# jaeyoungchoilab/Topsicle

Measured on AMD Instinct MI355X. Metric: bases_scanned_per_sec, higher is better.
Workload: dtype u8

## Files before the change

### __graft_entry__.py

```python
import os
import shutil
import subprocess
import sys

ROOT = os.path.dirname(os.path.abspath(__file__))
CSRC = os.path.join(ROOT, "topsicle_amd", "csrc")
LIB = os.path.join(ROOT, "topsicle_amd", "libtopsicle_hip.so")


def _newer(target, deps):
    return os.path.exists(target) and all(os.path.getmtime(target) >= os.path.getmtime(d) for d in deps)


HIP_FLAGS = ["--offload-arch=gfx950", "-O3", "-fno-vectorize", "-std=c++17", "-fPIC", "-Wall", "-Wno-unused-variable"]
KGROUPS = 18


def _build_hip_split(out, extra=()):
    hipcc = shutil.which("hipcc") or "/opt/rocm/bin/hipcc"
    flags = os.environ.get("TPS_HIPCC_EXTRA", "").split() + HIP_FLAGS + list(extra)
    bdir = os.path.join(CSRC, "_build", os.path.splitext(os.path.basename(out))[0])
    os.makedirs(bdir, exist_ok=True)
    jobs = []
    for g in range(KGROUPS):
        src = "topsicle_hip.hip" if g == 0 else "tps_kernels.hip"
        obj = os.path.join(bdir, f"group{g}.o")
        jobs.append((obj, subprocess.Popen([hipcc] + flags + [f"-DTPS_KGROUP={g}", "-c", "-o", obj, os.path.join(CSRC, src)], cwd=CSRC)))
    failed = [obj for obj, p in jobs if p.wait() != 0]
    if failed:
        raise RuntimeError("hipcc failed for " + ", ".join(failed))
    subprocess.check_call([hipcc, "--offload-arch=gfx950", "-shared", "-fPIC", "-o", out] + [obj for obj, _ in jobs], cwd=CSRC)
    return out


def build_hip(force=False):
    deps = [os.path.join(CSRC, f) for f in ("topsicle_hip.hip", "tps_kernels.hip", "tps_kernels.h", "tps_device.h", "tps_wave.h", "tps_plan.h", "tps_pack.h", "tps_wide.h", "tps_wide_plan.h")] + \
           [os.path.join(ROOT, "include", "topsicle_hip.h")]
    if not force and _newer(LIB, deps):
        return LIB
    return _build_hip_split(LIB)


def build_hip_diag():
    return _build_hip_split(os.path.join(ROOT, "topsicle_amd", "libtopsicle_hip_diag.so"), extra=["-DTPS_STAMPS"])


def build_io(force=False):
    src = os.path.join(CSRC, "tps_io.cpp")
    out = os.path.join(ROOT, "topsicle_amd", "libtopsicle_io.so")
    if not force and _newer(out, [src, os.path.join(CSRC, "tps_pack.h"), os.path.join(CSRC, "tps_gzpar.h"), os.path.join(ROOT, "include", "topsicle_hip.h")]):
        return out
    subprocess.check_call(["g++", "-O2", "-std=c++17", "-shared", "-fPIC", "-Wall", "-o", out, src, "-lz", "-lpthread"])
    return out


def build_oracle():
    mk = os.path.join(ROOT, "oracle", "Makefile")
    if os.path.exists(mk):
        subprocess.check_call(["make", "-s", "-C", os.path.join(ROOT, "oracle")])


def build_emulation():
    sys.path.insert(0, os.path.join(ROOT, "tests"))
    sys.path.insert(0, ROOT)
    import emu_driver
    import emu_wide_driver
    emu_driver.build()
    emu_wide_driver.build()


def build_sanitizer_variants():
    sys.path.insert(0, os.path.join(ROOT, "tests"))
    sys.path.insert(0, ROOT)
    import emu_driver
    import emu_wide_driver
    import test_sanitizers
    emu_driver.build(asan=True)
    emu_wide_driver.build(asan=True)
    test_sanitizers._build_io_asan()


def build() -> None:
    import threading
    errs = []

    def side(fn):
        try:
            fn()
        except BaseException as e:
            errs.append(e)
    th = [threading.Thread(target=side, args=(fn,)) for fn in (build_emulation, build_sanitizer_variants)]
    for t in th:
        t.start()
    build_hip()
    build_io()
    build_oracle()
    for t in th:
        t.join()
    if errs:
        raise errs[0]
    sys.path.insert(0, ROOT)
    import topsicle_amd
    from topsicle_amd import hiplib
    lib = hiplib.load_library()
    assert lib.tps_abi_version() == 4
    print("built", LIB)


def smoke() -> None:
    sys.path.insert(0, ROOT)
    sys.path.insert(0, os.path.join(ROOT, "oracle"))
    import numpy as np
    from topsicle_amd import hiplib, synth
    import topsicle_oracle as orc

    motif, k = "CCCTAA", 4
    pats = orc.kmer_table(motif, k)
    bases, offsets, _ = synth.make_reads(24, 3000, motif, seed=7, tract_min=300, tract_max=1500)
    seqs = synth.split_reads(bases, offsets)
    ratio = 1000 / len(motif)
    min_count = max(c for c in range(1001) if not (c / ratio > 0.4))
    with hiplib.HipScanner(0) as sc:
        print("smoke on:", sc.device_info())
        sc.set_patterns(pats)
        sc.upload(0, bases, offsets)
        prm = hiplib.make_params(min_len=1000, min_count=min_count, window=100, slide=6, trimfirst=100, maxlen=20000,
                                 flags=hiplib.F_STEP1 | hiplib.F_WINDOWS | hiplib.F_BINSEG | hiplib.F_STORE_SUMS)
        sc.scan(0, prm)
        sc.sync()
        res = sc.results(0)
        sums, win_off = sc.window_sums(0)
    n_pass = 0
    for i, seq in enumerate(seqs):
        cs, ce = orc.trc_counts(seq, pats)
        call = orc.trc_call(cs, ce, pats, len(motif), 0.4)
        assert bool(res["pass"][i]) == (call is not None), i
        if call is None:
            continue
        n_pass += 1
        tail = call[1]
        assert res["tail"][i] == (0 if tail == "forward" else 1)
        _, counts = orc.window_count_matrix(seq, tail, pats, 100, 6, 100, 20000)
        assert np.array_equal(sums[win_off[i]:win_off[i + 1]], counts.sum(axis=1)), i
        assert res["bkp"][i] == orc.binseg_l2_exact(counts.sum(axis=1)), i
    assert n_pass >= 12
    print(f"smoke ok: {len(seqs)} reads, {n_pass} telomeric, per-window counts bit-exact, boundaries equal")


if __name__ == "__main__":
    build()
    if len(sys.argv) > 1 and sys.argv[1] == "smoke":
        smoke()
```

### topsicle_amd/csrc/tps_device.h

```cpp
#pragma once
#include <stdint.h>
#include "../../include/topsicle_hip.h"
#include "tps_wave.h"

namespace tps {

constexpr int WPG = 4;
constexpr int WPG_MAX = 8;
constexpr uint32_t FLAG_CONFLICT = 0x80000000u;
constexpr uint32_t FLAG16 = 0x8000u;
constexpr int HIST_COPIES = 8;
constexpr int WIN_U = 4;
constexpr int COOP_MAX = 24;

typedef unsigned __int128 u128;

constexpr int cgcd(int a, int b) { return b == 0 ? a : cgcd(b, a % b); }
constexpr int clog2(int x) { return x <= 1 ? 0 : 1 + clog2(x / 2); }

struct PatInfo {
    int32_t P, k;
    uint32_t kmask;
    uint32_t all_mask;
    uint32_t so_mask;
    uint32_t dup_mask;
    int32_t n_periods;
    int32_t period[8];
    uint32_t period_pat[8];
    uint32_t hash_mul, hash_shift;
};

struct ScanArgs {
    const uint32_t* seq2;
    const uint16_t* inv;
    const tps_read_desc* desc;
    const uint8_t* tails_in;
    const uint32_t* lut;
    const uint32_t* lut_img;
    const uint32_t* pair_img;
    tps_read_result* results;
    int32_t* c_start;
    int32_t* c_end;
    const int64_t* win_off;
    int32_t* sums;
    uint16_t* sums16;
    const int64_t* win_off16;
    uint8_t* raw;
    uint64_t* stamps;
    int32_t raw_m;
    const int64_t* raw_win_off;
    const int32_t* order;
    int64_t n_reads;
    PatInfo pat;
    tps_params prm;
    int32_t variant;
    int32_t lut_n;
    int32_t seq_dw;
    int32_t head_dw;
    int32_t nblk_cap;
    int32_t spans_per_tile;
    int32_t span_dw;
    int32_t blk_log2;
    int32_t rec_rs;
    int32_t tot_dw;
    int32_t blk_dw;
    int32_t lc_cap;
    uint32_t jump_magic;
    int32_t q, r, lw;
    int32_t lc16;
    int32_t lc_global;
    int32_t lc_stride;
    uint16_t* lc_scratch;
    int32_t pair_n;
    int32_t tile_cap;
    int32_t tw;
    uint32_t tw_magic;
    int32_t tile_full;
    int32_t wpg;
    int32_t pp_d;
    int32_t so_fast;
    int32_t val_on;
    int32_t seq_alias;
    int32_t lut_fields;
    int32_t lut16;
    int32_t xt_alias;
    int32_t xt_own;
    int32_t pair16;
};

struct BinsegArgs {
    const int32_t* sums;
    const int64_t* win_off;
    int32_t* bkp;
    double* gain;
    int64_t n_reads;
    int32_t n_patterns, jump, min_size;
    uint8_t* tie;
};

constexpr int MISC_DW = 20;
constexpr int XS_DW = 64 + NT + 4 * NT + NT + 16 * 5 + 8;
constexpr int HIST_STRIDE = 33;
constexpr int HIST_DW = 2 * HIST_COPIES * HIST_STRIDE;
struct Lds {
    uint32_t* lut;
    uint32_t* lut2;
    int lshift;
    uint32_t* seq2;
    uint16_t* val;
    uint32_t* blk;
    uint32_t* G;
    uint32_t* Gp;
    uint16_t* C0;
    uint16_t* C1;
    uint32_t* XPC;
    uint32_t* XF;
    uint32_t* XT;
    uint32_t* Tot;
    uint32_t* Lc;
    uint16_t* Lc16;
    uint32_t* Tc;
    uint32_t* row;
    uint32_t* misc;
};
constexpr int XLANES = NT + 16;
TPS_HD int64_t xchg_dw(const ScanArgs& a) {
    return 9ll * NT + (a.xt_alias == 2 ? 0ll : 2ll) * XLANES;
}
TPS_HD int64_t lut_dw(const ScanArgs& a) { return a.lut16 ? ((((int64_t)a.lut_n + 1) / 2 + 3) & ~3ll) : (((int64_t)a.lut_n + 3) & ~3ll); }
TPS_HD int64_t blk_region_dw(const ScanArgs& a) {
    int64_t need = a.variant ? xchg_dw(a) : 2ll * a.nblk_cap + 2ll * ((a.nblk_cap + 1) / 2);
    if (need < XS_DW) need = XS_DW;
    if (need < HIST_DW) need = HIST_DW;
    return (need + 3) & ~3ll;
}
TPS_HD int64_t val_dw(const ScanArgs& a) { return a.val_on ? ((a.seq_dw + 4 + 3) / 4) * 2 : 0; }
TPS_HD int64_t lc_dw(const ScanArgs& a) {
    if (a.lc16) return (a.lc_global ? 0 : ((a.lc_cap + 3) / 4) * 2) + ((a.tile_cap + 1) / 2) * 2;
    return a.lc_global ? 0 : ((a.lc_cap + 1) / 2) * 2;
}
TPS_HD int64_t row_dw(const ScanArgs& a) {
    const int64_t fused = a.variant ? ((int64_t)NT << a.blk_log2) + NT : 0;
    return fused > WIN_U * NT ? fused : WIN_U * NT;
}
TPS_DEV Lds carve(uint32_t* base, uint32_t* lut, const ScanArgs& a) {
    Lds l;
    l.lut2 = lut - a.pair_n;
    uint32_t* p = base;
    l.blk = p;  p += a.blk_dw;
    l.lut = lut;
    l.lshift = a.variant ? 16 : 0;
    l.seq2 = p; p += a.seq_dw;
    l.val = (uint16_t*)p;  p += val_dw(a);
    l.Tot = p;  p += a.tot_dw;
    l.Lc = p;
    l.Lc16 = (uint16_t*)p;
    l.Tc = p + ((a.lc16 && a.lc_global) ? 0 : ((a.lc_cap + 3) / 4) * 2);
    p += lc_dw(a);
    l.row = p;  p += row_dw(a);
    l.misc = p;
    l.G = l.blk;
    l.Gp = l.G + a.nblk_cap;
    l.C0 = (uint16_t*)(l.Gp + a.nblk_cap);
    l.C1 = l.C0 + ((a.nblk_cap + 1) / 2) * 2;
    l.XPC = l.blk;
    l.XF = l.XPC + 9 * NT;
    l.XT = l.XF + XLANES;
    return l;
}
TPS_HD int64_t lds_dwords(const ScanArgs& a) {
    return (int64_t)a.blk_dw + (a.seq_alias ? 0 : a.seq_dw) + val_dw(a) + a.tot_dw + lc_dw(a) + row_dw(a) + MISC_DW +
           ((a.xt_alias && a.xt_own) ? (a.xt_alias == 2 ? 2 : 1) * XLANES : 0);
}
TPS_HD int64_t wg_lds_dwords(const ScanArgs& a) { return a.pair_n + lut_dw(a) + (int64_t)(a.wpg > 0 ? a.wpg : WPG) * ((lds_dwords(a) + 3) & ~3ll); }
constexpr int M_BEST = 0;
constexpr int M_CMASK = 2;
constexpr int M_INVALID = 4;
constexpr int M_SCAN = 10;
constexpr int M_MAXSC = 6;
constexpr int M_BESTB = 8;
constexpr int M_NTIE = 9;
constexpr int X_Q = 0;
constexpr int X_BS = 64;
constexpr int X_CD = X_BS + NT;
constexpr int X_CDEN = X_CD + 2 * NT;
constexpr int X_CB = X_CDEN + 2 * NT;
constexpr int X_R = X_CB + NT;

TPS_DEV int padded(int i, int pad_log2) { return i + (i >> pad_log2); }
TPS_DEV uint32_t wg_exclusive_scan(uint32_t* arr, int n, uint32_t* scratch, int pad_log2 = 30) {
    (void)scratch;
    const int per = (n + NT - 1) / NT;
    Lane<uint32_t> s;
    TPS_LANES {
        const int lo = tid * per, hi = (lo + per < n) ? lo + per : n;
        uint32_t t = 0;
        for (int i = lo; i < hi; ++i) t += arr[padded(i, pad_log2)];
        TPS_AT(s) = t;
    }
    const Lane<uint32_t> inc = wave_incl_sum(s);
    const uint32_t total = wave_read_lane(inc, 63);
    TPS_LANES {
        const int lo = tid * per, hi = (lo + per < n) ? lo + per : n;
        uint32_t run = TPS_AT(inc) - TPS_AT(s);
        for (int i = lo; i < hi; ++i) { uint32_t t = arr[padded(i, pad_log2)]; arr[padded(i, pad_log2)] = run; run += t; }
    }
    TPS_SYNC();
    return total;
}

struct Stage {
    uint64_t q0;
    uint64_t v0;
    int32_t delta;
    int32_t nq;
    int32_t n;
    bool reverse;
};
TPS_DEV Stage stage_plan(const uint32_t* seq2_base, const uint16_t* inv_base, int64_t word_off, int64_t L, bool reverse, int64_t t, int64_t i0, int32_t n) {
    Stage st;
    st.reverse = reverse;
    st.n = n;
    const int64_t pos = reverse ? (L - 1 - t - i0) : (t + i0);
    const int64_t w = word_off + 4 * (pos >> 6);
    st.delta = reverse ? 63 - (int32_t)(pos & 63) : (int32_t)(pos & 63);
    st.q0 = (uint64_t)(uintptr_t)seq2_base + (uint64_t)w * 4u;
    st.v0 = (uint64_t)(uintptr_t)inv_base + (uint64_t)w * 2u;
    st.nq = n > 0 ? (st.delta + n + 63) >> 6 : 0;
    return st;
}
constexpr int STAGE_KMAX = 1 << 16;
TPS_DEV const uint8_t* stage_addr(const Stage& st, int c) {
    const uint8_t* base = (const uint8_t*)(uintptr_t)(st.reverse ? st.q0 - 16ull * STAGE_KMAX : st.q0);
    const uint32_t off = st.reverse ? 16u * (uint32_t)(STAGE_KMAX - c) : 16u * (uint32_t)c;
    return base + off;
}
TPS_DEV const uint8_t* stage_inv_addr(const Stage& st, int c) {
    const uint8_t* base = (const uint8_t*)(uintptr_t)(st.reverse ? st.v0 - 8ull * STAGE_KMAX : st.v0);
    const uint32_t off = st.reverse ? 8u * (uint32_t)(STAGE_KMAX - c) : 8u * (uint32_t)c;
    return base + off;
}
TPS_DEV uint32_t rev2(uint32_t x) {
    const uint32_t y = bitrev32(x);
    return ((y >> 1) & 0x55555555u) | ((y & 0x55555555u) << 1);
}
TPS_DEV u32x4 stage_reversed(const u32x4& v) {
    u32x4 r;
    r.x = rev2(v.w); TPS_PIN_V(r.x);
    r.y = rev2(v.z); TPS_PIN_V(r.y);
    r.z = rev2(v.y); TPS_PIN_V(r.z);
    r.w = rev2(v.x); TPS_PIN_V(r.w);
    return r;
}
TPS_DEV u32x4 stage_orient(const Stage& st, const u32x4& v) {
    if (!st.reverse) return v;
    u32x4 r;
    r.x = rev2(v.w); r.y = rev2(v.z); r.z = rev2(v.y); r.w = rev2(v.x);
    return r;
}
TPS_DEV uint32_t stage_lane_off(bool reverse, int lane) { return reverse ? 16u * (uint32_t)(STAGE_KMAX - lane) : 16u * (uint32_t)lane; }
TPS_DEV const uint8_t* stage_base(const Stage& st, int c0) {
    return (const uint8_t*)(uintptr_t)(st.reverse ? st.q0 - 16ull * STAGE_KMAX - 16ull * (uint32_t)c0 : st.q0 + 16ull * (uint32_t)c0);
}
TPS_DEV const uint8_t* stage_inv_base(const Stage& st, int c0) {
    return (const uint8_t*)(uintptr_t)(st.reverse ? st.v0 - 8ull * STAGE_KMAX - 8ull * (uint32_t)c0 : st.v0 + 8ull * (uint32_t)c0);
}
TPS_DEV u32x2 stage_orient_inv(const Stage& st, const u32x2& v) {
    if (!st.reverse) return v;
    u32x2 r;
    r.x = bitrev32(v.y); r.y = bitrev32(v.x);
    return r;
}

TPS_DEV void stage_thread(const Stage& st, bool has_inv, uint32_t* seq2, uint16_t* val, int nqd, uint32_t* invalid_flag, int tid) {
    for (int base = tid; base < nqd; base += 4 * NT) {
        u32x4 v[4];
        u32x2 b[4];
        TPS_UNROLL
        for (int u = 0; u < 4; ++u) {
            const int c = base + u * NT;
            v[u].x = v[u].y = v[u].z = v[u].w = 0;
            b[u].x = b[u].y = 0;
            if (c < nqd && c < st.nq) {
                v[u] = load16(stage_addr(st, c));
                if (has_inv) b[u] = load8(stage_inv_addr(st, c));
            }
        }
        TPS_UNROLL
        for (int u = 0; u < 4; ++u) {
            const int c = base + u * NT;
            if (c < nqd) {
                lds_store16(seq2 + 4 * c, stage_orient(st, v[u]));
                if (has_inv) {
                    const u32x2 o = stage_orient_inv(st, b[u]);
                    if (o.x | o.y) *invalid_flag = 1u;
                    lds_store8((uint32_t*)val + 2 * c, o);
                }
            }
        }
    }
}

TPS_DEV uint32_t v_at(const uint32_t* seq2, int q) {
    int idx = q >> 4;
    return alignbit(seq2[idx + 1], seq2[idx], (uint32_t)(q & 15) * 2u);
}
TPS_DEV bool invalid_at(const uint16_t* val, int q, int k) {
    int idx = q >> 4;
    uint64_t v = (uint64_t)val[idx] | ((uint64_t)val[idx + 1] << 16) | ((uint64_t)val[idx + 2] << 32);
    return ((v >> (q & 15)) & ((1ull << k) - 1ull)) != 0;
}
constexpr int LUT_FIELDS = 32;
constexpr int LUT_M16 = 48;
constexpr int LUT_F16 = 64;
TPS_HD int pp_field(int p) { return 4 * (p & 3) + 2 * ((p >> 2) & 1) + (p >> 3); }
TPS_HD int pp_pattern(int f) { return (f >> 2) + 4 * (((f >> 1) & 1) + 2 * (f & 1)); }
TPS_HD uint32_t mask_to_fields(uint32_t m) {
    uint32_t f = 0;
    for (int p = 0; p < 16; ++p) f |= ((m >> p) & 1u) << (2 * pp_field(p));
    return f;
}
TPS_DEV uint32_t field_to_mask(uint32_t f) { return f ? 1u << pp_pattern(ffs0(f) >> 1) : 0u; }
TPS_DEV uint32_t field_to_entry(uint32_t f) { return f ? ((1u << (16 + pp_pattern(ffs0(f) >> 1))) | 1u) : 0u; }
template <int N> struct IntC { static constexpr int value = N; };
TPS_DEV uint32_t lut_mask(const uint32_t* lut, int lshift, const PatInfo& pat, uint32_t v) {
    const uint32_t code = v & pat.kmask;
    if (pat.hash_shift) {
        const uint32_t slot = (code * pat.hash_mul) >> pat.hash_shift;
        return lut[2 * slot] == code ? lut[2 * slot + 1] : 0u;
    }
    if (lshift == LUT_FIELDS) return field_to_mask(lut[code]);
    if (lshift == LUT_M16) return ((const uint16_t*)lut)[code];
    if (lshift == LUT_F16) { const uint32_t m = ((const uint16_t*)lut)[code]; return m ? 1u << pp_pattern(ffs0(m)) : 0u; }
    return lut[code] >> lshift;
}
TPS_DEV uint32_t h_at(const uint32_t* lut, int lshift, const uint32_t* seq2, const uint16_t* val, const PatInfo& pat, int q, bool any_invalid) {
    uint32_t h = lut_mask(lut, lshift, pat, v_at(seq2, q));
    if (any_invalid && h && invalid_at(val, q, pat.k)) h = 0;
    return h;
}
TPS_DEV uint32_t conflict_bits(const PatInfo& pat, uint32_t v, uint32_t h) {
    if (pat.hash_shift) return h & pat.so_mask;
    uint32_t c = 0;
    TPS_NOVEC
    for (int i = 0; i < pat.n_periods; ++i) {
        uint32_t hp = h & pat.period_pat[i];
        if (hp && (((v ^ (v >> (2 * pat.period[i]))) & pat.kmask) == 0)) c |= hp;
    }
    return c;
}

TPS_DEV void greedy_count(const uint32_t* lut, int lshift, const uint32_t* seq2, const uint16_t* val, const PatInfo& pat, int q0,
                          int npos, int bit, bool any_invalid, int& occ, int& greedy) {
    occ = 0; greedy = 0;
    int cursor = 0;
    for (int p = 0; p < npos; ++p) {
        uint32_t h = h_at(lut, lshift, seq2, val, pat, q0 + p, any_invalid);
        if ((h >> bit) & 1u) {
            ++occ;
            if (p >= cursor) { ++greedy; cursor = p + pat.k; }
        }
    }
}

template <bool PLAIN>
TPS_DEV void trc_count_thread(const ScanArgs& a, const Lds& l, const Stage& st_s, const Stage& st_e, int tid) {
    const PatInfo& pat = a.pat;
    const int side = tid >> 5, t = tid & 31;
    const int delta = side ? st_e.delta : st_s.delta;
    const uint32_t* seq2 = l.seq2 + side * a.head_dw;
    const uint16_t* val = l.val + side * a.head_dw;
    const bool inv = !PLAIN && l.misc[M_INVALID] != 0;
    const bool so = !PLAIN && pat.so_mask != 0;
    const int npos = st_s.n - pat.k + 1;
    uint32_t* hist = l.blk + (side * HIST_COPIES + (tid & (HIST_COPIES - 1))) * HIST_STRIDE;
    uint32_t cm = 0;
    for (int p0 = t * 8; p0 < npos; p0 += 32 * 8) {
        const int q0 = delta + p0, idx = q0 >> 4;
        const uint32_t sh = (uint32_t)(q0 & 15) * 2u;
        const uint32_t d0 = seq2[idx], d1 = seq2[idx + 1], d2 = seq2[idx + 2];
        const uint32_t w0 = alignbit(d1, d0, sh), w1 = alignbit(d2, d1, sh);
        uint32_t h[8], v[8];
        TPS_UNROLL
        for (int j = 0; j < 8; ++j) {
            v[j] = j ? alignbit(w1, w0, 2u * j) : w0;
            h[j] = lut_mask(l.lut, l.lshift, pat, v[j]);
        }
        TPS_UNROLL
        for (int j = 0; j < 8; ++j) {
            uint32_t hj = h[j];
            if (p0 + j >= npos) hj = 0;
            if (PLAIN) {
                if (hj) lds_add(&hist[ffs0(hj)], 1u);
            } else {
                if (hj && inv && invalid_at(val, q0 + j, pat.k)) hj = 0;
                if (hj) {
                    if (so && (hj & pat.so_mask)) cm |= conflict_bits(pat, v[j], hj);
                    do {
                        int b = ffs0(hj);
                        hj &= hj - 1;
                        lds_add(&hist[b], 1u);
                    } while (hj);
                }
            }
        }
    }
    if (!PLAIN && cm) lds_or(&l.misc[M_CMASK + side], cm);
}
TPS_DEV int min_period(const PatInfo& pat) {
    int m = pat.k;
    TPS_NOVEC
    for (int i = 0; i < pat.n_periods; ++i) m = pat.period[i] < m ? pat.period[i] : m;
    return m;
}
TPS_DEV bool trc_packed_ok(const ScanArgs& a, int npos) {
    const int nchunks = (npos + 15) >> 4, iters = (nchunks + 31) >> 5;
    const int mp = min_period(a.pat);
    int maxd = 0;
    TPS_NOVEC
    for (int i = 0; i < a.pat.n_periods; ++i) maxd = a.pat.period[i] > maxd ? a.pat.period[i] : maxd;
    return a.pat.P <= 15 && maxd <= 6 && mp >= 3 && npos <= 255 * mp && iters * ((16 + mp - 1) / mp) <= 15;
}
template <bool SO_, int FMT = 0>
TPS_DEV void trc_count_packed(const ScanArgs& a, const Lds& l, const Stage& st_s, const Stage& st_e, int tid, uint32_t* keep = nullptr) {
    const PatInfo& pat = a.pat;
    const int side = tid >> 5, t = tid & 31;
    const int delta = side ? st_e.delta : st_s.delta;
    const uint32_t* seq2 = l.seq2 + side * a.head_dw;
    constexpr bool FLD = FMT == 1, M16 = FMT == 2 || FMT == 3, F16 = FMT == 3;
    constexpr int LS = M16 ? 1 : 2;
    const uint32_t amask = pat.kmask << LS;
    const int npos = st_s.n - pat.k + 1;
    const int nchunks = (npos + 15) >> 4;
    const int k = pat.k;
    auto fieldsq = [&](uint32_t h) -> uint32_t { return FLD ? h : M16 ? mul24(h, h) : mulhi32(h, h); };
    uint32_t ne = 0, no = 0;
    uint32_t pe = 0, po = 0, te = 0, to = 0;
    uint32_t cf = 0;
    for (int c0 = 0; c0 < nchunks; c0 += 32) {
        const int c = c0 + t;
        const int bo = 2 * (delta + 16 * c) - LS;
        const int idx = bo >> 5;
        const uint32_t sh = (uint32_t)(bo & 31);
        const uint32_t d0 = seq2[idx], d1 = seq2[idx + 1], d2 = seq2[idx + 2];
        const uint32_t w0 = alignbit(d1, d0, sh), w1 = alignbit(d2, d1, sh);
        uint32_t h[16];
        TPS_UNROLL
        for (int j = 0; j < 16; ++j) {
            const uint32_t v_ = j == 0 ? w0 : alignbit(w1, w0, 2u * j);
            h[j] = M16 ? lut16_at(l.lut, v_, amask) : lut_at(l.lut, v_, amask);
        }
        const bool last_pass = 16 * (c0 + 32) + 32 > npos;
        if (last_pass) {
            int nv = npos - 16 * c;
            TPS_PIN_V(nv);
            TPS_UNROLL
            for (int j = 0; j < 16; ++j)
                if (j >= nv) h[j] = 0;
        }
        TPS_UNROLL
        for (int half = 0; half < 2; ++half) {
            uint32_t x2 = 0;
            TPS_UNROLL
            for (int j = 8 * half; j < 8 * half + 8; ++j) x2 += fieldsq(h[j]);
            ne += x2 & 0x33333333u;
            no += (x2 >> 2) & 0x33333333u;
        }
        if (SO_) {
            const uint32_t w2 = alignbit(seq2[idx + 3], d2, sh);
            const uint32_t a0 = alignbit(w1, w0, (uint32_t)LS), a1 = alignbit(w2, w1, (uint32_t)LS), a2 = w2 >> LS;
            TPS_NOVEC
            for (int pi = 0; pi < pat.n_periods; ++pi) {
                const int d = pat.period[pi];
                const uint32_t x0 = a0 ^ alignbit(a1, a0, 2u * (uint32_t)d), x1 = a1 ^ alignbit(a2, a1, 2u * (uint32_t)d);
// ... 46 lines not shown
    dst[3] = ((no >> 4) & 0x0F0F0F0Fu) - ((po >> 4) & 0x0F0F0F0Fu) + ((to >> 4) & 0x0F0F0F0Fu);
}
constexpr int OCC_SLOTS = 4;
constexpr int OCC_BASE_DW = 256;
TPS_DEV int occ_slot(uint32_t cmask, int p) {
    return popc(cmask & ((1u << p) - 1u));
}
TPS_DEV void trc_publish_occ(const ScanArgs& a, const Lds& l, const Stage& st_s, const Stage& st_e, int tid) {
    const PatInfo& pat = a.pat;
    const int side = tid >> 5, t = tid & 31;
    const uint32_t cmask = l.misc[M_CMASK + side];
    if (!cmask || popc(cmask) > OCC_SLOTS || st_s.n - a.pat.k + 1 > 1024) return;
    const int delta = side ? st_e.delta : st_s.delta;
    const uint32_t* seq2 = l.seq2 + side * a.head_dw;
    const uint32_t amask = pat.kmask << 2;
    const int npos = st_s.n - pat.k + 1;
    const int nchunks = (npos + 15) >> 4;
    uint16_t* occ = (uint16_t*)(l.blk + OCC_BASE_DW + side * OCC_SLOTS * 32);
    for (int c = t; c < 64; c += 32) {
        uint32_t bits[OCC_SLOTS] = {0, 0, 0, 0};
        if (c < nchunks) {
            const int qm = delta + 16 * c - 1;
            const int idx = qm >> 4;
            const uint32_t sh = (uint32_t)(qm & 15) * 2u;
            const uint32_t d0 = seq2[idx], d1 = seq2[idx + 1], d2 = seq2[idx + 2];
            const uint32_t w0 = alignbit(d1, d0, sh), w1 = alignbit(d2, d1, sh);
            TPS_UNROLL
            for (int j = 0; j < 16; ++j) {
                uint32_t h = lut_mask(l.lut, l.lshift, pat, (j ? alignbit(w1, w0, 2u * j) : w0) >> 2);
                if (16 * c + j >= npos) h = 0;
                h &= cmask;
                while (h) {
                    const int b = ffs0(h);
                    h &= h - 1;
                    const int sl = occ_slot(cmask, b);
                    TPS_UNROLL
                    for (int q = 0; q < OCC_SLOTS; ++q)
                        if (q == sl) bits[q] |= 1u << j;
                }
            }
        }
        TPS_UNROLL
        for (int q = 0; q < OCC_SLOTS; ++q) occ[q * 64 + c] = (uint16_t)bits[q];
    }
}
TPS_DEV int trc_walk_occ(const Lds& l, int side, int slot, int k) {
    const uint32_t* occ = l.blk + OCC_BASE_DW + (side * OCC_SLOTS + slot) * 32;
    int greedy = 0, cursor = 0;
    for (int wd = 0; wd < 32; ++wd) {
        uint32_t m = occ[wd];
        while (m) {
            const int p = 32 * wd + ffs0(m);
            m &= m - 1;
            if (p >= cursor) { ++greedy; cursor = p + k; }
        }
    }
    return greedy;
}
TPS_DEV void trc_sum_packed(const ScanArgs& a, const Lds& l, const Stage& st_s, const Stage& st_e, int64_t r, int tid) {
    const int side = tid >> 5, p = tid & 31;
    if (p < a.pat.P) {
        const int pbyte = (l.lshift == LUT_FIELDS || l.lshift == LUT_F16) ? p : 4 * (((p & 1) << 1) | ((p >> 1) & 1)) + (p >> 2);
        const uint8_t* src = (const uint8_t*)(l.blk + 4 * 32 * side) + pbyte;
        uint32_t sm = 0;
        TPS_UNROLL
        for (int t = 0; t < 32; ++t) sm += src[16 * t];
        const uint32_t cmask = l.misc[M_CMASK + side];
        if ((cmask >> p) & 1u) {
            if (popc(cmask) <= OCC_SLOTS && st_s.n - a.pat.k + 1 <= 1024) {
                sm = (uint32_t)trc_walk_occ(l, side, occ_slot(cmask, p), a.pat.k);
            } else {
                int occ, g;
                greedy_count(l.lut, l.lshift, l.seq2 + side * a.head_dw, l.val + side * a.head_dw, a.pat, side ? st_e.delta : st_s.delta,
                             st_s.n - a.pat.k + 1, p, false, occ, g);
                sm = (uint32_t)g;
            }
        }
        int32_t* dst = side ? a.c_end : a.c_start;
        if (dst) dst[r * a.pat.P + p] = (int32_t)sm;
        lds_max_i32((int32_t*)&l.misc[M_BEST + side], (int32_t)((sm << 5) | (uint32_t)(31 - p)));
    }
}

#ifndef TPS_EMU
template <int FMT = 0>
TPS_DEV void trc_decide_packed(const ScanArgs& a, const Lds& l, const Stage& st_s, const Stage& st_e, int64_t r, uint32_t& ks, uint32_t& ke) {
    uint32_t x[4];
    TPS_PHASE { trc_count_packed<false, FMT>(a, l, st_s, st_e, tid, x); }
    uint32_t s0[4], s1[4];
    TPS_UNROLL
    for (int w = 0; w < 4; ++w) {
        uint32_t v = x[w];
        v += (uint32_t)__builtin_amdgcn_update_dpp(0, (int)v, 0x111, 0xf, 0xf, false);
        v += (uint32_t)__builtin_amdgcn_update_dpp(0, (int)v, 0x112, 0xf, 0xf, false);
        v += (uint32_t)__builtin_amdgcn_update_dpp(0, (int)v, 0x114, 0xf, 0xf, false);
        v += (uint32_t)__builtin_amdgcn_update_dpp(0, (int)v, 0x118, 0xf, 0xf, false);
        v += (uint32_t)__builtin_amdgcn_update_dpp(0, (int)v, 0x142, 0xa, 0xf, false);
        s0[w] = (uint32_t)__builtin_amdgcn_readlane((int)v, 31);
        s1[w] = (uint32_t)__builtin_amdgcn_readlane((int)v, 63);
    }
    const int P = a.pat.P;
    uint32_t bs = 0, be = 0;
    TPS_UNROLL
    for (int p = 0; p < 15; ++p) {
        if (p < P) {
            const int wi = ((p & 1) << 1) | ((p >> 1) & 1), sh = 8 * (p >> 2);
            const uint32_t c0 = (s0[wi] >> sh) & 255u, c1 = (s1[wi] >> sh) & 255u;
            const uint32_t k0 = (c0 << 5) | (uint32_t)(31 - p), k1 = (c1 << 5) | (uint32_t)(31 - p);
            bs = k0 > bs ? k0 : bs;
            be = k1 > be ? k1 : be;
        }
    }
    ks = bs;
    ke = be;
    if (a.c_start) {
        const int lane = (int)(threadIdx.x & 63u), side = lane >> 5, p = lane & 31;
        if (p < P) {
            const int wi = ((p & 1) << 1) | ((p >> 1) & 1);
            const uint32_t w0 = wi == 0 ? s0[0] : wi == 1 ? s0[1] : wi == 2 ? s0[2] : s0[3];
            const uint32_t w1 = wi == 0 ? s1[0] : wi == 1 ? s1[1] : wi == 2 ? s1[2] : s1[3];
            const uint32_t c = ((side ? w1 : w0) >> (8 * (p >> 2))) & 255u;
            (side ? a.c_end : a.c_start)[r * P + p] = (int32_t)c;
        }
    }
}
#endif

TPS_DEV void trc_sum_thread(const ScanArgs& a, const Lds& l, const Stage& st_s, const Stage& st_e, int64_t r, int tid) {
    const int side = tid >> 5, p = tid & 31;
    if (p < a.pat.P) {
        uint32_t sm = 0;
        TPS_UNROLL
        for (int c = 0; c < HIST_COPIES; ++c) sm += l.blk[(side * HIST_COPIES + c) * HIST_STRIDE + p];
        if ((l.misc[M_CMASK + side] >> p) & 1u) {
            int occ, g;
            greedy_count(l.lut, l.lshift, l.seq2 + side * a.head_dw, l.val + side * a.head_dw, a.pat, side ? st_e.delta : st_s.delta,
                         st_s.n - a.pat.k + 1, p, l.misc[M_INVALID] != 0, occ, g);
            sm = (uint32_t)g;
        }
        int32_t* dst = side ? a.c_end : a.c_start;
        if (dst) dst[r * a.pat.P + p] = (int32_t)sm;
        lds_max_i32((int32_t*)&l.misc[M_BEST + side], (int32_t)((sm << 5) | (uint32_t)(31 - p)));
    }
}

TPS_DEV void blocks_span(const ScanArgs& a, const Lds& l, int delta, int span) {
    const PatInfo& pat = a.pat;
    const int s = a.prm.slide, r = a.r, k = pat.k;
    const bool inv = l.misc[M_INVALID] != 0;
    const bool so = pat.so_mask != 0;
    const uint32_t sh2 = (uint32_t)(delta & 15) * 2u;
    const int d0 = (delta >> 4) + span * a.span_dw;
    int j = span << a.blk_log2;
    uint32_t lo = l.seq2[d0], hi = l.seq2[d0 + 1];
    uint32_t cur = alignbit(hi, lo, sh2);
    uint32_t g = 0, cnt = 0;
    int pib = 0;
    for (int dw = 0; dw < a.span_dw; ++dw) {
        uint32_t nx2 = l.seq2[d0 + dw + 2];
        uint32_t nxt = alignbit(nx2, hi, sh2);
        uint32_t v[16], h[16];
        TPS_UNROLL
        for (int i = 0; i < 16; ++i) {
            v[i] = i ? alignbit(nxt, cur, 2u * i) : cur;
            h[i] = lut_mask(l.lut, 0, pat, v[i]);
        }
        if (inv) {
            int q = ((d0 + dw) << 4) + (delta & 15);
            TPS_UNROLL
            for (int i = 0; i < 16; ++i)
                if (h[i] && invalid_at(l.val, q + i, k)) h[i] = 0;
        }
        uint32_t cf = 0;
        if (so) {
            TPS_UNROLL
            for (int i = 0; i < 16; ++i)
                if ((h[i] & pat.so_mask) && conflict_bits(pat, v[i], h[i])) cf |= 1u << i;
        }
        TPS_UNROLL
        for (int i = 0; i < 16; ++i) {
            if (pib == 0) {
                g = 0;
                l.C0[j] = (uint16_t)cnt;
                if (r == 0) { l.C1[j] = (uint16_t)cnt; l.Gp[j] = 0; }
            }
            g |= h[i];
            if ((cf >> i) & 1u) g |= FLAG_CONFLICT;
            cnt += (uint32_t)popc(h[i]);
            ++pib;
            if (pib == r) { l.C1[j] = (uint16_t)cnt; l.Gp[j] = g; }
            if (pib == s) { l.G[j] = g; ++j; pib = 0; }
        }
        hi = nx2;
        cur = nxt;
    }
    l.Tot[span] = cnt;
}

template <typename F>
TPS_DEV void scan_positions(const Lds& l, const PatInfo& pat, int q0, int npos, bool inv, F f) {
    const int idx = q0 >> 4;
    const uint32_t sh = (uint32_t)(q0 & 15) * 2u;
    uint32_t d1 = l.seq2[idx + 1];
    uint32_t cur = alignbit(d1, l.seq2[idx], sh), nxt = 0;
    for (int p = 0; p < npos; ++p) {
        const int j = p & 15;
        if (j == 0) {
            if (p) cur = nxt;
            const uint32_t d2 = l.seq2[idx + (p >> 4) + 2];
            nxt = alignbit(d2, d1, sh);
            d1 = d2;
        }
        const uint32_t v = j ? alignbit(nxt, cur, 2u * (uint32_t)j) : cur;
        uint32_t h = lut_mask(l.lut, l.lshift, pat, v);
        if (inv && h && invalid_at(l.val, q0 + p, pat.k)) h = 0;
        f(p, h);
    }
}

TPS_DEV uint32_t window_exact(const ScanArgs& a, const Lds& l, int delta, int wl, uint32_t present, uint32_t fast_sw,
                              uint8_t* raw_row, bool full = false) {
    const PatInfo& pat = a.pat;
    const bool inv = l.misc[M_INVALID] != 0;
    const int q0 = delta + wl * a.prm.slide;
    uint32_t redo = present & pat.so_mask;
    if (!raw_row && !full) {
        uint32_t sum = fast_sw;
        while (redo) {
            const int bit = ffs0(redo);
            redo &= redo - 1;
            int occ = 0, greedy = 0, cursor = 0;
            scan_positions(l, pat, q0, a.lw, inv, [&](int p, uint32_t h) {
                if ((h >> bit) & 1u) {
                    ++occ;
                    if (p >= cursor) { ++greedy; cursor = p + pat.k; }
                }
            });
            sum -= (uint32_t)(occ - greedy);
        }
        return sum;
    }
    uint64_t clo = 0, chi = 0, c3 = 0, c4 = 0;
    scan_positions(l, pat, q0, a.lw, inv, [&](int, uint32_t h) {
        while (h) {
            const int b = ffs0(h);
            h &= h - 1;
            const uint64_t inc = 1ull << (8 * (b & 7));
            const int g = b >> 3;
            clo += g == 0 ? inc : 0ull;
            chi += g == 1 ? inc : 0ull;
            c3 += g == 2 ? inc : 0ull;
            c4 += g == 3 ? inc : 0ull;
        }
    });
    uint32_t sum = 0;
    for (int b = 0; b < pat.P; ++b) {
        const uint64_t word = (b >> 3) == 0 ? clo : (b >> 3) == 1 ? chi : (b >> 3) == 2 ? c3 : c4;
        int c = (int)((word >> (8 * (b & 7))) & 255u);
        if ((redo >> b) & 1u) {
            int greedy = 0, cursor = 0;
            scan_positions(l, pat, q0, a.lw, inv, [&](int p, uint32_t h) {
                if (((h >> b) & 1u) && p >= cursor) { ++greedy; cursor = p + pat.k; }
            });
            c = greedy;
        }
        if (c == 0) c = 1;
        if (raw_row) raw_row[b] = (uint8_t)c;
        sum += (uint32_t)c;
    }
    return sum;
}

TPS_DEV void windows_group(const ScanArgs& a, const Lds& l, int delta, int w0, int nw_tile, int64_t out_base, int base, int tid) {
    const PatInfo& pat = a.pat;
    const int q = a.q;
    for (int u = 0; u < WIN_U; ++u) {
        const int wl = base + u * NT + tid;
        uint32_t sw = 0;
        if (wl < nw_tile) {
            uint32_t m = l.Gp[wl + q];
            for (int i = 0; i < q; ++i) m |= l.G[wl + i];
            int je = wl + q;
            uint32_t cnt = ((uint32_t)l.C1[je] + l.Tot[je >> a.blk_log2]) - ((uint32_t)l.C0[wl] + l.Tot[wl >> a.blk_log2]);
            uint32_t present = m & pat.all_mask;
            sw = cnt + (uint32_t)(pat.P - popc(present));
            uint8_t* raw_row = a.raw ? a.raw + (out_base + w0 + wl) * (int64_t)pat.P : nullptr;
            if ((m & FLAG_CONFLICT) || raw_row) sw = window_exact(a, l, delta, wl, present, sw, raw_row);
            a.sums[out_base + w0 + wl] = (int32_t)sw;
        }
        l.row[u * NT + tid] = sw;
    }
}

TPS_DEV uint32_t div_jump(uint32_t w, uint32_t magic) { return magic ? (uint32_t)(((uint64_t)w * magic) >> 32) : w; }
TPS_DEV void candidates_group(const ScanArgs& a, const Lds& l, uint64_t lc_g, int w0, int nw_tile, int base, uint32_t carry, int tid) {
    const uint32_t jump = (uint32_t)a.prm.jump;
    TPS_UNROLL
    for (int u = 0; u < WIN_U; ++u) {
        const int wl = base + u * NT + tid;
        if (wl < nw_tile) {
            const uint32_t w = (uint32_t)(w0 + wl);
            const uint32_t c = div_jump(w, a.jump_magic);
            if (c * jump == w && (int)c < a.lc_cap) {
                if (lc_g) g32_store(lc_g, c, carry + l.row[u * NT + tid]);
                else l.Lc[c] = carry + l.row[u * NT + tid];
            }
        }
    }
}

struct TileConst {
    int32_t q, r;
    uint32_t jump, jump_magic, lc_cap, lc16;
    uint64_t lc_g;
    uint16_t* sw16;
    int64_t rd;
};
TPS_DEV TileConst tile_const(const ScanArgs& a, int64_t r) {
    TileConst t;
    t.lc_g = a.lc_global ? (uint64_t)(uintptr_t)(a.lc_scratch + r * (int64_t)a.lc_stride) : 0ull;
    t.sw16 = a.sums16 + (a.win_off16 ? a.win_off16[r] : 0);
    t.rd = r;
    t.q = (int32_t)uniform((uint32_t)a.q); t.r = (int32_t)uniform((uint32_t)a.r);
    t.jump = uniform((uint32_t)a.prm.jump); t.jump_magic = uniform(a.jump_magic);
    t.lc_cap = uniform((uint32_t)a.lc_cap); t.lc16 = uniform((uint32_t)a.lc16);
    TPS_PIN_S(t.q); TPS_PIN_S(t.r); TPS_PIN_S(t.jump); TPS_PIN_S(t.jump_magic); TPS_PIN_S(t.lc_cap); TPS_PIN_S(t.lc16);
    return t;
}

template <int S>
struct Geo {
    static constexpr int B = 8;
    static constexpr int LOG2B = 3;
    static constexpr int C = 8;
    static constexpr int LOG2C = 3;
    static constexpr int POS = B * S;
    static constexpr int WDW = (POS + 13 + 15) / 16;
};
constexpr int SEQ_LEAD = 4;
template <int S, bool FULL>
struct TileGeo {
    static constexpr int LANES = FULL ? NT : NT - 1;
    static constexpr int BASES = LANES * Geo<S>::POS + 13 + 15;
    static constexpr int NQ = (63 + BASES + 63) / 64;
    static constexpr int PF = (NQ + NT - 1) / NT;
    static constexpr int SEQ_TILE = SEQ_LEAD + 4 * NQ + 4;
    static constexpr int SEQ = SEQ_TILE < 144 ? 144 : SEQ_TILE;
};
constexpr bool tile_full_default(int s) { return s >= 1; }

template <int S, bool FULL>
TPS_DEV Lds carve_fused(uint32_t* base, uint32_t* lut, const ScanArgs& a) {
    constexpr int BLK = 9 * NT, ROW = NT * Geo<S>::B + NT, SEQ = TileGeo<S, FULL>::SEQ;
    const int VAL = a.val_on ? ((SEQ + 4 + 3) / 4) * 2 : 0;
    static_assert(BLK % 4 == 0 && ROW % 4 == 0 && MISC_DW % 4 == 0 && SEQ % 4 == 0, "seq2 must be 16-byte aligned");
    static_assert(BLK + ROW - SEQ >= HIST_DW && BLK + ROW - SEQ >= 4 * NT, "step 1 counts in front of the aliased bases");
    Lds l;
    l.lut2 = lut - a.pair_n;
    l.lut = lut;
    l.lshift = (a.lut16 && !a.lut_fields && !a.pair16) ? LUT_M16 : (a.lut_fields && a.lut16) ? LUT_F16 : a.lut_fields ? LUT_FIELDS : 16;
    l.blk = base;
    l.XPC = base;
    l.G = l.Gp = base; l.C0 = l.C1 = (uint16_t*)base;
    l.row = base + BLK;
    l.misc = l.row + ROW;
    l.Tot = l.misc + MISC_DW;
    uint32_t* p = l.Tot + 4;
    if (a.seq_alias) {
        l.seq2 = base + (BLK + ROW - SEQ);
    } else {
        l.seq2 = p;
        p += SEQ;
    }
    l.val = (uint16_t*)p;
    p += VAL;
    l.Lc = p;
    l.Lc16 = (uint16_t*)p;
    l.Tc = p + ((a.lc16 && a.lc_global) ? 0 : ((a.lc_cap + 3) / 4) * 2);
    l.XF = p + lc_dw(a);
    l.XT = l.XF + XLANES;
    return l;
}

TPS_DEV uint32_t pack_hi_lo(uint32_t hi_src, uint32_t lo_src) { return perm(hi_src, lo_src, 0x07060100u); }

template <int S, bool SO, bool INV, int RPT, bool RAW>
TPS_DEV void tile_fused_s(const ScanArgs& a, const TileConst& tc, const Lds& l, int delta, int w0, int tile, int nw_tile,
                          int64_t out_base, uint64_t& s_total, int64_t r) {
    constexpr bool RZ = RPT == 0;
    typedef Geo<S> g_;
    constexpr int WDW = g_::WDW, B = g_::B, LOG2B = g_::LOG2B, POS = g_::POS;
    constexpr int RS = NT + NT / B;
    const PatInfo& pat = a.pat;
    const int rp = RPT >= 0 ? RPT : tc.r, q = tc.q;
    const uint32_t amask = pat.kmask << 2;
    TPS_PHASE {
        const int span = tid;
        const int p0 = delta + span * POS;
        const uint32_t sh2 = (uint32_t)((p0 - 1) & 15) * 2u;
        const int d0 = (p0 - 1) >> 4;
        uint32_t w[WDW];
        {
            uint32_t prev = l.seq2[d0];
            TPS_UNROLL
            for (int i = 0; i < WDW; ++i) {
                uint32_t nx = l.seq2[d0 + i + 1];
                w[i] = alignbit(nx, prev, sh2);
                prev = nx;
            }
        }
        uint32_t cnt = 0, run_or = 0;
        uint32_t gs[B], c0s[B];
        uint32_t* xs = l.row + span * (B + 1);
        uint32_t* xpc = l.XPC + span * (B + 1);
        {
            uint32_t hc[S], hn[S];
            auto fetch = [&](int blk, uint32_t* hh, int cnt_) {
                TPS_UNROLL
                for (int i = 0; i < S; ++i) {
                    if (i < cnt_) {
                        const int p = blk * S + i;
                        const int dw = p >> 4, bit = p & 15;
                        uint32_t v4 = bit ? alignbit(dw + 1 < WDW ? w[dw + 1] : 0u, w[dw], 2u * bit) : w[dw];
                        uint32_t h;
                        if constexpr (SO && !RAW) {
                            const uint32_t m16 = lut16_at(l.lut, v4 >> 1, amask >> 1);
                            h = (m16 << 16) | (uint32_t)popc(m16);
                        } else {
                            h = lut_at(l.lut, v4, amask);
                        }
                        if constexpr (INV && RAW) {
                            if (a.lut_fields && a.lut16) {
                                const uint32_t m16 = lut16_at(l.lut, v4 >> 1, amask >> 1);
                                h = m16 ? ((1u << (16 + pp_pattern(ffs0(m16)))) | 1u) : 0u;
                            } else if (a.lut_fields) {
                                h = field_to_entry(h);
                            }
                        }
                        if (INV) {
                            if (h && invalid_at(l.val, p0 + p, pat.k)) h = 0;
                        }
                        hh[i] = h;
                    } else {
                        hh[i] = 0;
                    }
                }
            };
            constexpr int MAXD = S < 6 ? S : 6;
            uint32_t ppd[MAXD + 1];
            if (SO) {
                TPS_UNROLL
                for (int d = 0; d <= MAXD; ++d) ppd[d] = 0;
                TPS_NOVEC
                for (int i = 0; i < pat.n_periods; ++i) {
                    TPS_UNROLL
                    for (int d = 1; d <= MAXD; ++d)
                        if (pat.period[i] == d) ppd[d] |= pat.period_pat[i] << 16;
                }
            }
            fetch(0, hc, S);
            TPS_UNROLL
            for (int blk = 0; blk < B; ++blk) {
                if (blk + 1 < B) fetch(blk + 1, hn, S);
                else if (SO) fetch(B, hn, MAXD);
                uint32_t g = 0;
                c0s[blk] = cnt;
                uint32_t c1 = cnt, pp = run_or;
                if (SO) {
                    uint32_t cf = 0;
                    TPS_UNROLL
                    for (int d = 1; d <= MAXD; ++d) {
                        if (ppd[d]) {
                            TPS_UNROLL
                            for (int i = 0; i < S; ++i) cf |= hc[i] & (i + d < S ? hc[i + d] : hn[i + d - S]) & ppd[d];
                        }
                    }
                    if (cf) g = FLAG16 << 16;
                }
                TPS_UNROLL
                for (int i = 0; i < S; ++i) {
                    const uint32_t h = hc[i];
                    g |= h;
                    cnt += h;
                    if (!RZ) {
                        if (i + 1 == rp) { c1 = cnt; pp = run_or | g; }
                    }
                }
                xpc[blk] = pack_hi_lo(pp, c1);
                gs[blk] = g;
                run_or |= g;
                TPS_UNROLL
                for (int i = 0; i < S; ++i) hc[i] = hn[i];
            }
        }
        uint32_t sfx = 0;
        TPS_UNROLL
        for (int j = B - 1; j >= 0; --j) {
            sfx |= gs[j];
            xs[j] = pack_hi_lo(sfx, c0s[j]);
        }
        l.XF[span] = pack_hi_lo(sfx, cnt);
    }
    TPS_SYNC();
    if (w0 == 0) TPS_STAMP(6);
    if (w0 == 0) TPS_STAMP(7);
    const int rot = q & (B - 1), dl0 = q >> LOG2B;
    Lane<uint32_t> fo_a(0), fo_b(0);
    TPS_PHASE {
        uint32_t orw = 0, sumw = l.XF[tid];
        TPS_NOVEC
        for (int t = 1; t < dl0; ++t) {
            const uint32_t v = l.XF[tid + t];
            orw |= v;
            sumw += v;
        }
        const uint32_t vb = l.XF[tid + dl0];
        TPS_AT(fo_a) = pack_hi_lo(orw, sumw);
        TPS_AT(fo_b) = pack_hi_lo(orw | vb, sumw + vb);
    }
    TPS_SYNC();
    TPS_PHASE {
        l.XF[tid] = TPS_AT(fo_a);
        l.XT[tid] = TPS_AT(fo_b);
    }
    TPS_SYNC();
    Lane<uint32_t> redo_flags(0);
    LaneArr<uint32_t, Geo<S>::B / 2> redo_present = {};
    TPS_PHASE {
        const uint32_t lane = (uint32_t)tid;
        const bool farl = (((lane & (B - 1)) + (uint32_t)rot) >> LOG2B) != 0;
        uint32_t* ps = l.row + (lane + (lane >> LOG2B));
        const uint32_t* pe = l.XPC + ((lane + (uint32_t)q) + ((lane + (uint32_t)q) >> LOG2B));
        const uint32_t* pf = (farl ? l.XT : l.XF) + (lane >> LOG2B);
        uint16_t* out = tc.sw16 + w0;
        uint16_t* outl = out + lane;
        const uint32_t am = pat.all_mask << 16;
        const int nfull = nw_tile >> 6;
        const uint32_t npart = (uint32_t)(nw_tile & 63);
        uint32_t flags = 0;
        uint32_t present[B / 2];
        TPS_UNROLL
        for (int t = 0; t < B / 2; ++t) present[t] = 0;
        uint32_t xv[B], ev[B], fv[B];
        TPS_UNROLL
        for (int u = 0; u < B; ++u) { xv[u] = ps[u * RS]; ev[u] = pe[u * RS]; fv[u] = pf[u * (NT / B)]; }
        TPS_UNROLL
        for (int u = 0; u < B; ++u) {
            uint32_t sw = 0;
            if (u <= nfull) {
                const bool valid = (u < nfull) || (lane < npart);
                const uint32_t x = xv[u], e = ev[u], f = fv[u];
                const uint32_t m = x | e | f;
                const uint32_t s_ = ((e - x + f) & 0xFFFFu) + (uint32_t)popc(~m & am);
                if (valid) {
                    sw = s_;
                    if (SO) {
                        flags |= (m >> 31) << u;
                        present[u / 2] |= (u & 1) ? (m & 0xFFFF0000u) : (m >> 16);
                    }
                    outl[u * NT] = (uint16_t)sw;
                }
            }
            ps[u * RS] = sw;
        }
        if (SO || (RAW && a.raw)) {
            if (RAW && a.raw) {
                const int nv = nfull + ((lane < npart) ? 1 : 0);
                flags = nv >= B ? (1u << B) - 1u : (1u << nv) - 1u;
            }
            TPS_AT(redo_flags) = flags;
            TPS_UNROLL
            for (int t = 0; t < B / 2; ++t) TPS_AT(redo_present)[t] = present[t];
        }
    }
    if (SO || (RAW && a.raw)) {
        TPS_SYNC();
        uint32_t* queue = l.XPC;
        uint32_t* occ = l.XPC + NT * B;
        TPS_PHASE {
            uint32_t flags = TPS_AT(redo_flags);
            uint32_t present[B / 2];
            TPS_UNROLL
            for (int t = 0; t < B / 2; ++t) present[t] = TPS_AT(redo_present)[t];
            while (flags) {
                const int u = ffs0(flags);
                flags &= flags - 1;
                uint32_t pm = 0;
                TPS_UNROLL
                for (int t = 0; t < B / 2; ++t)
                    if (t == (u >> 1)) pm = present[t];
                pm = (pm >> (16 * (u & 1))) & pat.all_mask;
                const uint32_t e = lds_add_ret(&l.misc[M_NTIE], 1u);
                queue[e] = (uint32_t)(u * NT + tid) | (pm << 16);
            }
            occ[tid] = 0;
        }
        TPS_SYNC();
        const int n_redo = (int)uniform(l.misc[M_NTIE]);
        uint16_t* out = tc.sw16 + w0;
        if (n_redo > 0 && !(RAW && a.raw) && n_redo <= COOP_MAX && a.lw <= 128) {
            const bool inv = INV;
            for (int e = 0; e < n_redo; ++e) {
                const uint32_t ent = uniform(queue[e]);
                const int wl = (int)(ent & 0xFFFFu);
                const uint32_t redo = (ent >> 16) & pat.so_mask;
                const int q0 = delta + wl * S;
                TPS_PHASE {
                    for (int p = tid; p < a.lw; p += NT) {
                        uint32_t h = h_at(l.lut, l.lshift, l.seq2, l.val, pat, q0 + p, inv) & redo;
                        while (h) {
                            const int b = ffs0(h);
                            h &= h - 1;
                            lds_or(&occ[4 * b + (p >> 5)], 1u << (p & 31));
                        }
                    }
                }
                TPS_SYNC();
                TPS_PHASE {
                    if (tid < pat.P && ((redo >> tid) & 1u)) {
                        int n_occ = 0, greedy = 0, cursor = 0;
                        TPS_UNROLL
                        for (int wd = 0; wd < 4; ++wd) {
                            uint32_t m = occ[4 * tid + wd];
                            n_occ += popc(m);
                            while (m) {
                                const int p = 32 * wd + ffs0(m);
                                m &= m - 1;
                                if (p >= cursor) { ++greedy; cursor = p + pat.k; }
                            }
                            occ[4 * tid + wd] = 0;
                        }
                        if (n_occ != greedy) lds_add(&occ[60], (uint32_t)(n_occ - greedy));
                    }
                }
                TPS_SYNC();
                TPS_PHASE {
                    if (tid == 0) {
                        const uint32_t sw = l.row[padded(wl, LOG2B)] - occ[60];
                        l.row[padded(wl, LOG2B)] = sw;
                        out[wl] = (uint16_t)sw;
                        occ[60] = 0;
                    }
                }
                TPS_SYNC();
            }
        } else if (n_redo > 0) {
            TPS_PHASE {
                for (int e = tid; e < n_redo; e += NT) {
                    const uint32_t ent = queue[e];
                    const int wl = (int)(ent & 0xFFFFu);
                    uint8_t* raw_row = (RAW && a.raw) ? a.raw + (out_base + w0 + wl) * (int64_t)pat.P : nullptr;
                    const uint32_t sw = window_exact(a, l, delta, wl, ent >> 16, l.row[padded(wl, LOG2B)], raw_row);
                    l.row[padded(wl, LOG2B)] = sw;
                    out[wl] = (uint16_t)sw;
                }
            }
        }
    }
    TPS_SYNC();
    if (w0 == 0) TPS_STAMP(11);
    const uint32_t gsum = wg_exclusive_scan(l.row, NT * B, &l.misc[M_SCAN], LOG2B);
    if (w0 == 0) TPS_STAMP(12);
    {
        const uint32_t jump = tc.jump;
        const uint32_t c_lo = div_jump((uint32_t)w0 + jump - 1u, tc.jump_magic);
        uint32_t c_hi = div_jump((uint32_t)(w0 + nw_tile) + jump - 1u, tc.jump_magic);
        if (c_hi > tc.lc_cap) c_hi = tc.lc_cap;
        const int passes = c_hi > c_lo ? (int)((c_hi - c_lo + NT - 1) / NT) : 0;
        TPS_PHASE {
            const uint32_t carry = (uint32_t)s_total;
            if (tid == 0) { l.misc[M_INVALID] = 0; l.misc[M_NTIE] = 0; }
            if (tc.lc16 && tid == 0) l.Tc[tile] = carry;
            uint32_t c = c_lo + (uint32_t)tid;
            uint32_t w = c * jump - (uint32_t)w0;
            TPS_NOVEC
            for (int t = 0; t < passes; ++t) {
                if (c < c_hi) {
                    const uint32_t pre = l.row[w + (w >> LOG2B)];
                    if (tc.lc16) {
                        if (tc.lc_g) g16_store(tc.lc_g, c, pre);
                        else l.Lc16[c] = (uint16_t)pre;
                    } else if (tc.lc_g) {
                        g32_store(tc.lc_g, c, carry + pre);
                    } else {
                        l.Lc[c] = carry + pre;
                    }
                }
                c += NT;
                w += NT * jump;
            }
        }
    }
    s_total += gsum;
    TPS_SYNC();
}

TPS_DEV void tile_candidates(const TileConst& tc, const Lds& l, int w0, int tile, int nw_tile, uint64_t& s_total) {
    constexpr int B = 8, LOG2B = 3;
    const uint32_t gsum = wg_exclusive_scan(l.row, NT * B, &l.misc[M_SCAN], LOG2B);
    const uint32_t jump = tc.jump;
    const uint32_t c_lo = div_jump((uint32_t)w0 + jump - 1u, tc.jump_magic);
    uint32_t c_hi = div_jump((uint32_t)(w0 + nw_tile) + jump - 1u, tc.jump_magic);
    if (c_hi > tc.lc_cap) c_hi = tc.lc_cap;
    const int passes = c_hi > c_lo ? (int)((c_hi - c_lo + NT - 1) / NT) : 0;
    TPS_PHASE {
        const uint32_t carry = (uint32_t)s_total;
        if (tid == 0) { l.misc[M_INVALID] = 0; l.misc[M_NTIE] = 0; }
        if (tc.lc16 && tid == 0) l.Tc[tile] = carry;
        uint32_t c = c_lo + (uint32_t)tid;
        uint32_t w = c * jump - (uint32_t)w0;
        TPS_NOVEC
        for (int t = 0; t < passes; ++t) {
            if (c < c_hi) {
                const uint32_t pre = l.row[w + (w >> LOG2B)];
                if (tc.lc16) {
                    if (tc.lc_g) g16_store(tc.lc_g, c, pre);
                    else l.Lc16[c] = (uint16_t)pre;
                } else if (tc.lc_g) {
                    g32_store(tc.lc_g, c, carry + pre);
                } else {
                    l.Lc[c] = carry + pre;
                }
            }
            c += NT;
            w += NT * jump;
        }
    }
    s_total += gsum;
    TPS_SYNC();
}

template <int S, bool INV, int RPT, bool PAIR, bool ROTZ, int CD_ = 0, bool P16_ = false>
TPS_DEV void tile_lc_s(const ScanArgs& a, const TileConst& tc, const Lds& l, int delta, int w0, int tile, int nw_tile,
                       int64_t out_base, uint64_t& s_total, int64_t r) {
    static_assert(!(PAIR && INV), "pair lookups need per-position independence");
    constexpr int CD = CD_;
    static_assert(CD == 0 || (!PAIR && !INV && CD <= S), "chain corrections: single lookups on clean tiles, period <= slide");
    static_assert(!(P16_ && CD_ > 0), "the 16-bit pair table is for tables without self-overlap");
    constexpr bool RZ = RPT == 0;
    constexpr bool M16 = CD > 0 || P16_;
    constexpr int LS = M16 ? 1 : 2;
    typedef Geo<S> g_;
    auto xf_at = [&](int lane_) -> uint32_t& { return l.XPC[lane_ * (g_::B + 1) + g_::B]; };
    auto xt_at = [&](int lane_) -> uint32_t& { return l.row[lane_ * (g_::B + 1) + g_::B]; };
    constexpr int B = g_::B, LOG2B = g_::LOG2B, POS = g_::POS;
    constexpr int LB = CD;
    constexpr int WDW = (LB + POS + 13 + 15) / 16;
    static_assert(CD > 0 || WDW == g_::WDW, "the plain tiles keep Geo's register footprint");
    const PatInfo& pat = a.pat;
    int rp = RPT >= 0 ? RPT : tc.r, q = tc.q;
    TPS_PIN_S(q);
    if (RPT < 0) TPS_PIN_S(rp);
    const uint32_t amask = pat.kmask << LS;
    LaneArr<uint32_t, B> sfx_, c0s_;
    Lane<uint32_t> xf_own(0);
    uint32_t lane_chain = 0;
    Lane<uint32_t> pair_lo_(0), pair_hi_(0);
    auto chain_len = [&](int tp, uint32_t pm) -> int {
        constexpr int CD = CD_ > 0 ? CD_ : 1;
        auto occ = [&](int pos) -> bool { return uniform(lut_mask(l.lut, l.lshift, pat, v_at(l.seq2, delta + pos)) & pm) != 0u; };
        const int tend = NT * POS;
        int c = 3;
        while (tp + c * CD < tend && occ(tp + c * CD)) ++c;
        return c;
    };
    auto chain_windows = [&](int tp, int c, int ln) {
        constexpr int CD = CD_ > 0 ? CD_ : 1;
        const int lw = a.lw;
        auto w_in = [&](int e) -> int { const int x = e - lw + 1; return x <= 0 ? 0 : (x + S - 1) / S; };
        auto cur_of = [&](int w) -> int {
            const int a0 = w * S - tp, a1 = w * S + lw - 1 - tp;
            int jlo = a0 <= 0 ? 0 : (a0 + CD - 1) / CD, jhi = a1 < 0 ? -1 : a1 / CD;
            if (jhi > c - 1) jhi = c - 1;
            return jhi > jlo ? (jhi - jlo) >> 1 : 0;
        };
        const int wf = w_in(tp < 0 ? 0 : tp);
        int wb = (tp + (c - 1) * CD) / S + 1;
        if (wb > NT * B - 1) wb = NT * B - 1;
        for (int w = wf + ln; w <= wb; w += NT) {
            const int cur = cur_of(w), prev = w == wf ? 0 : cur_of(w - 1);
            if (cur != prev) lds_add(&l.row[w + (w >> LOG2B)], (uint32_t)(cur - prev));
        }
    };
    constexpr int MK = 10 * S + 1000 * (RPT + 1) + 100000 * ROTZ + 1000000 * PAIR + 10000000 * INV + 100000000 * (CD > 0 || P16_);
    TPS_ISA_MARK(MK + 1);
    TPS_PHASE {
        const int span = tid;
        const int p0 = delta + span * POS;
        const int bo = 2 * (p0 - LB) - LS;
        const uint32_t sh2 = (uint32_t)(bo & 31);
        const int d0 = bo >> 5;
        uint32_t w[WDW];
        {
            uint32_t prev = l.seq2[d0];
            TPS_UNROLL
            for (int i = 0; i < WDW; ++i) {
                uint32_t nx = l.seq2[d0 + i + 1];
                w[i] = alignbit(nx, prev, sh2);
                prev = nx;
            }
        }
        auto v4_at = [&](int p) -> uint32_t {
            const int dw = (p + LB) >> 4, bit = (p + LB) & 15;
            return bit ? alignbit(dw + 1 < WDW ? w[dw + 1] : 0u, w[dw], 2u * bit) : w[dw];
        };
        uint32_t cnt = 0, run_or = 0;
        uint32_t gs[B];
        TPS_AT(pair_lo_) = TPS_AT(pair_hi_) = 0;
        uint32_t* xpc = l.XPC + span * (B + 1);
        if constexpr (PAIR) {
            constexpr int NP = S / 2, NH = NP + (S & 1);
            const uint32_t amask2 = M16 ? ((pat.kmask << 3) | 0x6u) : ((pat.kmask << 4) | 0xCu);
            const int rpe = rp & ~1;
            uint32_t hc[NH], hn[NH];
            auto fetch = [&](int blk, uint32_t* hh) {
                TPS_UNROLL
                for (int j = 0; j < NP; ++j) hh[j] = M16 ? lut16_at(l.lut2, v4_at(blk * S + 2 * j), amask2) : lut_at(l.lut2, v4_at(blk * S + 2 * j), amask2);
                if (S & 1) hh[NP] = M16 ? lut16_at(l.lut, v4_at(blk * S + S - 1), amask) : lut_at(l.lut, v4_at(blk * S + S - 1), amask);
            };
            fetch(0, hc);
            TPS_UNROLL
            for (int blk = 0; blk < B; ++blk) {
                if (blk + 1 < B) fetch(blk + 1, hn);
                uint32_t g = 0;
                TPS_AT(c0s_)[blk] = cnt;
                if (RZ) xpc[blk] = M16 ? ((run_or << 16) | cnt) : pack_hi_lo(run_or, cnt);
                TPS_UNROLL
                for (int j = 0; j < NH; ++j) {
                    if (!RZ) {
                        if (2 * j == rpe) {
                            uint32_t c1 = cnt, pp = run_or | g;
                            if (rp & 1) {
                                const uint32_t h1 = M16 ? lut16_at(l.lut, v4_at(blk * S + 2 * j), amask) : lut_at(l.lut, v4_at(blk * S + 2 * j), amask);
                                c1 = M16 ? c1 + (uint32_t)popc(h1) : c1 + h1;
                                pp |= h1;
                            }
                            xpc[blk] = M16 ? ((pp << 16) | c1) : pack_hi_lo(pp, c1);
                        }
                    }
                    g |= hc[j];
                    cnt = M16 ? cnt + (uint32_t)popc(hc[j]) : cnt + hc[j];
                }
                gs[blk] = g;
                run_or |= g;
                TPS_UNROLL
                for (int j = 0; j < NH; ++j) hc[j] = hn[j];
            }
        } else {
            uint32_t hc[S], hn[S];
            auto fetch = [&](int blk, uint32_t* hh, int cnt_) {
                TPS_UNROLL
                for (int i = 0; i < S; ++i) {
                    if (i < cnt_) {
                        const int p = blk * S + i;
                        uint32_t h = M16 ? lut16_at_wide(l.lut, v4_at(p), amask) : lut_at(l.lut, v4_at(p), amask);
                        if (INV) {
                            if (h && invalid_at(l.val, p0 + p, pat.k)) h = 0;
                        }
                        hh[i] = h;
                    } else {
                        hh[i] = 0;
                    }
                }
            };
            fetch(0, hc, S);
            constexpr int NB_ = CD > 0 ? CD : 1;
            uint32_t hb[NB_];
            if constexpr (CD > 0) {
                TPS_UNROLL
                for (int i = 0; i < CD; ++i) hb[i] = lut16_at_wide(l.lut, v4_at(i - CD), amask);
            }
            TPS_UNROLL
            for (int blk = 0; blk < B; ++blk) {
                if (blk + 1 < B) fetch(blk + 1, hn, S);
                if constexpr (CD > 0) {
                    uint32_t cfb = 0;
                    TPS_UNROLL
                    for (int i = 0; i < S; ++i) cfb |= hc[i] & (i >= CD ? hc[i - CD] : hb[i]);
                    if (cfb != 0u) {
                        TPS_UNROLL
                        for (int i = 0; i < S; ++i) {
                            const uint32_t pr = (hc[i] & (i >= CD ? hc[i - CD] : hb[i])) ? 1u : 0u;
                            if (blk * S + i < 32) TPS_AT(pair_lo_) |= pr << ((blk * S + i) & 31);
                            else TPS_AT(pair_hi_) |= pr << ((blk * S + i) & 31);
                        }
                    }
                    TPS_UNROLL
                    for (int i = 0; i < CD; ++i) hb[i] = hc[S - CD + i];
                }
                uint32_t g = 0;
                TPS_AT(c0s_)[blk] = cnt;
                uint32_t c1 = cnt, pp = run_or;
                constexpr bool CNT_OR = CD > 0 && CD >= S - 2;
                if constexpr (CNT_OR) {
                    uint32_t g_rp = 0, dup = 0, dup_rp = 0;
                    TPS_UNROLL
                    for (int i = 0; i < S; ++i) {
                        g |= hc[i];
                        if (!RZ) {
                            if (i + 1 == rp) g_rp = g;
                        }
                        if (i >= CD) {
                            const uint32_t t = (uint32_t)popc(hc[i] & hc[i - CD]);
                            dup += t;
                            if (!RZ) {
                                if (i < rp) dup_rp += t;
                            }
                        }
                    }
                    if (CD == S - 2) dup += (uint32_t)popc(hc[S - 1] & hc[0]);
                    if (!RZ) { pp = run_or | g_rp; c1 = cnt + (uint32_t)popc(g_rp) + dup_rp; }
                    cnt += (uint32_t)popc(g) + dup;
                } else {
                TPS_UNROLL
                for (int i = 0; i < S; ++i) {
                    const uint32_t h = hc[i];
                    g |= h;
                    cnt = M16 ? cnt + (uint32_t)popc(h) : cnt + h;
                    if (!RZ) {
                        if (i + 1 == rp) { c1 = cnt; pp = run_or | g; }
                    }
                }
                }
                xpc[blk] = M16 ? ((pp << 16) | c1) : pack_hi_lo(pp, c1);
                gs[blk] = g;
                run_or |= g;
                TPS_UNROLL
                for (int i = 0; i < S; ++i) hc[i] = hn[i];
            }
        }
        uint32_t sf = 0;
        TPS_UNROLL
        for (int j = B - 1; j >= 0; --j) {
            sf = M16 ? ((gs[j] << 16) | sf) : (sf | gs[j]);
            TPS_AT(sfx_)[j] = sf;
        }
        TPS_AT(xf_own) = M16 ? (sf | cnt) : pack_hi_lo(sf, cnt);
        xf_at(span) = TPS_AT(xf_own);
        if constexpr (CD > 0) { TPS_PIN_V(TPS_AT(pair_lo_)); TPS_PIN_V(TPS_AT(pair_hi_)); }
    }
    if constexpr (CD > 0) {
        constexpr int PS = 8;
        Lane<bool> has_pair;
        TPS_LANES { TPS_AT(has_pair) = (TPS_AT(pair_lo_) | TPS_AT(pair_hi_)) != 0u; }
        const bool tile_pairs = wave_ballot(has_pair) != 0;
        if (tile_pairs) {
            TPS_SYNC();
            Lane<uint32_t> head3_lo(0), head3_hi(0);
            TPS_PHASE {
                const int lane = tid;
                const uint32_t pair_lo = TPS_AT(pair_lo_), pair_hi = TPS_AT(pair_hi_);
                auto below = [&](int n) -> uint32_t {
                    if (n <= 0) return 0u;
                    if (n >= 64) return (uint32_t)(popc(pair_lo) + popc(pair_hi));
                    if (n <= 32) return (uint32_t)popc(n == 32 ? pair_lo : (pair_lo & ((1u << n) - 1u)));
                    return (uint32_t)(popc(pair_lo) + popc(pair_hi & ((1u << (n - 32)) - 1u)));
                };
                if ((pair_lo | pair_hi) != 0u) {
                    uint32_t* xpc = l.XPC + lane * (B + 1);
                    TPS_UNROLL
                    for (int blk = 0; blk < B; ++blk) {
                        const uint32_t pe = below(blk * S + (RZ ? 0 : RPT));
                        if (pe) lds_add(&xpc[blk], pe << PS);
                        TPS_AT(c0s_)[blk] += below(blk * S + CD) << PS;
                    }
                    const uint32_t pt = below(64) << PS;
                    TPS_AT(xf_own) += pt;
                    lds_add(&xf_at(lane), pt);
                }
                uint32_t prev_hi = wave_shuffle(pair_hi_, lane, (lane + NT - 1) & (NT - 1));
                const uint32_t prev_lo_ = wave_shuffle(pair_lo_, lane, (lane + NT - 1) & (NT - 1));
                uint32_t next_lo = wave_shuffle(pair_lo_, lane, (lane + 1) & (NT - 1));
                if (lane == 0) prev_hi = 0u;
                if (lane == NT - 1) next_lo = 0u;
                const uint64_t pm64 = ((uint64_t)pair_hi << 32) | pair_lo;
                const uint64_t pv64 = lane > 0 ? (((uint64_t)prev_hi << 32) | prev_lo_) : 0ull;
                const uint64_t before = (pm64 << CD) | (pv64 >> (POS - CD));
                const uint64_t after = (pm64 >> CD) | ((uint64_t)(next_lo & ((1u << CD) - 1u)) << (POS - CD));
                const uint64_t lim = POS >= 64 ? ~0ull : ((1ull << POS) - 1ull);
                const uint64_t h3 = pm64 & ~before & after & lim;
                TPS_AT(head3_lo) = (uint32_t)h3; TPS_AT(head3_hi) = (uint32_t)(h3 >> 32);
            }
            Lane<bool> has_head3;
            TPS_LANES { TPS_AT(has_head3) = (TPS_AT(head3_lo) | TPS_AT(head3_hi)) != 0u; }
            const bool tile_long = wave_ballot(has_head3) != 0;
            if (tile_long) {
                TPS_PHASE {
                    TPS_UNROLL
                    for (int i = 0; i < B + 1; ++i) l.row[tid + i * NT] = 0;
                }
                TPS_SYNC();
                auto one_owner = [&](int src, uint32_t h_lo, uint32_t h_hi, auto&& each_lane) {
                    while (h_lo | h_hi) {
                        int e;
                        if (h_lo) { e = ffs0(h_lo); h_lo &= h_lo - 1u; }
                        else { e = 32 + ffs0(h_hi); h_hi &= h_hi - 1u; }
                        const int te = src * POS + e;
                        const uint32_t pm = uniform(lut_mask(l.lut, l.lshift, pat, v_at(l.seq2, delta + te)));
                        const int c = chain_len(te - CD, pm);
                        each_lane(te - CD, c);
                    }
                };
                {
                    const int ln = tps_fresh_lane();
                    uint64_t owners = wave_ballot(has_head3);
                    while (owners) {
                        const int src = __builtin_ctzll(owners);
                        owners &= owners - 1ull;
                        const uint32_t h_lo = wave_read_lane(head3_lo, src), h_hi = wave_read_lane(head3_hi, src);
                        one_owner(src, h_lo, h_hi, [&](int tp, int c) { TPS_PHASE_WITH(ln) chain_windows(tp, c, tid); });
                    }
                }
                lane_chain = 1u;
            }
        }
    }
    TPS_SYNC();
    if (w0 == 0) TPS_STAMP(6);
    TPS_ISA_MARK(MK + 2);
    const int rot = ROTZ ? 0 : (q & (B - 1)), dl0 = q >> LOG2B;
    const int brk = B - rot;
    constexpr bool SWP = CD == 0 && !M16 && ROTZ;
    LaneArr<uint32_t, B> sw_;
    LaneArr<uint32_t, B / 2> swp_;
    Lane<uint32_t> ltot(0);
    TPS_PHASE {
        const int lane = tid;
        uint32_t* const sw = TPS_AT(sw_);
        uint32_t* const swp = TPS_AT(swp_);
        const uint32_t* const sfx = TPS_AT(sfx_);
        const uint32_t* const c0s = TPS_AT(c0s_);
        const uint32_t* pe = l.XPC + (lane + dl0) * (B + 1) + rot;
        uint32_t ev[B];
        TPS_UNROLL
        for (int j = 0; j < B; ++j) ev[j] = pe[j + ((!ROTZ && j >= brk) ? 1 : 0)];
        uint32_t orw = 0, sumw = TPS_AT(xf_own);
        TPS_NOVEC
        for (int t = 1; t < dl0; ++t) {
            const uint32_t v = xf_at(lane + t);
            orw |= v;
            sumw += v;
        }
        uint32_t orb = orw, sumb = sumw;
        if (!ROTZ) {
            const uint32_t vb = xf_at(lane + dl0);
            orb |= vb;
            sumb += vb;
        }
        const uint32_t am = pat.all_mask << 16;
        orw |= ~am;
        orb |= ~am;
        uint32_t run = 0;
        if constexpr (SWP) {
            if (tid == 0) TPS_EMU_COUNT(3);
            uint32_t lo_lo = 0x05040100u;
            TPS_PIN_S(lo_lo);
            TPS_UNROLL
            for (int j = 0; j < B; j += 2) {
                const uint32_t ep = perm(ev[j + 1], ev[j], lo_lo), cp = perm(c0s[j + 1], c0s[j], lo_lo);
                const uint32_t d = pk_u16_add(pk_u16_sub(ep, cp), sumw);
                const uint32_t p = (uint32_t)popc(~(sfx[j] | ev[j] | orw)) + d;
                swp[j >> 1] = p + ((uint32_t)popc(~(sfx[j + 1] | ev[j + 1] | orw)) << 16);
                sw[j] = swp[j >> 1] & 0xFFFFu;
                sw[j + 1] = swp[j >> 1] >> 16;
                run += sw[j] + sw[j + 1];
            }
        } else {
        TPS_UNROLL
        for (int j = 0; j < B; ++j) {
            const bool far_ = !ROTZ && j >= brk;
            const uint32_t e = ev[j], fo = far_ ? orb : orw, fs = far_ ? sumb : sumw;
            const uint32_t c = (e - c0s[j] + fs) & 0xFFFFu;
            sw[j] = (CD > 0 ? (c & 0xFFu) - (c >> 8) : c) + (uint32_t)popc(~(sfx[j] | e | fo));
            run += sw[j];
        }
        }
        TPS_AT(ltot) = run;
    }
    TPS_ISA_MARK(MK + 3);
    if constexpr (CD > 0) {
        const bool tile_chain = lane_chain != 0;
        if (tile_chain) {
            TPS_EMU_COUNT(5);
            LaneArr<uint32_t, B> pd;
            Lane<uint32_t> dt(0);
            TPS_PHASE {
                const uint32_t* pr = l.row + tid * (B + 1);
                TPS_UNROLL
                for (int j = 0; j < B; ++j) { TPS_AT(dt) += pr[j]; TPS_AT(pd)[j] = TPS_AT(dt); }
            }
            const Lane<uint32_t> dbase = wave_excl_sum(dt);
            TPS_LANES {
                uint32_t run = 0;
                TPS_UNROLL
                for (int j = 0; j < B; ++j) { TPS_AT(sw_)[j] += TPS_AT(dbase) + TPS_AT(pd)[j]; run += TPS_AT(sw_)[j]; }
                TPS_AT(ltot) = run;
            }
        } else {
            TPS_EMU_COUNT(6);
        }
    }
    const Lane<uint32_t> lexc = wave_excl_sum(ltot);
    bool lane_cands = false;
    if constexpr (CD == 0 && !M16) lane_cands = tc.lc_g != 0ull && !tc.lc16 && tc.jump >= 4u;
    TPS_PHASE {
        const int lane = tid;
        const uint32_t* const sw = TPS_AT(sw_);
        if constexpr (SWP) g_store_sw8p(tc.sw16 + w0, lane, nw_tile, TPS_AT(swp_));
        else g_store_sw8(tc.sw16 + w0, lane, nw_tile, sw);
        uint32_t* pr = l.row + lane * (B + 1);
        uint32_t run = 0;
        TPS_UNROLL
        for (int j = 0; j < B; ++j) { pr[j] = run; run += sw[j]; }
        xt_at(lane) = TPS_AT(lexc);
        if (lane_cands) {
            if (tid == 0) TPS_EMU_COUNT(7);
            const uint32_t carry = (uint32_t)s_total + TPS_AT(lexc);
            const uint32_t wl = (uint32_t)(lane * B), wa = (uint32_t)w0 + wl;
            const uint32_t c = mulhi32(wa + tc.jump - 1u, tc.jump_magic);
            const uint32_t f = c * tc.jump - wa;
            if (f < (uint32_t)B && wl + f < (uint32_t)nw_tile && c < tc.lc_cap) g32_store(tc.lc_g, c, carry + pr[f]);
            const uint32_t f2 = f + tc.jump;
            if (f2 < (uint32_t)B && wl + f2 < (uint32_t)nw_tile && c + 1u < tc.lc_cap) g32_store(tc.lc_g, c + 1u, carry + pr[f2]);
        }
    }
    TPS_SYNC();
    if (w0 == 0) TPS_STAMP(12);
    TPS_ISA_MARK(MK + 4);
    const uint32_t gsum = uniform(l.row[nw_tile + (nw_tile >> LOG2B)] + xt_at(nw_tile >> LOG2B));
    {
        const uint32_t jump = tc.jump;
        const uint32_t c_lo = div_jump((uint32_t)w0 + jump - 1u, tc.jump_magic);
        uint32_t c_hi = div_jump((uint32_t)(w0 + nw_tile) + jump - 1u, tc.jump_magic);
        if (c_hi > tc.lc_cap) c_hi = tc.lc_cap;
        const int passes = (c_hi > c_lo && !lane_cands) ? (int)((c_hi - c_lo + NT - 1) / NT) : 0;
        TPS_ISA_MARK(MK + 6);
        TPS_PHASE {
            const uint32_t carry = (uint32_t)s_total;
            if (tid == 0) { l.misc[M_INVALID] = 0; l.misc[M_NTIE] = 0; }
            if (tc.lc16 && tid == 0) l.Tc[tile] = carry;
            uint32_t c = c_lo + (uint32_t)tid;
            uint32_t w = c * jump - (uint32_t)w0;
            TPS_NOVEC
            for (int t = 0; t < passes; ++t) {
                if (c < c_hi) {
                    const uint32_t pre = l.row[w + (w >> LOG2B)] + xt_at((int)(w >> LOG2B));
                    if (tc.lc16) {
                        if (tc.lc_g) g16_store(tc.lc_g, c, pre);
                        else l.Lc16[c] = (uint16_t)pre;
                    } else if (tc.lc_g) {
                        g32_store(tc.lc_g, c, carry + pre);
                    } else {
                        l.Lc[c] = carry + pre;
                    }
                }
                c += NT;
                w += NT * jump;
            }
        }
    }
    s_total += gsum;
    TPS_ISA_MARK(MK + 5);
    TPS_SYNC();
    (void)r;
}

template <int S>
struct GeoPP {
    static constexpr int B = 8, POS = B * S, LBK = 16;
    static constexpr int WDW = (1 + LBK + POS + 6 + 7 + 15) / 16;
};
constexpr uint32_t PP_BIAS = 14;
TPS_DEV void pp_expand(uint32_t ne, uint32_t no, uint32_t* b) {
    b[0] = ne & 0x0F0F0F0Fu;
    b[1] = (ne >> 4) & 0x0F0F0F0Fu;
    b[2] = no & 0x0F0F0F0Fu;
    b[3] = (no >> 4) & 0x0F0F0F0Fu;
}

template <int S, int D, int CD = 0, bool F16 = false, int RPT = -1, bool PAIRF = false>
TPS_DEV bool tile_pp_s(const ScanArgs& a, const TileConst& tc, const Lds& l, int delta, int w0, int tile, int nw_tile,
                       int64_t out_base, uint64_t& s_total) {
    static_assert(CD == 0 || (D == 0 && CD <= 6), "chain detection runs on the tile without self-overlap logic");
    static_assert(RPT < S, "r is a position inside a block");
    static_assert(!PAIRF || (D == 0 && CD == 0 && !F16 && RPT >= 0 && (RPT & 1) == 0), "pair lookups: plain tiles, the partial block ends between two pairs");
    constexpr int B = 8, POS = B * S, LBK = D > 0 ? 2 * D + 2 : 0;
    constexpr int WDW = (1 + LBK + POS + 6 + 7 + 15) / 16;
    constexpr int DH = D > 0 ? D : 1;
    constexpr int AHEAD = (D > 0 && 2 * D > S) ? 2 * D - S : 0;
    constexpr uint32_t M3 = 0x33333333u;
    const PatInfo& pat = a.pat;
    int rp = RPT >= 0 ? RPT : tc.r, q = tc.q;
    if constexpr (RPT < 0) TPS_PIN_S(rp);
    TPS_PIN_S(q);
    constexpr int LS = F16 ? 1 : 2;
    const uint32_t amask = pat.kmask << LS;
    uint32_t* ende = l.XPC;
    uint32_t* endo = l.row;
    uint32_t* tne = ende + B;
    uint32_t* tno = endo + B;
    uint32_t* carry = l.misc + M_SCAN;
    const int cblk = a.tw & (B - 1), clane = a.tw >> 3;
    uint32_t cold[7];
    TPS_UNROLL
    for (int i = 0; i < 7; ++i) cold[i] = (D > 0) ? uniform(carry[i]) : 0u;
    auto picked_before_tile = [&](int pos, int fidx) -> bool {
        uint32_t cv = 0;
        TPS_UNROLL
        for (int i = 0; i < DH; ++i) cv = (pos - (delta - DH) == i) ? cold[i] : cv;
        return w0 != 0 && ((cv >> (2 * fidx)) & 1u) != 0;
    };
    if (CD == 0) TPS_EMU_COUNT(0);
    LaneArr<uint32_t, B> ve_, vo_;
    Lane<uint32_t> chm_(0), chw_(0), unc_(0);
    Lane<uint32_t> chain_any_(0);
    TPS_PHASE {
        const int span = tid;
        uint32_t* const ve = TPS_AT(ve_);
        uint32_t* const vo = TPS_AT(vo_);
        uint32_t &chm = TPS_AT(chm_), &chw = TPS_AT(chw_), &unc = TPS_AT(unc_), &chain_any = TPS_AT(chain_any_);
        const int p0 = delta + span * POS;
        const int bo = 2 * (p0 - LBK) - LS;
        const uint32_t sh2 = (uint32_t)(bo & 31);
        const int d0 = bo >> 5;
        uint32_t w[WDW];
        {
            uint32_t prev = l.seq2[d0];
            TPS_UNROLL
            for (int i = 0; i < WDW; ++i) {
                uint32_t nx = l.seq2[d0 + i + 1];
                w[i] = alignbit(nx, prev, sh2);
                prev = nx;
            }
        }
        auto look = [&](int p) -> uint32_t {
            const int idx = p + LBK, dw = idx >> 4, bit = idx & 15;
            const uint32_t v4 = bit ? alignbit(dw + 1 < WDW ? w[dw + 1] : 0u, w[dw], 2u * bit) : w[dw];
            if constexpr (F16) {
                const uint32_t m = lut16_at(l.lut, v4, amask);
                return mul24(m, m);
            }
            const uint32_t h = lut_at(l.lut, v4, amask);
            return h;
        };
        uint32_t pk[LBK + POS + AHEAD + 1];
        uint32_t tv[POS + 1];
        if constexpr (D > 0) {
            uint32_t ca[LBK > 0 ? LBK : 1];
            TPS_UNROLL
            for (int i = 0; i < LBK; ++i) {
                const uint32_t h = look(i - LBK);
                if (i >= DH) {
                    pk[i] = h ^ (h & pk[i - DH]);
                    ca[i] = h & ca[i - DH];
                } else {
                    pk[i] = h;
                    ca[i] = h;
                }
            }
            TPS_UNROLL
            for (int i = LBK - DH; i < LBK; ++i) unc |= ca[i];
            if (unc && span > 0) {
                unc = 0;
                TPS_UNROLL
                for (int i = LBK - DH; i < LBK; ++i) {
                    if (ca[i]) {
                        const int fidx = ffs0(ca[i]) >> 1, pidx = pp_pattern(fidx);
                        int n = 0, pw = p0 - LBK + (i % DH) - DH;
                        while (pw >= delta && ((lut_mask(l.lut, l.lshift, pat, v_at(l.seq2, pw)) >> pidx) & 1u)) { ++n; pw -= DH; }
                        const bool blocked = pw < delta && picked_before_tile(pw, fidx);
                        if (pw < delta && w0 != 0 && cold[6]) unc |= ca[i];
                        else if (((n & 1) != 0) != blocked) pk[i] ^= ca[i];
                    }
                }
            }
            if (span == 0) {
                TPS_UNROLL
                for (int i = 0; i < DH; ++i) pk[LBK - DH + i] = cold[i];
                unc = cold[6];
            }
        }
        uint32_t pe = 0, po = 0;
        uint32_t ch3[B];
        TPS_UNROLL
        for (int blk = 0; blk < B; ++blk) ch3[blk] = 0;
        TPS_UNROLL
        for (int blk = 0; blk < B; ++blk) {
            if (D > 0) {
                if (blk == cblk && span == clane) {
                    TPS_UNROLL
                    for (int i = 0; i < DH; ++i) carry[i] = pk[LBK + blk * S - DH + i];
                    carry[6] = unc;
                }
            }
            uint32_t acc = 0, pb = 0, sfw = 0;
            if constexpr (PAIRF) {
                const uint32_t amask2 = (pat.kmask << 4) | 0xCu;
                TPS_UNROLL
                for (int i = 0; i + 1 < S; i += 2) {
                    const int idx = blk * S + i, dw = idx >> 4, bit = idx & 15;
                    const uint32_t v4 = bit ? alignbit(dw + 1 < WDW ? w[dw + 1] : 0u, w[dw], 2u * bit) : w[dw];
                    acc += lut_at(l.lut2, v4, amask2);
                    if (i + 2 == RPT) pb = acc;
                }
                if (S & 1) acc += look(blk * S + S - 1);
            } else {
            TPS_UNROLL
            for (int i = 0; i < S; ++i) {
                const int p = blk * S + i;
                const uint32_t h = look(p);
                uint32_t t = 0;
                if (D > 0) {
                    t = h & pk[LBK + p - DH];
                    if (i < D) sfw |= t;
                    const int pm = p - D;
                    if (pm >= 0 && pm % S < D) ch3[pm / S] |= h & tv[pm];
                }
                tv[p] = t;
                const uint32_t pick = h ^ t;
                pk[LBK + p] = pick;
                if constexpr (CD > 0) {
                    if (p >= CD) chain_any |= h & pk[p - CD];
                }
                acc += pick;
                if constexpr (RPT >= 0) { if (i + 1 == RPT) pb = acc; }
                else pb = (i + 1 == rp) ? acc : pb;
            }
            }
            const uint32_t ee = pe + (pb & M3), eo = po + ((pb >> 2) & M3);
            ende[span * (B + 1) + blk] = ee;
            endo[span * (B + 1) + blk] = eo;
            ve[blk] = PP_BIAS * 0x11111111u - pe + (sfw & M3);
            vo[blk] = PP_BIAS * 0x11111111u - po + ((sfw >> 2) & M3);
            pe += acc & M3;
            po += (acc >> 2) & M3;
            if (D > 0 && blk > 0) {
                chm |= ch3[blk - 1] ? (1u << (blk - 1)) : 0u;
                chw |= ch3[blk - 1];
                TPS_PIN_V(chm); TPS_PIN_V(chw);
            }
        }
        if (D > 0) {
            TPS_UNROLL
            for (int i = 0; i < AHEAD; ++i) {
                const int p = POS + i, pm = p - D;
                if (pm % S < D) ch3[pm / S] |= look(p) & tv[pm];
            }
            chm |= ch3[B - 1] ? (1u << (B - 1)) : 0u;
            chw |= ch3[B - 1];
        }
        if constexpr (CD > 0) {
            TPS_UNROLL
            for (int i = 0; i < CD; ++i) chain_any |= look(POS + i) & pk[POS + i - CD];
        }
        tne[span * (B + 1)] = pe;
        tno[span * (B + 1)] = po;
        TPS_PIN_V(chm); TPS_PIN_V(chw); TPS_PIN_V(unc);
        TPS_UNROLL
        for (int i = 0; i < B; ++i) { TPS_PIN_V(ve[i]); TPS_PIN_V(vo[i]); }
    }
    TPS_SYNC();
    TPS_PP_STAMP(6);
    if constexpr (CD > 0) {
        Lane<bool> has_chain;
        TPS_LANES { TPS_AT(has_chain) = TPS_AT(chain_any_) != 0; }
        const bool chained = wave_ballot(has_chain) != 0;
        if (chained) return true;
        TPS_EMU_COUNT(0);
        TPS_EMU_COUNT(7);
    }
    uint64_t unc_mask = 0;
    if (D > 0) {
        Lane<bool> is_unc;
        TPS_LANES { TPS_AT(is_unc) = TPS_AT(unc_) != 0; }
        unc_mask = wave_ballot(is_unc);
        TPS_EMU_COUNT_N(2, __builtin_popcountll(unc_mask));
    }
    const int rot = q & (B - 1), dl0 = q >> 3;
    LaneArr<uint32_t, B> swv_;
    LaneArr<uint32_t[3], B> rows_;
    LaneArr<uint32_t, B / 2> rx_;
    Lane<uint32_t> todo_(0);
    const bool staged = a.raw != nullptr && (pat.P & 3) == 0;
    const bool staged16 = a.raw != nullptr && (pat.P & 3) != 0;
    TPS_PHASE {
        const int lane = tid;
        const uint32_t* const ve = TPS_AT(ve_);
        const uint32_t* const vo = TPS_AT(vo_);
        uint32_t* const swv = TPS_AT(swv_);
        uint32_t (*const rows)[3] = TPS_AT(rows_);
        uint32_t* const rx = TPS_AT(rx_);
        bool redo_all = false;
        if (D > 0) redo_all = ((unc_mask >> lane) & ((2ull << (dl0 + 1)) - 1ull)) != 0;
        const uint32_t* pee = ende + lane * (B + 1);
        const uint32_t* peo = endo + lane * (B + 1);
        uint32_t ee[B], eo[B];
        TPS_UNROLL
        for (int j = 0; j < B; ++j) {
            const int eb = j + q;
            ee[j] = pee[eb + (eb >> 3)];
            eo[j] = peo[eb + (eb >> 3)];
        }
        if (D > 0) {
            TPS_AT(todo_) = redo_all ? 0xFFu : (TPS_AT(chm_) << 8);
        }
        const int nv = nw_tile - lane * B;
        auto windows = [&](auto nw_c) {
            constexpr int NW = decltype(nw_c)::value;
            uint32_t fa[NW], fb[NW];
            TPS_UNROLL
            for (int i = 0; i < NW; ++i) fa[i] = 0;
            TPS_NOVEC
            for (int t = 0; t < dl0; ++t) {
                uint32_t x[4];
                pp_expand(tne[(lane + t) * (B + 1)], tno[(lane + t) * (B + 1)], x);
                TPS_UNROLL
                for (int i = 0; i < NW; ++i) fa[i] += x[i];
            }
            {
                uint32_t x[4];
                pp_expand(tne[(lane + dl0) * (B + 1)], tno[(lane + dl0) * (B + 1)], x);
                TPS_UNROLL
                for (int i = 0; i < NW; ++i) {
                    fa[i] -= PP_BIAS * 0x01010101u;
                    fb[i] = fa[i] + x[i];
                }
            }
            uint32_t fc[NW];
            TPS_UNROLL
            for (int i = 0; i < NW; ++i) fc[i] = fa[i];
            const int brk = B - rot;
            TPS_UNROLL
            for (int j = 0; j < B; ++j) {
                if (j == brk) {
                    TPS_UNROLL
                    for (int i = 0; i < NW; ++i) { fc[i] = fb[i]; TPS_PIN_V(fc[i]); }
                }
                uint32_t v[4], e[4], c[4] = {0, 0, 0, 0};
                pp_expand(ve[j], vo[j], v);
                pp_expand(ee[j], eo[j], e);
                uint32_t sw = (uint32_t)pat.P - 4u * NW;
                TPS_UNROLL
                for (int i = 0; i < NW; ++i) {
                    c[i] = fc[i] + v[i] + e[i];
                    c[i] |= ((0x80808080u - c[i]) >> 7) & 0x01010101u;
                    sw = add_bytes(c[i], sw);
                }
                swv[j] = j < nv ? sw : 0u;
                TPS_UNROLL
                for (int i = 0; i < 3; ++i) rows[j][i] = c[i];
                if (j & 1) rx[j >> 1] = pack_hi_lo(c[3] << 16, rx[j >> 1]);
                else rx[j >> 1] = c[3] & 0xFFFFu;
            }
        };
        if (pat.P <= 12) windows(IntC<3>{});
        else windows(IntC<4>{});
        g_store_sw8(tc.sw16 + w0, lane, nw_tile, swv);
// ... 75 lines not shown
        uint16_t* gout = (uint16_t*)(a.raw + (out_base + w0) * (int64_t)pat.P);
        for (int l0 = 0; l0 < NT; l0 += LPP) {
            TPS_PHASE {
                if (tid >= l0 && tid < l0 + LPP) {
                    uint32_t* dst = buf + (tid - l0) * B * 4;
                    uint32_t (*const rows)[3] = TPS_AT(rows_);
                    const uint32_t* const rx = TPS_AT(rx_);
                    TPS_UNROLL
                    for (int j = 0; j < B; ++j) {
                        u32x4 t;
                        t.x = rows[j][0]; t.y = rows[j][1]; t.z = rows[j][2]; t.w = (rx[j >> 1] >> (16 * (j & 1))) & 0xFFFFu;
                        *(u32x4*)(dst + 4 * j) = t;
                    }
                }
            }
            TPS_SYNC();
            if ((pat.P & 1) == 0) {
                TPS_PHASE {
                    int nvalid = (nw_tile - l0 * B) * ph;
                    const int ncap = LPP * B * ph;
                    if (nvalid > ncap) nvalid = ncap;
                    uint16_t* g = gout + (int64_t)l0 * B * ph;
                    const uint16_t* b16 = (const uint16_t*)buf;
                    for (int u = tid; u < nvalid; u += NT) {
                        const uint32_t row = ((uint32_t)u * ph_magic) >> 16;
                        g[u] = b16[row * 8u + ((uint32_t)u - row * (uint32_t)ph)];
                    }
                }
            } else {
                const uint32_t pb = (uint32_t)pat.P, pb_magic = (65536u + pb - 1u) / pb;
                TPS_PHASE {
                    int nvalid = (nw_tile - l0 * B) * (int)pb;
                    const int ncap = LPP * B * (int)pb;
                    if (nvalid > ncap) nvalid = ncap;
                    uint8_t* g = (uint8_t*)gout + (int64_t)l0 * B * pb;
                    const uint8_t* b8 = (const uint8_t*)buf;
                    for (int u = tid; u < nvalid; u += NT) {
                        const uint32_t row = ((uint32_t)u * pb_magic) >> 16;
                        g[u] = b8[row * 16u + ((uint32_t)u - row * pb)];
                    }
                }
            }
            TPS_SYNC();
        }
    }
    TPS_PHASE {
        TPS_UNROLL
        for (int j = 0; j < B; ++j) l.row[tid * (B + 1) + j] = TPS_AT(swv_)[j];
        if constexpr (CD > 0) {
            if (tid == clane) {
                TPS_UNROLL
                for (int i = 0; i < 7; ++i) carry[i] = 0u;
            }
        }
    }
    TPS_SYNC();
    if (D > 0) {
        TPS_FENCE_WG();
        TPS_PHASE {
            const int lane = tid;
            uint32_t todo = TPS_AT(todo_);
            const uint32_t chw = TPS_AT(chw_);
            while (todo) {
                const int bit = ffs0(todo);
                todo &= todo - 1u;
                const int j = bit & 7, wl = lane * B + j;
                if (wl >= nw_tile) continue;
                uint8_t* raw_row = a.raw ? a.raw + (out_base + w0 + wl) * (int64_t)pat.P : nullptr;
                if (a.raw && a.raw_m == 2)
                    raw_row = ((w0 + wl) & 1) ? nullptr : a.raw + (a.raw_win_off[tc.rd] + ((w0 + wl) >> 1)) * (int64_t)pat.P;
                uint32_t sw = l.row[lane * (B + 1) + j];
                if (bit < 8) {
                    TPS_EMU_COUNT(1);
                    sw = window_exact(a, l, delta, wl, pat.all_mask, 0u, raw_row, true);
                } else {
                    TPS_EMU_COUNT(3);
                    const int a0 = delta + wl * S;
                    uint32_t fw = chw;
                    bool lost = false;
                    while (fw) {
                        const int fidx = ffs0(fw) >> 1, pidx = pp_pattern(fidx);
                        fw &= fw - 1u;
                        int x = -1;
                        TPS_NOVEC
                        for (int i = 0; i < D; ++i)
                            if ((lut_mask(l.lut, l.lshift, pat, v_at(l.seq2, a0 + i)) >> pidx) & 1u) x = a0 + i;
                        if (x >= 0) {
                            int n = 0, pb = x - D;
                            while (pb >= delta && ((lut_mask(l.lut, l.lshift, pat, v_at(l.seq2, pb)) >> pidx) & 1u)) { ++n; pb -= D; }
                            const bool blocked = pb < delta && picked_before_tile(pb, fidx);
                            if (pb < delta && w0 != 0 && cold[6]) lost = true;
                            int m = 1;
                            for (int pw = x + D; pw < a0 + a.lw && ((lut_mask(l.lut, l.lshift, pat, v_at(l.seq2, pw)) >> pidx) & 1u); pw += D) ++m;
                            if ((((n & 1) != 0) != blocked) && (m & 1) == 0) {
                                sw -= 1u;
                                if (raw_row) raw_row[pidx] = (uint8_t)(raw_row[pidx] - 1u);
                            }
                        }
                    }
                    if (lost) {
                        TPS_EMU_COUNT(1);
                        sw = window_exact(a, l, delta, wl, pat.all_mask, 0u, raw_row, true);
                    }
                }
                l.row[lane * (B + 1) + j] = sw;
                tc.sw16[w0 + wl] = (uint16_t)sw;
            }
        }
        TPS_SYNC();
    }
    TPS_PP_STAMP(11);
    tile_candidates(tc, l, w0, tile, nw_tile, s_total);
    TPS_PP_STAMP(12);
    return false;
}

struct Cand { uint64_t d; uint64_t den; int32_t b; };
TPS_DEV bool cand_better(const Cand& x, const Cand& y) {
    if (x.b < 0) return false;
    if (y.b < 0) return true;
    u128 lhs = (u128)x.d * x.d * y.den;
    u128 rhs = (u128)y.d * y.d * x.den;
    if (lhs != rhs) return lhs > rhs;
    return x.b > y.b;
}
TPS_DEV bool binseg_admissible(int n, int jump, int min_size) {
    if (n / jump < 1) return false;
    int need = ((min_size + jump - 1) / jump) * jump + min_size;
    return need <= n;
}
template <typename ST>
TPS_DEV Cand binseg_chunk(const ST* S, int n, int jump, int min_size, int lo, int hi, uint64_t prefix, uint64_t total) {
    Cand best{0, 1, -1};
    uint64_t run = prefix;
    for (int b = lo; b < hi; ++b) {
        if (b % jump == 0 && b >= min_size && n - b >= min_size) {
            int64_t d = (int64_t)n * (int64_t)run - (int64_t)total * (int64_t)b;
            Cand c{(uint64_t)(d < 0 ? -d : d), (uint64_t)b * (uint64_t)(n - b), b};
            if (cand_better(c, best)) best = c;
        }
        run += (uint64_t)S[b];
    }
    return best;
}
TPS_DEV double score_f64(int64_t d, uint64_t den) {
    double x = (double)d;
    return x * x / (double)den;
}
TPS_DEV double gain_from(int64_t d, uint64_t den, int n, int n_patterns) {
    double x = (double)d;
    return x * x / ((double)n * (double)den) / ((double)n_patterns * (double)n_patterns);
}

template <typename ST>
TPS_DEV Cand binseg_exact_wg(const ST* S, int n, int jump, int min_size, uint32_t* xs) {
    const int cl = (n + NT - 1) / NT;
    TPS_PHASE {
        int lo = tid * cl, hi = lo + cl < n ? lo + cl : n;
        uint32_t sm = 0;
        for (int i = lo; i < hi; ++i) sm += (uint32_t)S[i];
        xs[X_BS + tid] = sm;
    }
    TPS_SYNC();
    constexpr int NG = NT / 16;
    TPS_PHASE {
        if (tid < NG) {
            uint32_t sm = 0;
            for (int i = 0; i < 16; ++i) sm += xs[X_BS + tid * 16 + i];
            xs[X_Q + tid] = sm;
        }
    }
    TPS_SYNC();
    TPS_PHASE {
        if (tid == 0) {
            uint32_t run = 0;
            for (int i = 0; i < NG; ++i) { uint32_t t = xs[X_Q + i]; xs[X_Q + i] = run; run += t; }
            xs[X_Q + 16] = run;
        }
    }
    TPS_SYNC();
    TPS_PHASE {
        uint64_t pre = xs[X_Q + (tid >> 4)];
        for (int i = (tid & ~15); i < tid; ++i) pre += xs[X_BS + i];
        int lo = tid * cl, hi = lo + cl < n ? lo + cl : n;
        Cand c = binseg_chunk(S, n, jump, min_size, lo, hi, pre, (uint64_t)xs[X_Q + 16]);
        ((uint64_t*)&xs[X_CD])[tid] = c.d;
        ((uint64_t*)&xs[X_CDEN])[tid] = c.den;
        ((int32_t*)&xs[X_CB])[tid] = c.b;
    }
    TPS_SYNC();
    TPS_PHASE {
        if (tid < NG) {
            Cand best{0, 1, -1};
            for (int i = 0; i < 16; ++i) {
                int t = tid * 16 + i;
                Cand c{((uint64_t*)&xs[X_CD])[t], ((uint64_t*)&xs[X_CDEN])[t], ((int32_t*)&xs[X_CB])[t]};
                if (cand_better(c, best)) best = c;
            }
            ((uint64_t*)&xs[X_R])[tid] = best.d;
            ((uint64_t*)&xs[X_R + 32])[tid] = best.den;
            ((int32_t*)&xs[X_R + 64])[tid] = best.b;
        }
    }
    TPS_SYNC();
    Cand best{0, 1, -1};
    for (int i = 0; i < NG; ++i) {
        Cand c{((uint64_t*)&xs[X_R])[i], ((uint64_t*)&xs[X_R + 32])[i], ((int32_t*)&xs[X_R + 64])[i]};
        if (cand_better(c, best)) best = c;
    }
    TPS_SYNC();
    return best;
}

constexpr int CHUNK_REGS = 16;
template <typename ST>
TPS_DEV void binseg_wg(const ST* S, int n, int jump, int min_size, int n_patterns, uint32_t* bs, uint32_t* misc,
                       uint32_t* xs, int& bkp, double& gain, bool& tie) {
    const int per = (n + jump * NT - 1) / (jump * NT);
    const int cl = per * jump;
    const bool in_regs = cl <= CHUNK_REGS;
    TPS_PHASE {
        const int lo = tid * cl, hi = lo + cl < n ? lo + cl : n;
        uint32_t sm = 0;
        if (in_regs) {
            TPS_UNROLL
            for (int i = 0; i < CHUNK_REGS; ++i)
                if (lo + i < hi) sm += (uint32_t)S[lo + i];
        } else {
            for (int i = lo; i < hi; ++i) sm += (uint32_t)S[i];
        }
        bs[tid] = sm;
        if (tid == 0) { *(uint64_t*)&misc[M_MAXSC] = 0ull; misc[M_BESTB] = (uint32_t)-1; misc[M_NTIE] = 0u; }
    }
    TPS_SYNC();
    const uint64_t tot = wg_exclusive_scan(bs, NT, &misc[M_SCAN]);
    Lane<double> best_(-1.0), second_(-1.0);
    Lane<int> best_b_(-1);
    TPS_PHASE {
        double &best = TPS_AT(best_), &second = TPS_AT(second_);
        int& best_b = TPS_AT(best_b_);
        const int lo = tid * cl, hi = lo + cl < n ? lo + cl : n;
        uint64_t run = bs[tid];
        best = -1.0; second = -1.0; best_b = -1;
        auto visit = [&](int b, uint32_t sv, int& j) {
            if (j == 0 && b >= min_size && n - b >= min_size) {
                int64_t d = (int64_t)n * (int64_t)run - (int64_t)tot * (int64_t)b;
                double sc = score_f64(d, (uint64_t)b * (uint64_t)(n - b));
                if (sc >= best) { second = best; best = sc; best_b = b; }
                else if (sc > second) second = sc;
            }
            run += (uint64_t)sv;
            if (++j == jump) j = 0;
        };
        int j = 0;
        if (in_regs) {
            TPS_UNROLL
            for (int i = 0; i < CHUNK_REGS; ++i)
                if (lo + i < hi) visit(lo + i, (uint32_t)S[lo + i], j);
        } else {
            for (int b = lo; b < hi; ++b) visit(b, (uint32_t)S[b], j);
        }
        uint64_t bits = 0;
        if (best >= 0.0) __builtin_memcpy(&bits, &best, 8);
        wg_max_bits(bits, (uint64_t*)&misc[M_MAXSC]);
    }
    TPS_SYNC();
    TPS_PHASE {
        const double best = TPS_AT(best_), second = TPS_AT(second_);
        const int best_b = TPS_AT(best_b_);
        double m;
        __builtin_memcpy(&m, &misc[M_MAXSC], 8);
        const double thr = m * (1.0 - 1e-14);
        uint32_t near = (best >= thr && best >= 0.0 ? 1u : 0u) + (second >= thr && second >= 0.0 ? 1u : 0u);
        if (near) lds_add(&misc[M_NTIE], near);
        if (best == m && best_b >= 0) lds_max_i32((int32_t*)&misc[M_BESTB], best_b);
    }
    TPS_SYNC();
    tie = misc[M_NTIE] > 1u;
    if (tie) {
        Cand ex = binseg_exact_wg(S, n, jump, min_size, xs);
        bkp = ex.b;
        gain = ex.b < 0 ? 0.0 : gain_from((int64_t)ex.d, ex.den, n, n_patterns);
    } else {
        bkp = (int32_t)misc[M_BESTB];
        double m;
        __builtin_memcpy(&m, &misc[M_MAXSC], 8);
        gain = bkp < 0 ? 0.0 : m / (double)n / ((double)n_patterns * (double)n_patterns);
        TPS_SYNC();
    }
}

template <typename ST>
TPS_DEV void binseg_from_lc(const ScanArgs& a, const Lds& l, uint64_t lc_g, const ST* S_global, int n, uint64_t tot, int jump,
                            int min_size, int n_patterns, uint32_t* misc, uint32_t* xs, int& bkp, double& gain, bool& tie) {
    const int ncand = (n - 1) / jump;
    Lane<double> best_(-1.0);
    Lane<int> best_b_(-1);
    Lane<bool> amb_(false);
    Lane<uint64_t> bits_(0);
    const int c_min = (min_size + jump - 1) / jump > 1 ? (min_size + jump - 1) / jump : 1;
    const int c_max = (n - min_size) / jump < ncand ? (n - min_size) / jump : ncand;
    const bool exact53 = (double)n * 4294967296.0 < 9007199254740992.0 && (double)tot * (double)n < 9007199254740992.0;
    const double nf = (double)n, totf = (double)tot;
    const bool int_d = (double)tot * (double)n < 2147483648.0;
    constexpr int LCV = 16;
    const bool prefilter = !a.lc16 && lc_g && exact53 && c_max - c_min < LCV * NT;
    int nslot = c_max >= c_min ? (c_max - c_min + NT) / NT : 0;
    TPS_PIN_S(nslot);
    auto tile_sum = [&](int c) { return l.Tc[(uint32_t)(((uint64_t)(uint32_t)(c * jump) * a.tw_magic) >> 32)]; };
    Lane<float> p_s1_(-1.0f), p_s2_(-1.0f);
    Lane<uint32_t> p_lc_(0);
    Lane<int> p_c_(-1);
    float thr32 = -1.0f;
    bool crowded = false;
    TPS_ISA_REGION(5);
    if (prefilter) {
        auto prefilter_phase = [&](auto lean_) {
        TPS_PHASE {
            float &p_s1 = TPS_AT(p_s1_), &p_s2 = TPS_AT(p_s2_);
            uint32_t& p_lc = TPS_AT(p_lc_);
            int& p_c = TPS_AT(p_c_);
            p_s1 = -1.0f; p_s2 = -1.0f; p_lc = 0; p_c = -1;
            auto group = [&](int g) {
                constexpr bool LEAN = decltype(lean_)::value != 0;
                uint32_t lcv[4];
                TPS_UNROLL
                for (int i = 0; i < 4; ++i) {
                    const int c = c_min + tid + (4 * g + i) * NT;
                    if constexpr (LEAN) lcv[i] = g32_load_at(lc_g, 4u * (uint32_t)(c <= c_max ? c : c_max));
                    else lcv[i] = c <= c_max ? g32_load(lc_g, (uint32_t)c) : 0u;
                }
                const int b0 = (c_min + tid + 4 * g * NT) * jump;
                const uint32_t tb0 = (uint32_t)tot * (uint32_t)b0, tb_step = (uint32_t)tot * (uint32_t)(NT * jump);
                TPS_UNROLL
                for (int i = 0; i < 4; ++i) {
                    const int c = c_min + tid + (4 * g + i) * NT;
                    const int b = LEAN ? b0 + i * (NT * jump) : c * jump;
                    float d32;
                    if constexpr (LEAN) {
                        uint32_t tb = tb0 + (uint32_t)i * tb_step;
                        TPS_PIN_V(tb);
                        d32 = (float)(int32_t)((uint32_t)n * lcv[i] - tb);
                    } else {
                        const double bf = (double)b;
                        d32 = (float)__builtin_fma(-totf, bf, nf * (double)lcv[i]);
                    }
                    const float den32 = (float)b * (float)(n - b);
                    float s_ = d32 * d32 * rcp_f32(den32);
                    s_ = c <= c_max ? s_ : -1.0f;
                    const bool gt = s_ > p_s1;
                    const float lose = gt ? p_s1 : s_;
                    p_s2 = lose > p_s2 ? lose : p_s2;
                    p_lc = gt ? lcv[i] : p_lc;
                    p_c = gt ? c : p_c;
                    p_s1 = gt ? s_ : p_s1;
                }
            };
            if (nslot > 0) group(0);
            if (nslot > 4) group(1);
            if (nslot > 8) group(2);
            if (nslot > 12) group(3);
        }
        };
        if (int_d) prefilter_phase(IntC<1>());
        else prefilter_phase(IntC<0>());
        float m32;
        {
            Lane<uint32_t> key;
            TPS_LANES {
                const float nn = TPS_AT(p_s1_) > 0.0f ? TPS_AT(p_s1_) : 0.0f;
                __builtin_memcpy(&TPS_AT(key), &nn, 4);
            }
            const uint32_t mb = wave_max_u32(key);
            __builtin_memcpy(&m32, &mb, 4);
        }
        thr32 = m32 * (1.0f - 1e-4f);
        Lane<bool> close2;
        TPS_LANES { TPS_AT(close2) = TPS_AT(p_s2_) >= thr32 && TPS_AT(p_s2_) >= 0.0f; }
        crowded = wave_ballot(close2) != 0;
    }
    TPS_ISA_REGION(6);
    TPS_PHASE {
        double bn = -1.0, bd = 1.0;
        int best_b = -1;
        bool amb = false;
        auto offer = [&](int c, uint32_t lc) {
            const int b = c * jump;
            const double bf = (double)b;
            double dd;
            if (exact53) dd = __builtin_fma(-totf, bf, nf * (double)lc);
            else dd = (double)((int64_t)n * (int64_t)lc - (int64_t)tot * (int64_t)b);
            const double num = dd * dd, den = bf * (nf - bf);
            const double t1 = num * bd, t2 = bn * den;
            const double diff = t1 - t2;
            const bool near = __builtin_fabs(diff) <= 1e-13 * t2;
            const bool take = diff >= 0.0;
            amb = near || (amb && !take);
            if (take) { bn = num; bd = den; best_b = b; }
        };
        if (prefilter) {
            if (TPS_AT(p_c_) >= 0 && TPS_AT(p_s1_) >= thr32) offer(TPS_AT(p_c_), TPS_AT(p_lc_));
        } else if (a.lc16 && lc_g && c_max - c_min < LCV * NT) {
            uint32_t lcv[LCV];
            TPS_UNROLL
            for (int i = 0; i < LCV; ++i) {
                const int c = c_min + tid + i * NT;
                lcv[i] = c <= c_max ? g16_load(lc_g, (uint32_t)c) : 0u;
            }
            TPS_UNROLL
            for (int i = 0; i < LCV; ++i) {
                const int c = c_min + tid + i * NT;
                if (c <= c_max) offer(c, tile_sum(c) + lcv[i]);
            }
        } else {
            TPS_NOVEC
            for (int c = c_min + tid; c <= c_max; c += NT) {
                uint32_t lc;
                if (a.lc16) lc = tile_sum(c) + (lc_g ? g16_load(lc_g, (uint32_t)c) : (uint32_t)l.Lc16[c]);
                else lc = lc_g ? g32_load(lc_g, (uint32_t)c) : l.Lc[c];
                offer(c, lc);
            }
        }
        const double best = best_b >= 0 ? bn / bd : -1.0;
        uint64_t bits = 0;
        if (best >= 0.0) __builtin_memcpy(&bits, &best, 8);
        TPS_AT(best_) = best; TPS_AT(best_b_) = best_b; TPS_AT(amb_) = amb; TPS_AT(bits_) = bits;
    }
    double m;
    uint32_t ntie = 0;
    int32_t bestb = -1;
    {
        Lane<uint32_t> key;
        TPS_LANES { TPS_AT(key) = (uint32_t)(TPS_AT(bits_) >> 32); }
        const uint32_t mh = wave_max_u32(key);
        TPS_LANES { TPS_AT(key) = (uint32_t)(TPS_AT(bits_) >> 32) == mh ? (uint32_t)TPS_AT(bits_) : 0u; }
        const uint32_t ml = wave_max_u32(key);
        const uint64_t mbits = ((uint64_t)mh << 32) | ml;
        __builtin_memcpy(&m, &mbits, 8);
        Lane<bool> n1, n1_amb;
        TPS_LANES {
            const double best = TPS_AT(best_);
            const bool amb = TPS_AT(amb_), near = best >= m * (1.0 - 1e-14) && best >= 0.0;
            TPS_AT(n1) = near;
            TPS_AT(n1_amb) = near && amb;
        }
        ntie = (uint32_t)__builtin_popcountll(wave_ballot(n1)) + (uint32_t)__builtin_popcountll(wave_ballot(n1_amb));
        TPS_LANES {
            const double best = TPS_AT(best_);
            const int best_b = TPS_AT(best_b_);
            TPS_AT(key) = (best == m && best_b >= 0) ? (uint32_t)best_b + 1u : 0u;
        }
        bestb = (int32_t)wave_max_u32(key) - 1;
    }
    (void)misc;
    TPS_ISA_REGION(7);
    if (crowded) ntie = 2u;
    tie = ntie > 1u;
    if (ntie > 1u) {
        TPS_EMU_COUNT(4);
        Cand ex = binseg_exact_wg(S_global, n, jump, min_size, xs);
        bkp = ex.b;
        gain = ex.b < 0 ? 0.0 : gain_from((int64_t)ex.d, ex.den, n, n_patterns);
    } else {
        bkp = bestb;
        gain = bkp < 0 ? 0.0 : m / (double)n / ((double)n_patterns * (double)n_patterns);
    }
}

template <int SV, bool SO, bool PAIR = false, bool RAW = true, bool FULL = tile_full_default(SV), int DCLASS = 0>
TPS_DEV void scan_read(const ScanArgs& a, int64_t r, uint32_t* lds_base, uint32_t* lut) {
    constexpr bool M16K = SV != 0 && SO && !RAW;
    constexpr bool F16K = SV != 0 && SO && RAW && DCLASS == 3;
    constexpr bool P16K = SV != 0 && !SO && !RAW && PAIR && DCLASS == 4;
    Lds l_ = SV ? carve_fused<SV ? SV : 5, FULL>(lds_base, lut, a) : carve(lds_base, lut, a);
    if constexpr (P16K) l_.lshift = LUT_M16;
    const Lds l = l_;
    const PatInfo& pat = a.pat;
    const tps_params& prm = a.prm;
    const int64_t woff = a.desc[r].word_off;
    const int64_t L = a.desc[r].len;
    const bool has_inv = (a.desc[r].flags & TPS_RD_HAS_INVALID) != 0;
    const bool step1 = (prm.flags & TPS_F_STEP1) != 0;

    const int n1 = (int)(L < prm.no_bp ? L : prm.no_bp);
    const Stage st_s = stage_plan(a.seq2, a.inv, woff, L, false, 0, 0, n1);
    const Stage st_e = stage_plan(a.seq2, a.inv, woff, L, true, 0, 0, n1);

    TPS_STAMP(0);
    TPS_PHASE { for (int i = tid; i < MISC_DW; i += NT) l.misc[i] = 0; }
    TPS_SYNC();
    TPS_STAMP(1);
    TPS_PHASE {
        if (step1) {
            const int hq = a.head_dw >> 2;
            const int side = tid >> 5;
            const Stage& st = side ? st_e : st_s;
            uint32_t* dst = l.seq2 + side * a.head_dw;
            uint32_t* dstv = (uint32_t*)l.val + side * (a.head_dw >> 1);
            for (int c = tid & 31; c < hq; c += 32) {
                u32x4 v;
                u32x2 b;
                v.x = v.y = v.z = v.w = 0;
                b.x = b.y = 0;
                if (c < st.nq) {
                    v = load16(stage_addr(st, c));
                    if (has_inv) b = load8(stage_inv_addr(st, c));
                }
                lds_store16(dst + 4 * c, stage_orient(st, v));
                if (has_inv) {
                    const u32x2 o = stage_orient_inv(st, b);
                    if (o.x | o.y) l.misc[M_INVALID] = 1u;
                    lds_store8(dstv + 2 * c, o);
                }
            }
        }
    }
    TPS_SYNC();

    int tail = 0, pass = 1;
    tps_read_result res;
    res.best_start = res.best_end = 0;
    res.best_start_idx = res.best_end_idx = 0;
    res.n_win = 0; res.bkp = -1; res.gain = 0.0;
    res.flags = 0; res.reserved = 0;

    TPS_STAMP(2);
    if (step1) {
        const bool clean = uniform(l.misc[M_INVALID]) == 0 && pat.dup_mask == 0;
        const bool plain = clean && pat.so_mask == 0;
        bool packed1 = false;
        if constexpr (SV != 0) packed1 = clean && trc_packed_ok(a, st_s.n - pat.k + 1);
        uint32_t ks = 0, ke = 0;
        bool decided = false;
#ifndef TPS_EMU
        if constexpr (SV != 0 && !SO && !RAW) {
            if (packed1) {
                trc_decide_packed<P16K ? 2 : 0>(a, l, st_s, st_e, r, ks, ke);
                decided = true;
                TPS_STAMP(3);
            }
        }
#endif
        if (decided) {
        } else if (packed1) {
            bool fld = false;
            if constexpr (RAW) fld = a.lut_fields != 0;
            if (fld) {
                if constexpr (RAW) { TPS_PHASE { trc_count_packed<SO, F16K ? 3 : 1>(a, l, st_s, st_e, tid); } }
            } else if (SO) {
                TPS_PHASE { trc_count_packed<true, M16K ? 2 : 0>(a, l, st_s, st_e, tid); }
            } else {
                TPS_PHASE { trc_count_packed<false, P16K ? 2 : 0>(a, l, st_s, st_e, tid); }
            }
            TPS_SYNC();
            if (SO && (uniform(l.misc[M_CMASK]) | uniform(l.misc[M_CMASK + 1]))) {
                TPS_PHASE { trc_publish_occ(a, l, st_s, st_e, tid); }
                TPS_SYNC();
            }
            TPS_STAMP(3);
            TPS_PHASE { trc_sum_packed(a, l, st_s, st_e, r, tid); }
        } else {
            TPS_PHASE { for (int i = tid; i < HIST_DW; i += NT) l.blk[i] = 0; }
            TPS_SYNC();
            if (plain) {
                TPS_PHASE { trc_count_thread<true>(a, l, st_s, st_e, tid); }
            } else {
                TPS_PHASE { trc_count_thread<false>(a, l, st_s, st_e, tid); }
            }
            TPS_SYNC();
            TPS_STAMP(3);
            TPS_PHASE { trc_sum_thread(a, l, st_s, st_e, r, tid); }
        }
        if (!decided) {
            TPS_SYNC();
            ks = uniform(l.misc[M_BEST]);
            ke = uniform(l.misc[M_BEST + 1]);
        }
        res.best_start = (int32_t)(ks >> 5); res.best_start_idx = 31 - (int32_t)(ks & 31u);
        res.best_end = (int32_t)(ke >> 5); res.best_end_idx = 31 - (int32_t)(ke & 31u);
        tail = res.best_start > res.best_end ? 0 : 1;
        int best = tail ? res.best_end : res.best_start;
        pass = (L > prm.min_len && best > prm.min_count) ? 1 : 0;
    } else if (a.tails_in) {
        uint8_t tv = a.tails_in[r];
        tail = tv & 1;
        pass = (tv & 2) ? 0 : 1;
    }
    res.tail = tail;
    res.pass = pass;
    TPS_STAMP(4);

    int n_win = 0;
    uint64_t s_total = 0;
    if (pass && (prm.flags & TPS_F_WINDOWS)) {
        const int64_t m = L < prm.maxlen ? L : prm.maxlen;
        const int64_t n_s = m - prm.trimfirst;
        if (n_s >= prm.window) n_win = (int)((n_s - prm.window) / prm.slide) + 1;
        if (n_win / prm.jump + 1 > a.lc_cap) n_win = 0;
        const int64_t out_base = a.win_off ? a.win_off[r] : 0;
        if constexpr (SV == 0) {
            const uint64_t lc_gen = a.lc_global ? (uint64_t)(uintptr_t)(a.lc_scratch + r * (int64_t)a.lc_stride) : 0ull;
            const int blk_per_tile = a.spans_per_tile << a.blk_log2;
            const int tw = blk_per_tile - a.q - 1;
            for (int w0 = 0; w0 < n_win; w0 += tw) {
                const int nw_tile = (n_win - w0) < tw ? (n_win - w0) : tw;
                const int64_t i0 = (int64_t)w0 * prm.slide;
                int64_t n_stage = n_s - i0;
                const int64_t cap = (int64_t)blk_per_tile * prm.slide + 32;
                if (n_stage > cap) n_stage = cap;
                const Stage st = stage_plan(a.seq2, a.inv, woff, L, tail == 1, prm.trimfirst, i0, (int)n_stage);
                const int blk_need = nw_tile + a.q + 1;
                const int spans = (blk_need + (1 << a.blk_log2) - 1) >> a.blk_log2;
                const int ndw = spans * a.span_dw + 8 < a.seq_dw ? spans * a.span_dw + 8 : a.seq_dw;
                TPS_PHASE { if (tid == 0) l.misc[M_INVALID] = 0; }
                TPS_SYNC();
                TPS_PHASE { stage_thread(st, has_inv, l.seq2, l.val, (ndw + 3) >> 2, &l.misc[M_INVALID], tid); }
                TPS_SYNC();
                if (w0 == 0) TPS_STAMP(5);
                TPS_PHASE {
                    for (int sp = tid; sp < spans; sp += NT) blocks_span(a, l, st.delta, sp);
                }
                TPS_SYNC();
                if (w0 == 0) TPS_STAMP(6);
                wg_exclusive_scan(l.Tot, spans, &l.misc[M_SCAN]);
                if (w0 == 0) TPS_STAMP(7);
                for (int base = 0; base < nw_tile; base += WIN_U * NT) {
                    TPS_PHASE { windows_group(a, l, st.delta, w0, nw_tile, out_base, base, tid); }
                    TPS_SYNC();
                    const uint32_t gsum = wg_exclusive_scan(l.row, WIN_U * NT, &l.misc[M_SCAN]);
                    TPS_PHASE { candidates_group(a, l, lc_gen, w0, nw_tile, base, (uint32_t)s_total, tid); }
                    s_total += gsum;
                    TPS_SYNC();
                }
                if (w0 == 0) TPS_STAMP(8);
            }
        } else {
            typedef TileGeo<SV ? SV : 1, FULL> t_;
            constexpr int PF = t_::PF;
            const TileConst tc = tile_const(a, r);
            int tw = (int)uniform((uint32_t)a.tw);
            TPS_PIN_S(tw);
            bool pp = false;
            if constexpr (RAW) pp = a.pp_d >= 0 && (SO ? a.pp_d > 0 : (a.pp_d == 0 && a.raw != nullptr));
            bool pp_expect = a.so_fast != 2;
            auto tile_stage = [&](int w0_) {
                const int64_t i0 = (int64_t)w0_ * prm.slide;
                int64_t n_stage = n_s - i0;
                int64_t cap = (int64_t)t_::BASES;
                const int64_t need = (int64_t)(tw - 1 + tc.q) * prm.slide + tc.r + 13;
                if (cap > need) cap = need;
                const int ns32 = (int)n_stage, cap32 = (int)cap;
                const int n_st = ns32 > cap32 ? cap32 : ns32;
                return stage_plan(a.seq2, a.inv, woff, L, tail == 1, prm.trimfirst, i0, n_st);
            };
            LaneArr<u32x4, PF> pf_;
            LaneArr<u32x2, PF> pv_;
            TPS_LANES { for (int u = 0; u < PF; ++u) TPS_AT(pv_)[u].x = TPS_AT(pv_)[u].y = 0; }
            const bool rv = tail == 1;
            constexpr bool ORIENT = !RAW && !SO && PF == 1;
            Lane<uint32_t> pf_off(0);
            if constexpr (ORIENT) {
                TPS_LANES {
                    TPS_AT(pf_off) = stage_lane_off(rv, tid);
                    TPS_PIN_V(TPS_AT(pf_off));
                }
            }
            auto pf_load = [&](const Stage& stn, int tid) {
                u32x4* const pf = TPS_AT(pf_);
                u32x2* const pv = TPS_AT(pv_);
                TPS_UNROLL
                for (int u = 0; u < PF; ++u) {
                    const int c = tid + u * NT;
                    pf[u].x = pf[u].y = pf[u].z = pf[u].w = 0;
                    if constexpr (!ORIENT) pv[u].x = pv[u].y = 0;
                    if (c < stn.nq) {
                        const uint32_t off = ORIENT ? TPS_AT(pf_off) : stage_lane_off(rv, tid);
                        pf[u] = load16(stage_base(stn, u * NT) + off);
                        if (has_inv) pv[u] = load8(stage_inv_base(stn, u * NT) + (off >> 1));
                    }
                }
            };
            TPS_ISA_REGION(1);
            if (n_win > 0) {
                const Stage st0 = tile_stage(0);
                TPS_PHASE {
                    if (tid == 0) { l.misc[M_INVALID] = 0; l.misc[M_NTIE] = 0; }
                    pf_load(st0, tid);
                }
            }
            for (int w0 = 0, tile = 0; w0 < n_win; w0 += tw, ++tile) {
                const int nw_tile = (n_win - w0) < tw ? (n_win - w0) : tw;
                TPS_ISA_REGION(2);
                const Stage st = tile_stage(w0);
                TPS_PHASE {
                    const u32x4* const pf = TPS_AT(pf_);
                    const u32x2* const pv = TPS_AT(pv_);
                    TPS_UNROLL
                    for (int u = 0; u < PF; ++u) {
                        const int c = tid + u * NT;
                        if (c < t_::NQ) {
                            if constexpr (!ORIENT) lds_store16(l.seq2 + SEQ_LEAD + 4 * c, stage_orient(st, pf[u]));
                            else if (rv) lds_store16(l.seq2 + SEQ_LEAD + 4 * c, stage_reversed(pf[u]));
                            else lds_store16(l.seq2 + SEQ_LEAD + 4 * c, pf[u]);
                            if (has_inv) {
                                u32x2 o;
                                o.x = o.y = 0;
                                if (!ORIENT || c < st.nq) o = stage_orient_inv(st, pv[u]);
                                if (o.x | o.y) l.misc[M_INVALID] = 1u;
                                lds_store8((uint32_t*)l.val + (SEQ_LEAD >> 1) + 2 * c, o);
                            }
                        }
                    }
                    if (tid == NT - 1) {
                        u32x4 z;
                        z.x = z.y = z.z = z.w = 0;
                        lds_store16(l.seq2, z);
                        if (has_inv) { u32x2 z2; z2.x = z2.y = 0; lds_store8((uint32_t*)l.val, z2); }
                    }
                }
                TPS_SYNC();
                TPS_ISA_REGION(3);
                if (w0 + tw < n_win) {
                    const Stage stn = tile_stage(w0 + tw);
                    TPS_PHASE { pf_load(stn, tid); }
                }
                if (w0 == 0) TPS_STAMP(5);
                TPS_ISA_REGION(4);
                const int fdelta = st.delta + 16 * SEQ_LEAD;
                if constexpr (RAW) {
                    constexpr int SP = SV ? SV : 5;
                    if (pp && uniform(l.misc[M_INVALID]) == 0) {
                        if constexpr (SO) {
                            constexpr int HD = F16K ? 5 : 4, HR = (F16K ? 94 : 95) % SP;
                            const bool home = a.pp_d == HD && tc.r == HR;
                            bool chained = true;
                            if (a.so_fast && !pp_expect) {
                                if (home) chained = tile_pp_s<SP, 0, HD, F16K, HR>(a, tc, l, fdelta, w0, tile, nw_tile, out_base, s_total);
                                else switch (a.pp_d) {
                                    case 2: chained = tile_pp_s<SP, 0, 2, F16K>(a, tc, l, fdelta, w0, tile, nw_tile, out_base, s_total); break;
                                    case 3: chained = tile_pp_s<SP, 0, 3, F16K>(a, tc, l, fdelta, w0, tile, nw_tile, out_base, s_total); break;
                                    case 4: chained = tile_pp_s<SP, 0, 4, F16K>(a, tc, l, fdelta, w0, tile, nw_tile, out_base, s_total); break;
                                    case 5: chained = tile_pp_s<SP, 0, 5, F16K>(a, tc, l, fdelta, w0, tile, nw_tile, out_base, s_total); break;
                                    default: chained = tile_pp_s<SP, 0, (SP < 6 ? SP : 6), F16K>(a, tc, l, fdelta, w0, tile, nw_tile, out_base, s_total); break;
                                }
                            }
                            if (!chained) { pp_expect = false; continue; }
                            const uint64_t s_before = s_total;
                            if (home) tile_pp_s<SP, HD, 0, F16K, HR>(a, tc, l, fdelta, w0, tile, nw_tile, out_base, s_total);
                            else switch (a.pp_d) {
                                case 2: tile_pp_s<SP, 2, 0, F16K>(a, tc, l, fdelta, w0, tile, nw_tile, out_base, s_total); break;
                                case 3: tile_pp_s<SP, 3, 0, F16K>(a, tc, l, fdelta, w0, tile, nw_tile, out_base, s_total); break;
                                case 4: tile_pp_s<SP, 4, 0, F16K>(a, tc, l, fdelta, w0, tile, nw_tile, out_base, s_total); break;
                                case 5: tile_pp_s<SP, 5, 0, F16K>(a, tc, l, fdelta, w0, tile, nw_tile, out_base, s_total); break;
                                default: tile_pp_s<SP, (SP < 6 ? SP : 6), 0, F16K>(a, tc, l, fdelta, w0, tile, nw_tile, out_base, s_total); break;
                            }
                            pp_expect = a.so_fast != 2 && (s_total - s_before) > (uint64_t)nw_tile * (uint64_t)(pat.P + 4);
                        } else {
// ... 269 lines not shown
```

### topsicle_amd/csrc/tps_plan.h

```cpp
#pragma once
#include <cstdlib>
#include <algorithm>
#include <cstdint>
#include <string>
#include <vector>

#include "tps_device.h"

namespace tps {

inline int64_t window_count(int64_t L, int W, int s, int t, int M) {
    int64_t m = std::min<int64_t>(L, M);
    int64_t ns = m - t;
    if (W < 1 || s < 1 || ns < W) return 0;
    return (ns - W) / s + 1;
}

inline void plan_dispatch_order(const int64_t* n_win, const uint8_t* passes, int64_t n, std::vector<int32_t>& order) {
    order.clear();
    if (n < 2 || n > 0x7FFFFFFFll) return;
    constexpr int NCLS = 64;
    int64_t mx = 0;
    for (int64_t i = 0; i < n; ++i) if (passes[i] && n_win[i] > mx) mx = n_win[i];
    if (mx == 0) return;
    auto cls = [&](int64_t i) -> int { return passes[i] ? (int)(1 + (n_win[i] * (NCLS - 2) + mx - 1) / mx) : 0; };
    int64_t cnt[NCLS + 1] = {0};
    for (int64_t i = 0; i < n; ++i) ++cnt[cls(i)];
    int used = 0;
    for (int c = 0; c < NCLS; ++c) used += cnt[c] != 0;
    if (used < 2) return;
    int64_t start[NCLS];
    int64_t acc = 0;
    for (int c = NCLS - 1; c >= 0; --c) { start[c] = acc; acc += cnt[c]; }
    order.resize((size_t)n);
    for (int64_t i = 0; i < n; ++i) order[(size_t)start[cls(i)]++] = (int32_t)i;
}

inline int64_t sums16_slots(int64_t nw) { return (nw + 7) & ~7ll; }

inline int gcd_i(int a, int b) { while (b) { int t = a % b; a = b; b = t; } return a; }

inline std::string build_patterns(const char* pats, int P, int k, std::vector<uint32_t>& lut, PatInfo& pi) {
    if (k < 1 || k > TPS_MAX_K) return "k=" + std::to_string(k) + " not supported (1.." + std::to_string(TPS_MAX_K) + ")";
    if (P < 1 || P > TPS_MAX_PATTERNS) return std::to_string(P) + " patterns not supported (1.." + std::to_string(TPS_MAX_PATTERNS) + ")";
    const bool hashed = k > TPS_DIRECT_K;
    if (!hashed) lut.assign((size_t)1 << (2 * k), 0u);
    pi = PatInfo{};
    pi.P = P;
    pi.k = k;
    pi.kmask = (1u << (2 * k)) - 1u;
    pi.all_mask = (1u << P) - 1u;
    uint32_t per_pat[16] = {0, 0, 0, 0, 0, 0, 0, 0, 0, 0, 0, 0, 0, 0, 0, 0};
    std::vector<uint32_t> code_mask((size_t)P, 0u);
    std::vector<uint32_t> codes((size_t)P);
    for (int p = 0; p < P; ++p) {
        uint32_t code = 0;
        char up[16];
        for (int i = 0; i < k; ++i) {
            char ch = pats[p * k + i];
            if (ch >= 'a' && ch <= 'z') ch = (char)(ch - 32);
            up[i] = ch;
            uint32_t v;
            switch (ch) {
                case 'A': v = 0; break;
                case 'C': v = 1; break;
                case 'T': v = 2; break;
                case 'G': v = 3; break;
                default: return "pattern " + std::to_string(p) + " has a non-ACGT letter";
            }
            code |= v << (2 * i);
        }
        if (!hashed) lut[code] |= 1u << p;
        codes[(size_t)p] = code;
        for (int d = 1; d < k; ++d) {
            bool periodic = true;
            for (int i = 0; i + d < k; ++i) periodic = periodic && (up[i] == up[i + d]);
            if (periodic) { per_pat[d] |= 1u << p; pi.so_mask |= 1u << p; }
        }
    }
    for (int p = 0; p < P; ++p)
        for (int o = 0; o < P; ++o)
            if (codes[(size_t)o] == codes[(size_t)p]) code_mask[(size_t)p] |= 1u << o;
    for (int p = 0; p < P; ++p)
        if (code_mask[(size_t)p] & (code_mask[(size_t)p] - 1)) pi.dup_mask |= 1u << p;
    if (hashed) {
        const int log2h = 8;
        const uint32_t H = 1u << log2h;
        uint32_t mul = 0;
        for (uint32_t cand = 0x9E3779B1u, tries = 0; tries < 200000 && !mul; ++tries, cand += 0xC657CB56u) {
            const uint32_t m = cand | 1u;
            std::vector<int> owner(H, -1);
            bool ok = true;
            for (int p = 0; p < P && ok; ++p) {
                const uint32_t slot = (codes[(size_t)p] * m) >> (32 - log2h);
                if (owner[slot] >= 0 && codes[(size_t)owner[slot]] != codes[(size_t)p]) ok = false;
                else owner[slot] = p;
            }
            if (ok) mul = m;
        }
        if (!mul) return "no collision-free hash for this pattern table";
        lut.assign((size_t)2 * H, 0u);
        for (uint32_t i = 0; i < H; ++i) lut[2 * i] = 0xFFFFFFFFu;
        for (int p = 0; p < P; ++p) {
            const uint32_t slot = (codes[(size_t)p] * mul) >> (32 - log2h);
            lut[2 * slot] = codes[(size_t)p];
            lut[2 * slot + 1] = code_mask[(size_t)p];
        }
        pi.hash_mul = mul;
        pi.hash_shift = 32 - log2h;
    }
    for (int d = 1; d < k; ++d)
        if (per_pat[d]) {
            if (pi.n_periods == 8) return "pattern table has more than 8 distinct self-overlap periods";
            pi.period[pi.n_periods] = d;
            pi.period_pat[pi.n_periods] = per_pat[d];
            ++pi.n_periods;
        }
    return "";
}

inline int fused_seq_dw(int slide) {
    const int bases = NT * 8 * slide + 13 + 15;
    const int nq = (63 + bases + 63) / 64;
    const int seq = SEQ_LEAD + 4 * nq + 4;
    return seq < 144 ? 144 : seq;
}

inline void plan_wpg(ScanArgs& a, int64_t budget_dw, int max_waves_simd = 8) {
    auto waves_per_cu = [&](int w) {
        a.wpg = w;
        const int64_t dw = wg_lds_dwords(a);
        if (dw > budget_dw) return 0;
        const int64_t gran = std::max<int64_t>(1, (dw * 4 + 1279) / 1280);
        const int64_t wgs = std::min<int64_t>(std::min<int64_t>(8, 128 / gran), (4 * max_waves_simd) / w);
        return (int)std::min<int64_t>(32, wgs * w);
    };
    int best = WPG, best_w = waves_per_cu(WPG);
    if (lut_dw(a) * 4 >= 8192 || (a.pair16 && (a.pair_n + lut_dw(a)) * 4 >= 8192)) {
        const int v = waves_per_cu(WPG_MAX);
        if (v > best_w) { best = WPG_MAX; best_w = v; }
    }
    a.wpg = best;
}


inline bool has_specialised_slide(int s) { return s == 5 || s == 6 || s == 7 || s == 8; }
inline bool has_default_only_slide(int s) { return s == 3 || s == 4 || (s >= 9 && s <= 12); }

struct PlanKnobs {
    int spans_per_tile = 0;
    int force_generic = 0;
    int force_pair = 0;
    int so_order = 0;
    int wpg = 0;
};

inline std::string plan_geometry_core(ScanArgs& a, const tps_params& prm, int k, int P, int64_t max_nwin, int64_t budget_dw, const PlanKnobs& kn);
inline std::string plan_geometry(ScanArgs& a, const tps_params& prm, int k, int P, int64_t max_nwin, int64_t budget_dw,
                                 const PlanKnobs& kn = PlanKnobs()) {
    a.wpg = WPG;
    std::string err = plan_geometry_core(a, prm, k, P, max_nwin, budget_dw, kn);
    if (err.empty() && a.variant && !a.pat.hash_shift) {
        const int64_t single_bytes = (int64_t)a.lut_n * (a.lut16 ? 2 : 4);
        if ((single_bytes & (single_bytes - 1)) != 0 || ((int64_t)a.pair_n * 4) % single_bytes != 0)
            err = "LDS plan: the single table (" + std::to_string(single_bytes) + " B) would not be aligned behind a pair table of " + std::to_string((int64_t)a.pair_n * 4) + " B";
    }
    if (err.empty()) {
        const bool raw = (prm.flags & TPS_F_STORE_RAW) != 0;
        plan_wpg(a, budget_dw, !a.variant ? 8 : raw ? 5 : a.pat.so_mask != 0 ? 6 : 8);
        if ((kn.wpg == WPG || kn.wpg == WPG_MAX) && a.variant) {
            const int32_t keep = a.wpg;
            a.wpg = kn.wpg;
            if (wg_lds_dwords(a) > budget_dw) a.wpg = keep;
        }
    }
    return err;
}
inline std::string plan_geometry_core(ScanArgs& a, const tps_params& prm, int k, int P, int64_t max_nwin, int64_t budget_dw, const PlanKnobs& kn) {
    const int spans_pref = kn.spans_per_tile, force_generic = kn.force_generic;
    a.lut_n = a.pat.hash_shift ? 2 * 256 : 1 << (2 * k);
    a.lw = std::max(0, prm.window - k);
    a.q = a.lw / prm.slide;
    a.r = a.lw % prm.slide;
    if (max_nwin > 500000) return "too many windows per read (" + std::to_string(max_nwin) + ")";
    {
        int min_per = k;
        for (int i = 0; i < a.pat.n_periods; ++i) min_per = std::min(min_per, std::max(1, (int)a.pat.period[i]));
        const int64_t occ_max = a.lw > 0 ? (a.lw - 1) / min_per + 1 : 0;
        if ((prm.flags & TPS_F_STORE_RAW) && occ_max > 255)
            return "raw counts are bytes: a pattern can occur " + std::to_string(occ_max) + " times in a window of " +
                   std::to_string(prm.window) + " (max 255); use a smaller --windowSize with --rawcountpattern";
        const int64_t sw_max = (int64_t)P * ((a.lw + k - 1) / k + 1);
        if (max_nwin * sw_max >= (1ll << 32)) return "window sums of one read exceed 32 bits (windows per read x window size too large)";
        if ((double)max_nwin * (double)max_nwin * (double)max_nwin * (double)sw_max >= 18446744073709551616.0 )
            return "change-point arithmetic would exceed 128 bits (windows per read x window size too large)";
    }
    const int jump = std::max(prm.jump, 1);
    a.lc_cap = (int)(max_nwin / jump + 2);
    a.jump_magic = jump == 1 ? 0u : (uint32_t)(((1ull << 32) + (uint64_t)jump - 1) / (uint64_t)jump);
    a.head_dw = 4 * ((prm.no_bp + 63 + 63) / 64) + 4;
    int max_period = 0;
    for (int i = 0; i < a.pat.n_periods; ++i) max_period = std::max(max_period, a.pat.period[i]);
    const bool sw16_ok = (int64_t)P * ((a.lw + k - 1) / k + 1) < 65536;
    const int one_period = (a.pat.dup_mask == 0 && k >= 4 && a.pat.n_periods == 1 && a.pat.period[0] >= 2 && 2 * a.pat.period[0] >= k) ? a.pat.period[0] : 0;
    const bool p16_ok = P == 16 && a.pat.dup_mask == 0 && !(prm.flags & TPS_F_STORE_RAW) &&
                        (a.pat.so_mask == 0 || (!a.val_on && one_period > 0 && one_period <= prm.slide && a.lw <= 255));
    const bool fused = !force_generic && spans_pref <= 0 && k <= TPS_DIRECT_K && (has_specialised_slide(prm.slide) || (has_default_only_slide(prm.slide) && a.pat.so_mask == 0 && !(prm.flags & TPS_F_STORE_RAW))) &&
                       (P <= 15 || p16_ok) && a.q >= 8 && sw16_ok &&
                       a.q / 8 + 2 < (XLANES - NT) && max_period <= std::min(prm.slide, 6) &&
                       2 * a.head_dw <= fused_seq_dw(prm.slide);
    a.lc16 = 0; a.tile_cap = 0; a.tw = 0; a.tw_magic = 0; a.pair_n = 0; a.lc_global = 0; a.lc_stride = 0; a.pp_d = -1; a.so_fast = 0; a.seq_alias = 0; a.lut_fields = 0; a.tile_full = 0;
    a.lut16 = 0; a.xt_alias = 0; a.xt_own = 0; a.pair16 = 0;
    if (fused) {
        const bool pp_counts = a.pat.dup_mask == 0 && k >= 4 && P <= 14 && (8 * prm.slide + k - 1) / k <= 14 && (prm.slide + k - 1) / k <= 2 &&
                               a.lw / k + 2 <= 127;
        if (pp_counts && a.pat.n_periods == 0) a.pp_d = 0;
        if (pp_counts && a.pat.n_periods == 1 && a.pat.period[0] >= 2 && 2 * a.pat.period[0] >= k) a.pp_d = a.pat.period[0];
        if (!(prm.flags & TPS_F_STORE_RAW) && P > 14 && one_period > 0) a.pp_d = one_period;
        a.lut_fields = (a.pp_d >= 0 && (prm.flags & TPS_F_STORE_RAW)) ? 1 : 0;
        a.so_fast = kn.so_order == 2 ? 2 : 1;
        if (!(prm.flags & TPS_F_STORE_RAW) && a.pp_d > 0 && a.lw > 255) a.so_fast = 0;
        if (a.pat.so_mask != 0 && !(prm.flags & TPS_F_STORE_RAW)) {
            a.lut16 = 1;
            a.xt_alias = 2;
            a.xt_own = (a.val_on || !a.so_fast || a.pp_d <= 0) ? 1 : 0;
        }
        if (prm.flags & TPS_F_STORE_RAW) {
            if (a.lut_fields && a.pat.so_mask != 0 && a.pp_d > 0 && a.lut_n >= 4096) a.lut16 = 1;
            a.xt_alias = 2;
            a.xt_own = (a.val_on || (a.pat.so_mask != 0 ? a.pp_d <= 0 : a.pp_d != 0)) ? 1 : 0;
        }
        if (a.pat.so_mask == 0 && !(prm.flags & TPS_F_STORE_RAW)) { a.xt_alias = 2; a.xt_own = 0; }
        a.variant = prm.slide;
        a.blk_log2 = 3;
        a.span_dw = 0;
        a.spans_per_tile = NT;
        a.nblk_cap = NT * 8;
        a.rec_rs = 0;
        a.tot_dw = 4;
        a.tile_full = 1;
        a.seq_dw = fused_seq_dw(prm.slide);
        a.seq_alias = 0;
#ifndef TPS_EMU
        if (a.pat.so_mask == 0 && !(prm.flags & TPS_F_STORE_RAW)) a.seq_alias = 1;
#endif
        a.tw = ((int)NT * 8 - a.q - 1) & ~1;
        a.tw_magic = (uint32_t)(((1ull << 32) + (uint64_t)a.tw - 1) / (uint64_t)a.tw);
        a.tile_cap = (int)((max_nwin + a.tw - 1) / a.tw) + 1;
        a.lc16 = 0;
        a.lc_global = 1;
        a.lc_stride = 2 * ((a.lc_cap + 1) & ~1);
        a.pair_n = (a.pat.so_mask == 0 && k <= 4 && !(prm.flags & TPS_F_STORE_RAW)) ? (1 << (2 * (k + 1))) : 0;
        if (a.pat.so_mask == 0 && k <= 4 && (prm.flags & TPS_F_STORE_RAW) && a.lut_fields && a.pp_d == 0 && prm.slide == 6 && a.r == 0) a.pair_n = 1 << (2 * (k + 1));
        a.pair16 = 0;
        if (a.pat.so_mask == 0 && a.pat.dup_mask == 0 && k == 5 && P <= 15 && has_specialised_slide(prm.slide) && !(prm.flags & TPS_F_STORE_RAW)) {
            a.pair16 = 1;
            a.lut16 = 1;
            a.pair_n = (1 << (2 * (k + 1))) / 2;
        }
        a.blk_dw = (int32_t)blk_region_dw(a);
        if (a.pair_n && !kn.force_pair) {
            auto waves_per_cu = [&](int w) {
                const int32_t w0 = a.wpg;
                a.wpg = w;
                const int64_t dw = wg_lds_dwords(a);
                a.wpg = w0;
                if (dw > budget_dw) return 0;
                return (int)(std::min<int64_t>(8, 128 / std::max<int64_t>(1, (dw * 4 + 1279) / 1280)) * w);
            };
            const int with_pair = a.pair16 ? std::max(waves_per_cu(WPG), waves_per_cu(WPG_MAX)) : waves_per_cu(WPG);
            const int32_t keep = a.pair_n;
            const int32_t keep16 = a.pair16;
            a.pair_n = 0;
            if (keep16) { a.lut16 = 0; a.pair16 = 0; }
            if (with_pair >= 5 * WPG || waves_per_cu(WPG) <= with_pair) { a.pair_n = keep; if (keep16) { a.pair16 = 1; a.lut16 = 1; } }
        }
        if (wg_lds_dwords(a) <= budget_dw) return "";
        a.lc16 = 0; a.tile_cap = 0; a.tw = 0; a.tw_magic = 0; a.pair_n = 0; a.lc_global = 0; a.lc_stride = 0; a.pp_d = -1; a.so_fast = 0; a.seq_alias = 0; a.lut_fields = 0;
        a.lut16 = 0; a.xt_alias = 0; a.xt_own = 0; a.pair16 = 0;
    }
    a.variant = 0;
    a.lc_global = 1;
    a.lc_stride = 2 * ((a.lc_cap + 1) & ~1);
    const int g = gcd_i(prm.slide, 16);
    a.span_dw = prm.slide / g;
    const int bps = 16 / g;
    a.blk_log2 = 0;
    while ((1 << a.blk_log2) < bps) ++a.blk_log2;
    const int max_spans = 2 * NT;
    const int min_spans = (a.q + 2 + bps - 1) / bps;
    const int64_t need_blk = max_nwin + a.q + 1;
    const int need_spans = (int)std::min<int64_t>((need_blk + bps - 1) / bps, max_spans);
    int spans = spans_pref > 0 ? std::min(spans_pref, max_spans) : std::min(std::max(need_spans, 1), (int)NT);
    spans = std::max(min_spans, std::min(spans, std::max(need_spans, 1)));
    if (spans > max_spans) return "window/slide combination needs " + std::to_string(spans) + " spans per tile (max " + std::to_string(max_spans) + ")";
    auto fill = [&](int sp) {
        a.spans_per_tile = sp;
        a.nblk_cap = sp * bps;
        a.rec_rs = 0;
        a.tot_dw = std::max(((sp + 2) / 2) * 2, (int)NT);
        a.seq_dw = (std::max(sp * a.span_dw + 8, 2 * a.head_dw) + 3) & ~3;
        a.blk_dw = (int32_t)blk_region_dw(a);
        return wg_lds_dwords(a);
    };
    if (spans_pref > 0) {
        if (fill(spans) > budget_dw)
            return "LDS plan does not fit with " + std::to_string(spans) + " spans per tile";
        return "";
    }
    while (fill(spans) > budget_dw) {
        if (spans <= min_spans)
            return "LDS plan does not fit: window=" + std::to_string(prm.window) + " slide=" + std::to_string(prm.slide) +
                   " k=" + std::to_string(k) + " windows/read=" + std::to_string(max_nwin);
        spans = std::max(min_spans, spans / 2);
    }
    return "";
}

template <typename F>
inline int stride_base(const ScanArgs& planned, const tps_params& prm, int k, int P, F max_nwin_of, int64_t budget_dw, const PlanKnobs& kn) {
    if (planned.variant != 0 || kn.force_generic || kn.spans_per_tile > 0 || !(prm.flags & TPS_F_WINDOWS)) return 0;
    for (int s0 = 12; s0 >= 3; --s0) {
        if (prm.slide <= s0 || prm.slide % s0 != 0 || prm.slide / s0 > 6) continue;
        if (!has_specialised_slide(s0) && !has_default_only_slide(s0)) continue;
        ScanArgs t{};
        t.val_on = planned.val_on;
        t.pat = planned.pat;
        tps_params pb = prm;
        pb.slide = s0;
        pb.flags = (prm.flags | TPS_F_STORE_SUMS) & ~(uint32_t)TPS_F_BINSEG;
        if (plan_geometry(t, pb, k, P, max_nwin_of(s0), budget_dw, kn).empty() && t.variant != 0) return s0;
    }
    return 0;
}

}
```

### topsicle_amd/csrc/tps_wave.h

```cpp
#pragma once
#include <stdint.h>

#ifdef TPS_EMU
#define TPS_DEV static inline
#define TPS_HD static inline
#define TPS_AT(x) ((x).v[tid])
#define TPS_PHASE for (int tid = 0; tid < tps::NT; ++tid)
#define TPS_LANES for (int tid = 0; tid < tps::NT; ++tid)
#define TPS_PHASE_WITH(ln) for (int tid = (ln) * 0; tid < tps::NT; ++tid)
#define TPS_SYNC() ((void)0)
#define TPS_FENCE_WG() ((void)0)
#define TPS_UNROLL
#define TPS_NOVEC
#define TPS_PIN_S(x) ((void)0)
#define TPS_PIN_V(x) ((void)0)
#else
#define TPS_DEV __device__ __forceinline__
#define TPS_HD __host__ __device__ inline
#define TPS_AT(x) (x)
__device__ __forceinline__ int tps_fresh_lane() {
    int t = (int)(threadIdx.x & 63u);
    asm volatile("" : "+v"(t));
    return t;
}
#define TPS_PHASE for (int tid = tps_fresh_lane(), once_ = 1; once_; once_ = 0)
#define TPS_LANES for (int tid = (int)(threadIdx.x & 63u), once_ = 1; once_; once_ = 0)
#define TPS_PHASE_WITH(ln) if (const int tid = (ln); true)
#define TPS_SYNC() do { __builtin_amdgcn_fence(__ATOMIC_SEQ_CST, "wavefront"); __builtin_amdgcn_wave_barrier(); } while (0)
#define TPS_FENCE_WG() __builtin_amdgcn_fence(__ATOMIC_SEQ_CST, "workgroup")
#define TPS_UNROLL _Pragma("unroll")
#define TPS_NOVEC _Pragma("clang loop vectorize(disable) interleave(disable) unroll(disable)")
#define TPS_PIN_S(x) asm volatile("" : "+s"(x))
#define TPS_PIN_V(x) asm volatile("" : "+v"(x))
#endif

#if defined(TPS_ISA_MARKS) && !defined(TPS_EMU)
#define TPS_STAMP(i) asm volatile(";tps_stamp %0" ::"i"(i))
#define TPS_ISA_MARK(id) asm volatile(";tps_mark %0" ::"i"(id))
#define TPS_ISA_REGION(id) asm volatile(";tps_region %0" ::"i"(id))
#elif defined(TPS_EMU) || !defined(TPS_STAMPS)
#define TPS_STAMP(i) ((void)0)
#define TPS_ISA_MARK(id) ((void)(id))
#define TPS_ISA_REGION(id) ((void)(id))
#else
#define TPS_STAMP(i) do { if (a.stamps && (threadIdx.x & 63u) == 0) a.stamps[r * 16 + (i)] = __builtin_readcyclecounter(); } while (0)
#define TPS_ISA_MARK(id) ((void)(id))
#define TPS_ISA_REGION(id) ((void)(id))
#endif
#if defined(TPS_EMU) || !defined(TPS_STAMPS)
#define TPS_PP_STAMP(i) ((void)0)
#else
#define TPS_PP_STAMP(i) do { if (w0 == 0 && a.stamps && (threadIdx.x & 63u) == 0) a.stamps[tc.rd * 16 + (i)] = __builtin_readcyclecounter(); } while (0)
#endif

namespace tps {

constexpr int NT = 64;

#ifdef TPS_EMU
inline int& emu_counter(int i) { static int c[8] = {0, 0, 0, 0, 0, 0, 0, 0}; return c[i]; }
#define TPS_EMU_COUNT(i) ((void)++tps::emu_counter(i))
#define TPS_EMU_COUNT_N(i, n) ((void)(tps::emu_counter(i) += (int)(n)))
TPS_DEV int tps_fresh_lane() { return 0; }
#else
#define TPS_EMU_COUNT(i) ((void)0)
#define TPS_EMU_COUNT_N(i, n) ((void)0)
#endif

#ifdef TPS_EMU
template <typename T>
struct Lane {
    T v[NT];
    Lane() {}
    Lane(T x) { for (int t = 0; t < NT; ++t) v[t] = x; }
};
template <typename T, int N>
struct LaneArr {
    T v[NT][N];
};
#else
template <typename T> using Lane = T;
template <typename T, int N> using LaneArr = T[N];
#endif

#ifdef TPS_EMU
TPS_DEV uint64_t wave_ballot(const Lane<bool>& p) {
    uint64_t m = 0;
    for (int t = 0; t < NT; ++t) m |= (uint64_t)(p.v[t] ? 1 : 0) << t;
    return m;
}
#else
TPS_DEV uint64_t wave_ballot(const Lane<bool>& p) { return __builtin_amdgcn_ballot_w64(p); }
#endif
#ifdef TPS_EMU
TPS_DEV Lane<uint32_t> wave_incl_sum(const Lane<uint32_t>& x) {
    Lane<uint32_t> r;
    uint32_t acc = 0;
    for (int t = 0; t < NT; ++t) { acc += x.v[t]; r.v[t] = acc; }
    return r;
}
TPS_DEV Lane<uint32_t> wave_excl_sum(const Lane<uint32_t>& x) {
    Lane<uint32_t> r;
    uint32_t acc = 0;
    for (int t = 0; t < NT; ++t) { r.v[t] = acc; acc += x.v[t]; }
    return r;
}
#else
TPS_DEV Lane<uint32_t> wave_incl_sum(const Lane<uint32_t>& x) {
    uint32_t inc = x;
    inc += (uint32_t)__builtin_amdgcn_update_dpp(0, (int)inc, 0x111, 0xf, 0xf, false);
    inc += (uint32_t)__builtin_amdgcn_update_dpp(0, (int)inc, 0x112, 0xf, 0xf, false);
    inc += (uint32_t)__builtin_amdgcn_update_dpp(0, (int)inc, 0x114, 0xf, 0xf, false);
    inc += (uint32_t)__builtin_amdgcn_update_dpp(0, (int)inc, 0x118, 0xf, 0xf, false);
    inc += (uint32_t)__builtin_amdgcn_update_dpp(0, (int)inc, 0x142, 0xa, 0xf, false);
    inc += (uint32_t)__builtin_amdgcn_update_dpp(0, (int)inc, 0x143, 0xc, 0xf, false);
    return inc;
}
TPS_DEV Lane<uint32_t> wave_excl_sum(const Lane<uint32_t>& x) { return wave_incl_sum(x) - x; }
#endif
#ifdef TPS_EMU
TPS_DEV uint32_t wave_max_u32(const Lane<uint32_t>& x) {
    uint32_t m = 0;
    for (int t = 0; t < NT; ++t) m = x.v[t] > m ? x.v[t] : m;
    return m;
}
#else
TPS_DEV uint32_t wave_max_u32(const Lane<uint32_t>& x) {
    uint32_t v = x;
    auto mx = [](uint32_t a, uint32_t b) { return a > b ? a : b; };
    v = mx(v, (uint32_t)__builtin_amdgcn_update_dpp(0, (int)v, 0x111, 0xf, 0xf, false));
    v = mx(v, (uint32_t)__builtin_amdgcn_update_dpp(0, (int)v, 0x112, 0xf, 0xf, false));
    v = mx(v, (uint32_t)__builtin_amdgcn_update_dpp(0, (int)v, 0x114, 0xf, 0xf, false));
    v = mx(v, (uint32_t)__builtin_amdgcn_update_dpp(0, (int)v, 0x118, 0xf, 0xf, false));
    v = mx(v, (uint32_t)__builtin_amdgcn_update_dpp(0, (int)v, 0x142, 0xa, 0xf, false));
    v = mx(v, (uint32_t)__builtin_amdgcn_update_dpp(0, (int)v, 0x143, 0xc, 0xf, false));
    return (uint32_t)__builtin_amdgcn_readlane((int)v, 63);
}
#endif
#ifdef TPS_EMU
TPS_DEV uint32_t wave_read_lane(const Lane<uint32_t>& x, int src) { return x.v[src]; }
TPS_DEV uint32_t wave_shuffle(const Lane<uint32_t>& x, int tid, int src) { (void)tid; return x.v[src]; }
#else
TPS_DEV uint32_t wave_read_lane(const Lane<uint32_t>& x, int src) { return (uint32_t)__builtin_amdgcn_readlane((int)x, src); }
TPS_DEV uint32_t wave_shuffle(const Lane<uint32_t>& x, int tid, int src) { (void)tid; return (uint32_t)__builtin_amdgcn_ds_bpermute(src << 2, (int)x); }
#endif

#ifdef TPS_EMU
TPS_DEV uint32_t alignbit(uint32_t hi, uint32_t lo, uint32_t sh) {
    return (uint32_t)(((((uint64_t)hi) << 32) | lo) >> (sh & 31));
}
TPS_DEV uint32_t udot4(uint32_t a, uint32_t b) {
    uint32_t s = 0;
    for (int i = 0; i < 4; ++i) s += ((a >> (8 * i)) & 255u) * ((b >> (8 * i)) & 255u);
    return s;
}
TPS_DEV uint32_t perm(uint32_t s0, uint32_t s1, uint32_t sel) {
    uint32_t out = 0;
    for (int i = 0; i < 4; ++i) {
        uint32_t c = (sel >> (8 * i)) & 255u, byte;
        if (c < 4) byte = (s1 >> (8 * c)) & 255u;
        else if (c < 8) byte = (s0 >> (8 * (c - 4))) & 255u;
        else byte = (c >= 13) ? 255u : 0u;
        out |= byte << (8 * i);
    }
    return out;
}
TPS_DEV int popc(uint32_t x) { return __builtin_popcount(x); }
TPS_DEV int ffs0(uint32_t x) { return __builtin_ctz(x); }
TPS_DEV uint32_t uniform(uint32_t x) { return x; }
TPS_DEV float rcp_f32(float x) { return 1.0f / x; }
TPS_DEV void lds_add(uint32_t* p, uint32_t v) { *p += v; }
TPS_DEV void lds_or(uint32_t* p, uint32_t v) { *p |= v; }
TPS_DEV uint32_t lds_add_ret(uint32_t* p, uint32_t v) { uint32_t o = *p; *p += v; return o; }
TPS_DEV void lds_max_u64(uint64_t* p, uint64_t v) { if (v > *p) *p = v; }
TPS_DEV void lds_max_i32(int32_t* p, int32_t v) { if (v > *p) *p = v; }
TPS_DEV void hist_add(unsigned long long* p) { *p += 1ull; }
struct u32x4 { uint32_t x, y, z, w; };
struct u32x2 { uint32_t x, y; };
TPS_DEV u32x4 load16(const uint8_t* p) { return *(const u32x4*)p; }
TPS_DEV u32x2 load8(const uint8_t* p) { return *(const u32x2*)p; }
TPS_DEV uint32_t bitrev32(uint32_t x) {
    x = ((x >> 1) & 0x55555555u) | ((x & 0x55555555u) << 1);
    x = ((x >> 2) & 0x33333333u) | ((x & 0x33333333u) << 2);
    x = ((x >> 4) & 0x0F0F0F0Fu) | ((x & 0x0F0F0F0Fu) << 4);
    return __builtin_bswap32(x);
}
#else
TPS_DEV uint32_t alignbit(uint32_t hi, uint32_t lo, uint32_t sh) { return __builtin_amdgcn_alignbit(hi, lo, sh); }
TPS_DEV uint32_t udot4(uint32_t a, uint32_t b) { return __builtin_amdgcn_udot4(a, b, 0u, false); }
TPS_DEV uint32_t perm(uint32_t s0, uint32_t s1, uint32_t sel) { return __builtin_amdgcn_perm(s0, s1, sel); }
TPS_DEV int popc(uint32_t x) { return __builtin_popcount(x); }
TPS_DEV int ffs0(uint32_t x) { return __builtin_ctz(x); }
TPS_DEV uint32_t uniform(uint32_t x) { return (uint32_t)__builtin_amdgcn_readfirstlane((int)x); }
TPS_DEV float rcp_f32(float x) { return __builtin_amdgcn_rcpf(x); }
TPS_DEV void lds_add(uint32_t* p, uint32_t v) { atomicAdd(p, v); }
TPS_DEV void lds_or(uint32_t* p, uint32_t v) { atomicOr(p, v); }
TPS_DEV uint32_t lds_add_ret(uint32_t* p, uint32_t v) { return atomicAdd(p, v); }
TPS_DEV void lds_max_u64(uint64_t* p, uint64_t v) { atomicMax((unsigned long long*)p, (unsigned long long)v); }
TPS_DEV void lds_max_i32(int32_t* p, int32_t v) { atomicMax(p, v); }
TPS_DEV void hist_add(unsigned long long* p) { atomicAdd(p, 1ull); }
typedef uint4 u32x4;
typedef uint2 u32x2;
TPS_DEV u32x4 load16(const uint8_t* p) {
    typedef unsigned int v4u __attribute__((ext_vector_type(4)));
    typedef const __attribute__((address_space(1))) v4u* gptr_t;
    const v4u t = *(gptr_t)(uintptr_t)p;
    u32x4 r;
    r.x = t.x; r.y = t.y; r.z = t.z; r.w = t.w;
    return r;
}
TPS_DEV u32x2 load8(const uint8_t* p) {
    typedef unsigned int v2u __attribute__((ext_vector_type(2)));
    typedef const __attribute__((address_space(1))) v2u* gptr_t;
    const v2u t = *(gptr_t)(uintptr_t)p;
    u32x2 r;
    r.x = t.x; r.y = t.y;
    return r;
}
TPS_DEV uint32_t bitrev32(uint32_t x) { return __builtin_bitreverse32(x); }
#endif

#ifdef TPS_EMU
TPS_DEV void wg_max_bits(uint64_t bits, uint64_t* slot) { lds_max_u64(slot, bits); }
#else
TPS_DEV void wg_max_bits(uint64_t bits, uint64_t* slot) {
    TPS_UNROLL
    for (int d = 32; d >= 1; d >>= 1) {
        uint32_t lo = __shfl_xor((uint32_t)bits, d), hi = __shfl_xor((uint32_t)(bits >> 32), d);
        uint64_t o = ((uint64_t)hi << 32) | lo;
        bits = o > bits ? o : bits;
    }
    if ((threadIdx.x & 63) != 0) return;
    lds_max_u64(slot, bits);
}
#endif

#ifdef TPS_EMU
TPS_DEV uint32_t lut_at(const uint32_t* lut, uint32_t v4, uint32_t amask) { return *(const uint32_t*)((const char*)lut + (v4 & amask)); }
#else
TPS_DEV uint32_t lut_at(const uint32_t* lut, uint32_t v4, uint32_t amask) {
    typedef const __attribute__((address_space(3))) uint32_t* lptr_t;
    const uint32_t base = (uint32_t)(uintptr_t)(lptr_t)lut;
    return *(lptr_t)(uintptr_t)((v4 & amask) | base);
}
#endif

#ifdef TPS_EMU
TPS_DEV uint32_t lut16_at(const uint32_t* lut, uint32_t v2, uint32_t amask1) { return *(const uint16_t*)((const char*)lut + (v2 & amask1)); }
#define lut16_at_wide lut16_at
#else
TPS_DEV uint32_t lut16_at(const uint32_t* lut, uint32_t v2, uint32_t amask1) {
    typedef const __attribute__((address_space(3))) uint16_t* lptr16_t;
    const uint32_t base = (uint32_t)(uintptr_t)(const __attribute__((address_space(3))) uint32_t*)lut;
    return *(lptr16_t)(uintptr_t)((v2 & amask1) | base);
}
TPS_DEV uint32_t lut16_at_wide(const uint32_t* lut, uint32_t v2, uint32_t amask1) {
    uint32_t h = lut16_at(lut, v2, amask1);
    asm("" : "+v"(h));
    return h;
}
#endif

#ifdef TPS_EMU
TPS_DEV void g8_store(uint64_t base, uint32_t i, uint32_t v) { ((uint8_t*)(uintptr_t)base)[i] = (uint8_t)v; }
TPS_DEV void g16_store(uint64_t base, uint32_t i, uint32_t v) { ((uint16_t*)(uintptr_t)base)[i] = (uint16_t)v; }
TPS_DEV uint32_t g16_load(uint64_t base, uint32_t i) { return ((const uint16_t*)(uintptr_t)base)[i]; }
TPS_DEV void g32_store(uint64_t base, uint32_t i, uint32_t v) { ((uint32_t*)(uintptr_t)base)[i] = v; }
TPS_DEV uint32_t g32_load(uint64_t base, uint32_t i) { return ((const uint32_t*)(uintptr_t)base)[i]; }
TPS_DEV uint32_t g32_load_at(uint64_t base, uint32_t byte_off) { return *(const uint32_t*)(uintptr_t)(base + byte_off); }
#else
TPS_DEV void g8_store(uint64_t base, uint32_t i, uint32_t v) {
    typedef __attribute__((address_space(1))) uint8_t* gp_t;
    ((gp_t)(uintptr_t)base)[i] = (uint8_t)v;
}
TPS_DEV void g16_store(uint64_t base, uint32_t i, uint32_t v) {
    typedef __attribute__((address_space(1))) uint16_t* gp_t;
    ((gp_t)(uintptr_t)base)[i] = (uint16_t)v;
}
TPS_DEV uint32_t g16_load(uint64_t base, uint32_t i) {
    typedef const __attribute__((address_space(1))) uint16_t* gp_t;
    return ((gp_t)(uintptr_t)base)[i];
}
TPS_DEV uint32_t g32_load_at(uint64_t base, uint32_t byte_off) {
    typedef const __attribute__((address_space(1))) uint8_t* gb_t;
    typedef const __attribute__((address_space(1))) uint32_t* gp_t;
    return *(gp_t)((gb_t)(uintptr_t)base + byte_off);
}
TPS_DEV void g32_store(uint64_t base, uint32_t i, uint32_t v) {
    typedef __attribute__((address_space(1))) uint32_t* gp_t;
    ((gp_t)(uintptr_t)base)[i] = v;
}
TPS_DEV uint32_t g32_load(uint64_t base, uint32_t i) {
    typedef const __attribute__((address_space(1))) uint32_t* gp_t;
    return ((gp_t)(uintptr_t)base)[i];
}
#endif

TPS_DEV uint32_t mulhi32(uint32_t x, uint32_t y) { return (uint32_t)(((uint64_t)x * (uint64_t)y) >> 32); }
TPS_DEV uint32_t mul24(uint32_t x, uint32_t y) { return (x & 0xFFFFFFu) * (y & 0xFFFFFFu); }
#ifdef TPS_EMU
TPS_DEV uint32_t add_bytes(uint32_t v, uint32_t acc) { return acc + (v & 255u) + ((v >> 8) & 255u) + ((v >> 16) & 255u) + (v >> 24); }
#else
TPS_DEV uint32_t add_bytes(uint32_t v, uint32_t acc) { return __builtin_amdgcn_sad_u8(v, 0u, acc); }
#endif

#ifdef TPS_EMU
TPS_DEV uint32_t pk_u16_sub(uint32_t a, uint32_t b) { return ((a - b) & 0xFFFFu) | (((a >> 16) - (b >> 16)) << 16); }
TPS_DEV uint32_t pk_u16_add(uint32_t a, uint32_t b) { return ((a + b) & 0xFFFFu) | (((a >> 16) + b) << 16); }
#else
typedef unsigned short tps_u16x2 __attribute__((ext_vector_type(2)));
TPS_DEV tps_u16x2 as_u16x2(uint32_t v) { return __builtin_bit_cast(tps_u16x2, v); }
TPS_DEV uint32_t pk_u16_sub(uint32_t a, uint32_t b) { return __builtin_bit_cast(uint32_t, as_u16x2(a) - as_u16x2(b)); }
TPS_DEV uint32_t pk_u16_add(uint32_t a, uint32_t b) { return __builtin_bit_cast(uint32_t, as_u16x2(a) + (tps_u16x2)((unsigned short)b)); }
#endif

#ifdef TPS_EMU
TPS_DEV u32x4 lds_load16(const uint32_t* p) { u32x4 v; v.x = p[0]; v.y = p[1]; v.z = p[2]; v.w = p[3]; return v; }
TPS_DEV void lds_store16(uint32_t* p, const u32x4& v) { p[0] = v.x; p[1] = v.y; p[2] = v.z; p[3] = v.w; }
TPS_DEV void lds_store8(uint32_t* p, const u32x2& v) { p[0] = v.x; p[1] = v.y; }
#else
TPS_DEV u32x4 lds_load16(const uint32_t* p) { return *(const u32x4*)p; }
TPS_DEV void lds_store16(uint32_t* p, const u32x4& v) { *(u32x4*)p = v; }
TPS_DEV void lds_store8(uint32_t* p, const u32x2& v) { *(u32x2*)p = v; }
#endif

constexpr int STORE_AUX = 2;
#ifdef TPS_EMU
TPS_DEV void g_store_sw8(uint16_t* tile_out, int lane, int nw_tile, const uint32_t* v) {
    for (int i = 0; i < 8; ++i)
        if (8 * lane + i < nw_tile) tile_out[8 * lane + i] = (uint16_t)v[i];
}
TPS_DEV void g_store_sw8p(uint16_t* tile_out, int lane, int nw_tile, const uint32_t* p) {
    for (int i = 0; i < 8; ++i)
        if (8 * lane + i < nw_tile) tile_out[8 * lane + i] = (uint16_t)(p[i >> 1] >> (16 * (i & 1)));
}
#else
TPS_DEV void g_store_sw8(uint16_t* tile_out, int lane, int nw_tile, const uint32_t* v) {
    typedef unsigned int v4u __attribute__((ext_vector_type(4)));
    const __amdgpu_buffer_rsrc_t rs = __builtin_amdgcn_make_buffer_rsrc((void*)tile_out, 0, ((nw_tile + 1) & ~1) * 2, 0x00020000);
    v4u t;
    t.x = v[0] | (v[1] << 16); t.y = v[2] | (v[3] << 16); t.z = v[4] | (v[5] << 16); t.w = v[6] | (v[7] << 16);
    __builtin_amdgcn_raw_buffer_store_b128(t, rs, lane * 16, 0, STORE_AUX);
}
TPS_DEV void g_store_sw8p(uint16_t* tile_out, int lane, int nw_tile, const uint32_t* p) {
    typedef unsigned int v4u __attribute__((ext_vector_type(4)));
    const __amdgpu_buffer_rsrc_t rs = __builtin_amdgcn_make_buffer_rsrc((void*)tile_out, 0, ((nw_tile + 1) & ~1) * 2, 0x00020000);
    v4u t;
    t.x = p[0]; t.y = p[1]; t.z = p[2]; t.w = p[3];
    __builtin_amdgcn_raw_buffer_store_b128(t, rs, lane * 16, 0, STORE_AUX);
}
#endif
#ifdef TPS_EMU
TPS_DEV void g_store16_clamped(uint32_t* base, int n_dw, int cdw, const u32x4& t) {
    const uint32_t v[4] = {t.x, t.y, t.z, t.w};
    for (int i = 0; i < 4; ++i)
        if (cdw + i < n_dw) base[cdw + i] = v[i];
}
#else
TPS_DEV void g_store16_clamped(uint32_t* base, int n_dw, int cdw, const u32x4& t) {
    typedef unsigned int v4u __attribute__((ext_vector_type(4)));
    const __amdgpu_buffer_rsrc_t rs = __builtin_amdgcn_make_buffer_rsrc((void*)base, 0, n_dw * 4, 0x00020000);
    v4u x;
    x.x = t.x; x.y = t.y; x.z = t.z; x.w = t.w;
    __builtin_amdgcn_raw_buffer_store_b128(x, rs, cdw * 4, 0, STORE_AUX);
}
#endif

}
```

Before: 3872 billion.

## Drop LDS/16-bit candidate paths, streamline binseg prefilter and add single-winner fast path

Removes the unused lc16 and LDS-resident candidate-prefix paths so the scan always writes candidate prefixes to global scratch, shrinking LDS layout and branches. Lane-owned candidate stores become branchless bounds-clamped buffer stores. The binseg prefilter is restructured with incremental integer/float accumulation, unchecked loads for full groups, and med3 for the runner-up tracking. When exactly one lane is close to the max and the wave is not crowded, the exact double refinement pass is skipped in favour of a single-lane recomputation. This adds risk around tie detection and exactness assumptions (int_d now also requires tot below 2^24).

Measured after the change: 3977 billion (median of 6 runs). 2.7% higher.

```diff
diff --git a/__graft_entry__.py b/__graft_entry__.py
--- a/__graft_entry__.py
+++ b/__graft_entry__.py
@@ -63,9 +63,11 @@
 def build_emulation():
     sys.path.insert(0, os.path.join(ROOT, "tests"))
     sys.path.insert(0, ROOT)
+    import emu_binseg_driver
     import emu_driver
     import emu_wide_driver
     emu_driver.build()
+    emu_binseg_driver.build()
     emu_wide_driver.build()
 
 
diff --git a/topsicle_amd/csrc/tps_device.h b/topsicle_amd/csrc/tps_device.h
--- a/topsicle_amd/csrc/tps_device.h
+++ b/topsicle_amd/csrc/tps_device.h
@@ -67,14 +67,11 @@
     int32_t lc_cap;
     uint32_t jump_magic;
     int32_t q, r, lw;
-    int32_t lc16;
     int32_t lc_global;
     int32_t lc_stride;
     uint16_t* lc_scratch;
     int32_t pair_n;
-    int32_t tile_cap;
     int32_t tw;
-    uint32_t tw_magic;
     int32_t tile_full;
     int32_t wpg;
     int32_t pp_d;
@@ -117,9 +114,6 @@
     uint32_t* XF;
     uint32_t* XT;
     uint32_t* Tot;
-    uint32_t* Lc;
-    uint16_t* Lc16;
-    uint32_t* Tc;
     uint32_t* row;
     uint32_t* misc;
 };
@@ -135,10 +129,6 @@
     return (need + 3) & ~3ll;
 }
 TPS_HD int64_t val_dw(const ScanArgs& a) { return a.val_on ? ((a.seq_dw + 4 + 3) / 4) * 2 : 0; }
-TPS_HD int64_t lc_dw(const ScanArgs& a) {
-    if (a.lc16) return (a.lc_global ? 0 : ((a.lc_cap + 3) / 4) * 2) + ((a.tile_cap + 1) / 2) * 2;
-    return a.lc_global ? 0 : ((a.lc_cap + 1) / 2) * 2;
-}
 TPS_HD int64_t row_dw(const ScanArgs& a) {
     const int64_t fused = a.variant ? ((int64_t)NT << a.blk_log2) + NT : 0;
     return fused > WIN_U * NT ? fused : WIN_U * NT;
@@ -153,10 +143,6 @@
     l.seq2 = p; p += a.seq_dw;
     l.val = (uint16_t*)p;  p += val_dw(a);
     l.Tot = p;  p += a.tot_dw;
-    l.Lc = p;
-    l.Lc16 = (uint16_t*)p;
-    l.Tc = p + ((a.lc16 && a.lc_global) ? 0 : ((a.lc_cap + 3) / 4) * 2);
-    p += lc_dw(a);
     l.row = p;  p += row_dw(a);
     l.misc = p;
     l.G = l.blk;
@@ -169,7 +155,7 @@
     return l;
 }
 TPS_HD int64_t lds_dwords(const ScanArgs& a) {
-    return (int64_t)a.blk_dw + (a.seq_alias ? 0 : a.seq_dw) + val_dw(a) + a.tot_dw + lc_dw(a) + row_dw(a) + MISC_DW +
+    return (int64_t)a.blk_dw + (a.seq_alias ? 0 : a.seq_dw) + val_dw(a) + a.tot_dw + row_dw(a) + MISC_DW +
            ((a.xt_alias && a.xt_own) ? (a.xt_alias == 2 ? 2 : 1) * XLANES : 0);
 }
 TPS_HD int64_t wg_lds_dwords(const ScanArgs& a) { return a.pair_n + lut_dw(a) + (int64_t)(a.wpg > 0 ? a.wpg : WPG) * ((lds_dwords(a) + 3) & ~3ll); }
@@ -822,8 +808,7 @@
             const uint32_t w = (uint32_t)(w0 + wl);
             const uint32_t c = div_jump(w, a.jump_magic);
             if (c * jump == w && (int)c < a.lc_cap) {
-                if (lc_g) g32_store(lc_g, c, carry + l.row[u * NT + tid]);
-                else l.Lc[c] = carry + l.row[u * NT + tid];
+                g32_store(lc_g, c, carry + l.row[u * NT + tid]);
             }
         }
     }
@@ -831,20 +816,20 @@
 
 struct TileConst {
     int32_t q, r;
-    uint32_t jump, jump_magic, lc_cap, lc16;
+    uint32_t jump, jump_magic, lc_cap;
     uint64_t lc_g;
     uint16_t* sw16;
     int64_t rd;
 };
 TPS_DEV TileConst tile_const(const ScanArgs& a, int64_t r) {
     TileConst t;
-    t.lc_g = a.lc_global ? (uint64_t)(uintptr_t)(a.lc_scratch + r * (int64_t)a.lc_stride) : 0ull;
+    t.lc_g = (uint64_t)(uintptr_t)(a.lc_scratch + r * (int64_t)a.lc_stride);
     t.sw16 = a.sums16 + (a.win_off16 ? a.win_off16[r] : 0);
     t.rd = r;
     t.q = (int32_t)uniform((uint32_t)a.q); t.r = (int32_t)uniform((uint32_t)a.r);
     t.jump = uniform((uint32_t)a.prm.jump); t.jump_magic = uniform(a.jump_magic);
-    t.lc_cap = uniform((uint32_t)a.lc_cap); t.lc16 = uniform((uint32_t)a.lc16);
-    TPS_PIN_S(t.q); TPS_PIN_S(t.r); TPS_PIN_S(t.jump); TPS_PIN_S(t.jump_magic); TPS_PIN_S(t.lc_cap); TPS_PIN_S(t.lc16);
+    t.lc_cap = uniform((uint32_t)a.lc_cap);
+    TPS_PIN_S(t.q); TPS_PIN_S(t.r); TPS_PIN_S(t.jump); TPS_PIN_S(t.jump_magic); TPS_PIN_S(t.lc_cap);
     return t;
 }
 
@@ -894,10 +879,7 @@
     }
     l.val = (uint16_t*)p;
     p += VAL;
-    l.Lc = p;
-    l.Lc16 = (uint16_t*)p;
-    l.Tc = p + ((a.lc16 && a.lc_global) ? 0 : ((a.lc_cap + 3) / 4) * 2);
-    l.XF = p + lc_dw(a);
+    l.XF = p;
     l.XT = l.XF + XLANES;
     return l;
 }
@@ -1190,21 +1172,13 @@
         TPS_PHASE {
             const uint32_t carry = (uint32_t)s_total;
             if (tid == 0) { l.misc[M_INVALID] = 0; l.misc[M_NTIE] = 0; }
-            if (tc.lc16 && tid == 0) l.Tc[tile] = carry;
             uint32_t c = c_lo + (uint32_t)tid;
             uint32_t w = c * jump - (uint32_t)w0;
             TPS_NOVEC
             for (int t = 0; t < passes; ++t) {
                 if (c < c_hi) {
                     const uint32_t pre = l.row[w + (w >> LOG2B)];
-                    if (tc.lc16) {
-                        if (tc.lc_g) g16_store(tc.lc_g, c, pre);
-                        else l.Lc16[c] = (uint16_t)pre;
-                    } else if (tc.lc_g) {
-                        g32_store(tc.lc_g, c, carry + pre);
-                    } else {
-                        l.Lc[c] = carry + pre;
-                    }
+                    g32_store(tc.lc_g, c, carry + pre);
                 }
                 c += NT;
                 w += NT * jump;
@@ -1226,21 +1200,13 @@
     TPS_PHASE {
         const uint32_t carry = (uint32_t)s_total;
         if (tid == 0) { l.misc[M_INVALID] = 0; l.misc[M_NTIE] = 0; }
-        if (tc.lc16 && tid == 0) l.Tc[tile] = carry;
         uint32_t c = c_lo + (uint32_t)tid;
         uint32_t w = c * jump - (uint32_t)w0;
         TPS_NOVEC
         for (int t = 0; t < passes; ++t) {
             if (c < c_hi) {
                 const uint32_t pre = l.row[w + (w >> LOG2B)];
-                if (tc.lc16) {
-                    if (tc.lc_g) g16_store(tc.lc_g, c, pre);
-                    else l.Lc16[c] = (uint16_t)pre;
-                } else if (tc.lc_g) {
-                    g32_store(tc.lc_g, c, carry + pre);
-                } else {
-                    l.Lc[c] = carry + pre;
-                }
+                g32_store(tc.lc_g, c, carry + pre);
             }
             c += NT;
             w += NT * jump;
@@ -1622,7 +1588,10 @@
     }
     const Lane<uint32_t> lexc = wave_excl_sum(ltot);
     bool lane_cands = false;
-    if constexpr (CD == 0 && !M16) lane_cands = tc.lc_g != 0ull && !tc.lc16 && tc.jump >= 4u;
+    if constexpr (CD == 0 && !M16) lane_cands = tc.jump >= 4u;
+    const uint32_t c_lo = div_jump((uint32_t)w0 + tc.jump - 1u, tc.jump_magic);
+    uint32_t c_hi = div_jump((uint32_t)(w0 + nw_tile) + tc.jump - 1u, tc.jump_magic);
+    if (c_hi > tc.lc_cap) c_hi = tc.lc_cap;
     TPS_PHASE {
         const int lane = tid;
         const uint32_t* const sw = TPS_AT(sw_);
@@ -1635,13 +1604,24 @@
         xt_at(lane) = TPS_AT(lexc);
         if (lane_cands) {
             if (tid == 0) TPS_EMU_COUNT(7);
-            const uint32_t carry = (uint32_t)s_total + TPS_AT(lexc);
-            const uint32_t wl = (uint32_t)(lane * B), wa = (uint32_t)w0 + wl;
-            const uint32_t c = mulhi32(wa + tc.jump - 1u, tc.jump_magic);
-            const uint32_t f = c * tc.jump - wa;
-            if (f < (uint32_t)B && wl + f < (uint32_t)nw_tile && c < tc.lc_cap) g32_store(tc.lc_g, c, carry + pr[f]);
-            const uint32_t f2 = f + tc.jump;
-            if (f2 < (uint32_t)B && wl + f2 < (uint32_t)nw_tile && c + 1u < tc.lc_cap) g32_store(tc.lc_g, c + 1u, carry + pr[f2]);
+            auto own_candidates = [&](auto bigj_) {
+                const uint32_t carry = (uint32_t)s_total + TPS_AT(lexc);
+                const uint32_t wa = (uint32_t)w0 + (uint32_t)(lane * B);
+                const uint32_t c = mulhi32(wa + tc.jump - 1u, tc.jump_magic);
+                const uint32_t f = c * tc.jump - wa, f2 = f + tc.jump;
+                uint32_t i1 = c, r1 = f;
+                if constexpr (decltype(bigj_)::value != 0) {
+                    i1 = f < (uint32_t)B ? c : c_hi;
+                    r1 = f < (uint32_t)B ? f : (uint32_t)(B - 1);
+                }
+                const uint32_t i2 = (f2 < (uint32_t)B ? c : c_hi) + 1u;
+                const uint32_t r2 = f2 < (uint32_t)B ? f2 : (uint32_t)(B - 1);
+                const uint32_t v1 = pr[r1], v2 = pr[r2];
+                g32_store_clamped(tc.lc_g, c_hi, i1, carry + v1);
+                g32_store_clamped(tc.lc_g, c_hi, i2, carry + v2);
+            };
+            if (tc.jump > (uint32_t)B) own_candidates(IntC<1>());
+            else own_candidates(IntC<0>());
         }
     }
     TPS_SYNC();
@@ -1650,29 +1630,18 @@
     const uint32_t gsum = uniform(l.row[nw_tile + (nw_tile >> LOG2B)] + xt_at(nw_tile >> LOG2B));
     {
         const uint32_t jump = tc.jump;
-        const uint32_t c_lo = div_jump((uint32_t)w0 + jump - 1u, tc.jump_magic);
-        uint32_t c_hi = div_jump((uint32_t)(w0 + nw_tile) + jump - 1u, tc.jump_magic);
-        if (c_hi > tc.lc_cap) c_hi = tc.lc_cap;
         const int passes = (c_hi > c_lo && !lane_cands) ? (int)((c_hi - c_lo + NT - 1) / NT) : 0;
         TPS_ISA_MARK(MK + 6);
         TPS_PHASE {
             const uint32_t carry = (uint32_t)s_total;
             if (tid == 0) { l.misc[M_INVALID] = 0; l.misc[M_NTIE] = 0; }
-            if (tc.lc16 && tid == 0) l.Tc[tile] = carry;
             uint32_t c = c_lo + (uint32_t)tid;
             uint32_t w = c * jump - (uint32_t)w0;
             TPS_NOVEC
             for (int t = 0; t < passes; ++t) {
                 if (c < c_hi) {
                     const uint32_t pre = l.row[w + (w >> LOG2B)] + xt_at((int)(w >> LOG2B));
-                    if (tc.lc16) {
-                        if (tc.lc_g) g16_store(tc.lc_g, c, pre);
-                        else l.Lc16[c] = (uint16_t)pre;
-                    } else if (tc.lc_g) {
-                        g32_store(tc.lc_g, c, carry + pre);
-                    } else {
-                        l.Lc[c] = carry + pre;
-                    }
+                    g32_store(tc.lc_g, c, carry + pre);
                 }
                 c += NT;
                 w += NT * jump;
@@ -2354,12 +2323,11 @@
     const int c_max = (n - min_size) / jump < ncand ? (n - min_size) / jump : ncand;
     const bool exact53 = (double)n * 4294967296.0 < 9007199254740992.0 && (double)tot * (double)n < 9007199254740992.0;
     const double nf = (double)n, totf = (double)tot;
-    const bool int_d = (double)tot * (double)n < 2147483648.0;
+    const bool int_d = (double)tot * (double)n < 2147483648.0 && tot < (1ull << 24);
     constexpr int LCV = 16;
-    const bool prefilter = !a.lc16 && lc_g && exact53 && c_max - c_min < LCV * NT;
+    const bool prefilter = exact53 && c_max - c_min < LCV * NT;
     int nslot = c_max >= c_min ? (c_max - c_min + NT) / NT : 0;
     TPS_PIN_S(nslot);
-    auto tile_sum = [&](int c) { return l.Tc[(uint32_t)(((uint64_t)(uint32_t)(c * jump) * a.tw_magic) >> 32)]; };
     Lane<float> p_s1_(-1.0f), p_s2_(-1.0f);
     Lane<uint32_t> p_lc_(0);
     Lane<int> p_c_(-1);
@@ -2367,55 +2335,69 @@
     bool crowded = false;
     TPS_ISA_REGION(5);
     if (prefilter) {
-        auto prefilter_phase = [&](auto lean_) {
+        auto prefilter_phase = [&](auto intd_) {
         TPS_PHASE {
+            constexpr bool INTD = decltype(intd_)::value != 0;
             float &p_s1 = TPS_AT(p_s1_), &p_s2 = TPS_AT(p_s2_);
             uint32_t& p_lc = TPS_AT(p_lc_);
-            int& p_c = TPS_AT(p_c_);
-            p_s1 = -1.0f; p_s2 = -1.0f; p_lc = 0; p_c = -1;
-            auto group = [&](int g) {
-                constexpr bool LEAN = decltype(lean_)::value != 0;
+            p_s1 = -1.0f; p_s2 = -1.0f; p_lc = 0;
+            int p_j = -1;
+            const int c0 = c_min + tid;
+            const uint32_t off0 = 4u * (uint32_t)c0;
+            const float nf32 = (float)n, bstep = (float)(NT * jump);
+            float bf = (float)(c0 * jump);
+            const uint32_t ntb_step = 0u - (uint32_t)tot * (uint32_t)(NT * jump);
+            uint32_t ntb = 0u - (uint32_t)tot * (uint32_t)(c0 * jump);
+            auto slot = [&](int j, uint32_t lc, auto last_) {
+                float d32;
+                if constexpr (INTD) {
+                    d32 = (float)(int32_t)(mul24((uint32_t)n, lc) + ntb);
+                    ntb += ntb_step;
+                } else {
+                    d32 = (float)__builtin_fma(-totf, (double)bf, nf * (double)lc);
+                }
+                const float den32 = bf * (nf32 - bf);
+                bf += bstep;
+                float s_ = d32 * d32 * rcp_f32(den32);
+                if constexpr (decltype(last_)::value != 0) s_ = tid <= c_max - c_min - j * NT ? s_ : -1.0f;
+                const bool gt = s_ > p_s1;
+                p_s2 = med3_f32(p_s1, p_s2, s_);
+                p_lc = gt ? lc : p_lc;
+                p_j = gt ? j : p_j;
+                p_s1 = gt ? s_ : p_s1;
+            };
+            auto group = [&](int g, auto checked_) {
+                constexpr bool CHECKED = decltype(checked_)::value != 0;
                 uint32_t lcv[4];
                 TPS_UNROLL
                 for (int i = 0; i < 4; ++i) {
-                    const int c = c_min + tid + (4 * g + i) * NT;
-                    if constexpr (LEAN) lcv[i] = g32_load_at(lc_g, 4u * (uint32_t)(c <= c_max ? c : c_max));
-                    else lcv[i] = c <= c_max ? g32_load(lc_g, (uint32_t)c) : 0u;
-                }
-                const int b0 = (c_min + tid + 4 * g * NT) * jump;
-                const uint32_t tb0 = (uint32_t)tot * (uint32_t)b0, tb_step = (uint32_t)tot * (uint32_t)(NT * jump);
+                    const uint32_t joff = 4u * NT * (uint32_t)(4 * g + i);
+                    if constexpr (CHECKED) lcv[i] = g32_load_at(lc_g, off0 + joff < 4u * (uint32_t)c_max ? off0 + joff : 4u * (uint32_t)c_max);
+                    else lcv[i] = g32_load_at(lc_g + joff, off0);
+                }
                 TPS_UNROLL
-                for (int i = 0; i < 4; ++i) {
-                    const int c = c_min + tid + (4 * g + i) * NT;
-                    const int b = LEAN ? b0 + i * (NT * jump) : c * jump;
-                    float d32;
-                    if constexpr (LEAN) {
-                        uint32_t tb = tb0 + (uint32_t)i * tb_step;
-                        TPS_PIN_V(tb);
-                        d32 = (float)(int32_t)((uint32_t)n * lcv[i] - tb);
-                    } else {
-                        const double bf = (double)b;
-                        d32 = (float)__builtin_fma(-totf, bf, nf * (double)lcv[i]);
-                    }
-                    const float den32 = (float)b * (float)(n - b);
-                    float s_ = d32 * d32 * rcp_f32(den32);
-                    s_ = c <= c_max ? s_ : -1.0f;
-                    const bool gt = s_ > p_s1;
-                    const float lose = gt ? p_s1 : s_;
-                    p_s2 = lose > p_s2 ? lose : p_s2;
-                    p_lc = gt ? lcv[i] : p_lc;
-                    p_c = gt ? c : p_c;
-                    p_s1 = gt ? s_ : p_s1;
-                }
+                for (int i = 0; i < 4; ++i) slot(4 * g + i, lcv[i], checked_);
             };
-            if (nslot > 0) group(0);
-            if (nslot > 4) group(1);
-            if (nslot > 8) group(2);
-            if (nslot > 12) group(3);
+            if constexpr (INTD) {
+                if (nslot > 4) group(0, IntC<0>()); else if (nslot > 0) group(0, IntC<1>());
+                if (nslot > 8) group(1, IntC<0>()); else if (nslot > 4) group(1, IntC<1>());
+                if (nslot > 12) group(2, IntC<0>()); else if (nslot > 8) group(2, IntC<1>());
+                if (nslot > 12) group(3, IntC<1>());
+            } else {
+                if (nslot > 0) group(0, IntC<1>());
+                if (nslot > 4) group(1, IntC<1>());
+                if (nslot > 8) group(2, IntC<1>());
+                if (nslot > 12) group(3, IntC<1>());
+            }
+            TPS_AT(p_c_) = p_j >= 0 ? c0 + p_j * NT : -1;
         }
         };
-        if (int_d) prefilter_phase(IntC<1>());
-        else prefilter_phase(IntC<0>());
+        if (int_d) {
+            prefilter_phase(IntC<1>());
+        } else {
+            TPS_EMU_COUNT(11);
+            prefilter_phase(IntC<0>());
+        }
         float m32;
         {
             Lane<uint32_t> key;
@@ -2430,81 +2412,86 @@
         Lane<bool> close2;
         TPS_LANES { TPS_AT(close2) = TPS_AT(p_s2_) >= thr32 && TPS_AT(p_s2_) >= 0.0f; }
         crowded = wave_ballot(close2) != 0;
-    }
-    TPS_ISA_REGION(6);
-    TPS_PHASE {
-        double bn = -1.0, bd = 1.0;
-        int best_b = -1;
-        bool amb = false;
-        auto offer = [&](int c, uint32_t lc) {
-            const int b = c * jump;
-            const double bf = (double)b;
-            double dd;
-            if (exact53) dd = __builtin_fma(-totf, bf, nf * (double)lc);
-            else dd = (double)((int64_t)n * (int64_t)lc - (int64_t)tot * (int64_t)b);
-            const double num = dd * dd, den = bf * (nf - bf);
-            const double t1 = num * bd, t2 = bn * den;
-            const double diff = t1 - t2;
-            const bool near = __builtin_fabs(diff) <= 1e-13 * t2;
-            const bool take = diff >= 0.0;
-            amb = near || (amb && !take);
-            if (take) { bn = num; bd = den; best_b = b; }
-        };
-        if (prefilter) {
-            if (TPS_AT(p_c_) >= 0 && TPS_AT(p_s1_) >= thr32) offer(TPS_AT(p_c_), TPS_AT(p_lc_));
-        } else if (a.lc16 && lc_g && c_max - c_min < LCV * NT) {
-            uint32_t lcv[LCV];
-            TPS_UNROLL
-            for (int i = 0; i < LCV; ++i) {
-                const int c = c_min + tid + i * NT;
-                lcv[i] = c <= c_max ? g16_load(lc_g, (uint32_t)c) : 0u;
-            }
-            TPS_UNROLL
-            for (int i = 0; i < LCV; ++i) {
-                const int c = c_min + tid + i * NT;
-                if (c <= c_max) offer(c, tile_sum(c) + lcv[i]);
-            }
-        } else {
-            TPS_NOVEC
-            for (int c = c_min + tid; c <= c_max; c += NT) {
-                uint32_t lc;
-                if (a.lc16) lc = tile_sum(c) + (lc_g ? g16_load(lc_g, (uint32_t)c) : (uint32_t)l.Lc16[c]);
-                else lc = lc_g ? g32_load(lc_g, (uint32_t)c) : l.Lc[c];
-                offer(c, lc);
-            }
-        }
-        const double best = best_b >= 0 ? bn / bd : -1.0;
-        uint64_t bits = 0;
-        if (best >= 0.0) __builtin_memcpy(&bits, &best, 8);
-        TPS_AT(best_) = best; TPS_AT(best_b_) = best_b; TPS_AT(amb_) = amb; TPS_AT(bits_) = bits;
+        if (crowded) TPS_EMU_COUNT(10);
+    }
+    uint64_t close = 0;
+    if (prefilter) {
+        Lane<bool> cl;
+        TPS_LANES { TPS_AT(cl) = TPS_AT(p_c_) >= 0 && TPS_AT(p_s1_) >= thr32; }
+        close = wave_ballot(cl);
     }
     double m;
     uint32_t ntie = 0;
     int32_t bestb = -1;
-    {
-        Lane<uint32_t> key;
-        TPS_LANES { TPS_AT(key) = (uint32_t)(TPS_AT(bits_) >> 32); }
-        const uint32_t mh = wave_max_u32(key);
-        TPS_LANES { TPS_AT(key) = (uint32_t)(TPS_AT(bits_) >> 32) == mh ? (uint32_t)TPS_AT(bits_) : 0u; }
-        const uint32_t ml = wave_max_u32(key);
-        const uint64_t mbits = ((uint64_t)mh << 32) | ml;
-        __builtin_memcpy(&m, &mbits, 8);
-        Lane<bool> n1, n1_amb;
-        TPS_LANES {
-            const double best = TPS_AT(best_);
-            const bool amb = TPS_AT(amb_), near = best >= m * (1.0 - 1e-14) && best >= 0.0;
-            TPS_AT(n1) = near;
-            TPS_AT(n1_amb) = near && amb;
-        }
-        ntie = (uint32_t)__builtin_popcountll(wave_ballot(n1)) + (uint32_t)__builtin_popcountll(wave_ballot(n1_amb));
-        TPS_LANES {
-            const double best = TPS_AT(best_);
-            const int best_b = TPS_AT(best_b_);
-            TPS_AT(key) = (best == m && best_b >= 0) ? (uint32_t)best_b + 1u : 0u;
-        }
-        bestb = (int32_t)wave_max_u32(key) - 1;
-    }
-    (void)misc;
+    if (!crowded && close != 0 && (close & (close - 1)) == 0) {
+        TPS_ISA_REGION(8);
+        TPS_EMU_COUNT(8);
+        const int src = __builtin_ctzll(close);
+        const int b = wave_read_lane(p_c_, src) * jump;
+        const uint32_t lc = wave_read_lane(p_lc_, src);
+        const double bf = (double)b;
+        const double dd = __builtin_fma(-totf, bf, nf * (double)lc);
+        const double num = dd * dd, den = bf * (nf - bf);
+        m = num / den;
+        ntie = 1u;
+        bestb = b;
+    } else {
+        TPS_ISA_REGION(6);
+        TPS_EMU_COUNT(9);
+        TPS_PHASE {
+            double bn = -1.0, bd = 1.0;
+            int best_b = -1;
+            bool amb = false;
+            auto offer = [&](int c, uint32_t lc) {
+                const int b = c * jump;
+                const double bf = (double)b;
+                double dd;
+                if (exact53) dd = __builtin_fma(-totf, bf, nf * (double)lc);
+                else dd = (double)((int64_t)n * (int64_t)lc - (int64_t)tot * (int64_t)b);
+                const double num = dd * dd, den = bf * (nf - bf);
+                const double t1 = num * bd, t2 = bn * den;
+                const double diff = t1 - t2;
+                const bool near = __builtin_fabs(diff) <= 1e-13 * t2;
+                const bool take = diff >= 0.0;
+                amb = near || (amb && !take);
+                if (take) { bn = num; bd = den; best_b = b; }
+            };
+            if (prefilter) {
+                if (TPS_AT(p_c_) >= 0 && TPS_AT(p_s1_) >= thr32) offer(TPS_AT(p_c_), TPS_AT(p_lc_));
+            } else {
+                TPS_NOVEC
+                for (int c = c_min + tid; c <= c_max; c += NT) offer(c, g32_load(lc_g, (uint32_t)c));
+            }
+            const double best = best_b >= 0 ? bn / bd : -1.0;
+            uint64_t bits = 0;
+            if (best >= 0.0) __builtin_memcpy(&bits, &best, 8);
+            TPS_AT(best_) = best; TPS_AT(best_b_) = best_b; TPS_AT(amb_) = amb; TPS_AT(bits_) = bits;
+        }
+        {
+            Lane<uint32_t> key;
+            TPS_LANES { TPS_AT(key) = (uint32_t)(TPS_AT(bits_) >> 32); }
+            const uint32_t mh = wave_max_u32(key);
+            TPS_LANES { TPS_AT(key) = (uint32_t)(TPS_AT(bits_) >> 32) == mh ? (uint32_t)TPS_AT(bits_) : 0u; }
+            const uint32_t ml = wave_max_u32(key);
+            const uint64_t mbits = ((uint64_t)mh << 32) | ml;
+            __builtin_memcpy(&m, &mbits, 8);
+            Lane<bool> n1, n1_amb;
+            TPS_LANES {
+                const double best = TPS_AT(best_);
+                const bool amb = TPS_AT(amb_), near = best >= m * (1.0 - 1e-14) && best >= 0.0;
+                TPS_AT(n1) = near;
+                TPS_AT(n1_amb) = near && amb;
+            }
+            ntie = (uint32_t)__builtin_popcountll(wave_ballot(n1)) + (uint32_t)__builtin_popcountll(wave_ballot(n1_amb));
+            TPS_LANES {
+                const double best = TPS_AT(best_);
+                const int best_b = TPS_AT(best_b_);
+                TPS_AT(key) = (best == m && best_b >= 0) ? (uint32_t)best_b + 1u : 0u;
+            }
+            bestb = (int32_t)wave_max_u32(key) - 1;
+        }
+    }
+    (void)misc; (void)a; (void)l;
     TPS_ISA_REGION(7);
     if (crowded) ntie = 2u;
     tie = ntie > 1u;
diff --git a/topsicle_amd/csrc/tps_plan.h b/topsicle_amd/csrc/tps_plan.h
--- a/topsicle_amd/csrc/tps_plan.h
+++ b/topsicle_amd/csrc/tps_plan.h
@@ -209,7 +209,7 @@
                        (P <= 15 || p16_ok) && a.q >= 8 && sw16_ok &&
                        a.q / 8 + 2 < (XLANES - NT) && max_period <= std::min(prm.slide, 6) &&
                        2 * a.head_dw <= fused_seq_dw(prm.slide);
-    a.lc16 = 0; a.tile_cap = 0; a.tw = 0; a.tw_magic = 0; a.pair_n = 0; a.lc_global = 0; a.lc_stride = 0; a.pp_d = -1; a.so_fast = 0; a.seq_alias = 0; a.lut_fields = 0; a.tile_full = 0;
+    a.tw = 0; a.pair_n = 0; a.lc_global = 0; a.lc_stride = 0; a.pp_d = -1; a.so_fast = 0; a.seq_alias = 0; a.lut_fields = 0; a.tile_full = 0;
     a.lut16 = 0; a.xt_alias = 0; a.xt_own = 0; a.pair16 = 0;
     if (fused) {
         const bool pp_counts = a.pat.dup_mask == 0 && k >= 4 && P <= 14 && (8 * prm.slide + k - 1) / k <= 14 && (prm.slide + k - 1) / k <= 2 &&
@@ -245,9 +245,6 @@
         if (a.pat.so_mask == 0 && !(prm.flags & TPS_F_STORE_RAW)) a.seq_alias = 1;
 #endif
         a.tw = ((int)NT * 8 - a.q - 1) & ~1;
-        a.tw_magic = (uint32_t)(((1ull << 32) + (uint64_t)a.tw - 1) / (uint64_t)a.tw);
-        a.tile_cap = (int)((max_nwin + a.tw - 1) / a.tw) + 1;
-        a.lc16 = 0;
         a.lc_global = 1;
         a.lc_stride = 2 * ((a.lc_cap + 1) & ~1);
         a.pair_n = (a.pat.so_mask == 0 && k <= 4 && !(prm.flags & TPS_F_STORE_RAW)) ? (1 << (2 * (k + 1))) : 0;
@@ -276,7 +273,7 @@
             if (with_pair >= 5 * WPG || waves_per_cu(WPG) <= with_pair) { a.pair_n = keep; if (keep16) { a.pair16 = 1; a.lut16 = 1; } }
         }
         if (wg_lds_dwords(a) <= budget_dw) return "";
-        a.lc16 = 0; a.tile_cap = 0; a.tw = 0; a.tw_magic = 0; a.pair_n = 0; a.lc_global = 0; a.lc_stride = 0; a.pp_d = -1; a.so_fast = 0; a.seq_alias = 0; a.lut_fields = 0;
+        a.tw = 0; a.pair_n = 0; a.lc_global = 0; a.lc_stride = 0; a.pp_d = -1; a.so_fast = 0; a.seq_alias = 0; a.lut_fields = 0;
         a.lut16 = 0; a.xt_alias = 0; a.xt_own = 0; a.pair16 = 0;
     }
     a.variant = 0;
diff --git a/topsicle_amd/csrc/tps_wave.h b/topsicle_amd/csrc/tps_wave.h
--- a/topsicle_amd/csrc/tps_wave.h
+++ b/topsicle_amd/csrc/tps_wave.h
@@ -58,7 +58,8 @@
 constexpr int NT = 64;
 
 #ifdef TPS_EMU
-inline int& emu_counter(int i) { static int c[8] = {0, 0, 0, 0, 0, 0, 0, 0}; return c[i]; }
+constexpr int EMU_COUNTERS = 16;
+inline int& emu_counter(int i) { static int c[EMU_COUNTERS] = {0}; return c[i]; }
 #define TPS_EMU_COUNT(i) ((void)++tps::emu_counter(i))
 #define TPS_EMU_COUNT_N(i, n) ((void)(tps::emu_counter(i) += (int)(n)))
 TPS_DEV int tps_fresh_lane() { return 0; }
@@ -139,9 +140,11 @@
 #endif
 #ifdef TPS_EMU
 TPS_DEV uint32_t wave_read_lane(const Lane<uint32_t>& x, int src) { return x.v[src]; }
+TPS_DEV int wave_read_lane(const Lane<int>& x, int src) { return x.v[src]; }
 TPS_DEV uint32_t wave_shuffle(const Lane<uint32_t>& x, int tid, int src) { (void)tid; return x.v[src]; }
 #else
 TPS_DEV uint32_t wave_read_lane(const Lane<uint32_t>& x, int src) { return (uint32_t)__builtin_amdgcn_readlane((int)x, src); }
+TPS_DEV int wave_read_lane(const Lane<int>& x, int src) { return __builtin_amdgcn_readlane(x, src); }
 TPS_DEV uint32_t wave_shuffle(const Lane<uint32_t>& x, int tid, int src) { (void)tid; return (uint32_t)__builtin_amdgcn_ds_bpermute(src << 2, (int)x); }
 #endif
 
@@ -169,6 +172,10 @@
 TPS_DEV int ffs0(uint32_t x) { return __builtin_ctz(x); }
 TPS_DEV uint32_t uniform(uint32_t x) { return x; }
 TPS_DEV float rcp_f32(float x) { return 1.0f / x; }
+TPS_DEV float med3_f32(float a, float b, float c) {
+    const float lo = a < b ? a : b, hi = a < b ? b : a;
+    return c < lo ? lo : (c > hi ? hi : c);
+}
 TPS_DEV void lds_add(uint32_t* p, uint32_t v) { *p += v; }
 TPS_DEV void lds_or(uint32_t* p, uint32_t v) { *p |= v; }
 TPS_DEV uint32_t lds_add_ret(uint32_t* p, uint32_t v) { uint32_t o = *p; *p += v; return o; }
@@ -193,6 +200,7 @@
 TPS_DEV int ffs0(uint32_t x) { return __builtin_ctz(x); }
 TPS_DEV uint32_t uniform(uint32_t x) { return (uint32_t)__builtin_amdgcn_readfirstlane((int)x); }
 TPS_DEV float rcp_f32(float x) { return __builtin_amdgcn_rcpf(x); }
+TPS_DEV float med3_f32(float a, float b, float c) { return __builtin_amdgcn_fmed3f(a, b, c); }
 TPS_DEV void lds_add(uint32_t* p, uint32_t v) { atomicAdd(p, v); }
 TPS_DEV void lds_or(uint32_t* p, uint32_t v) { atomicOr(p, v); }
 TPS_DEV uint32_t lds_add_ret(uint32_t* p, uint32_t v) { return atomicAdd(p, v); }
@@ -365,5 +373,15 @@
     __builtin_amdgcn_raw_buffer_store_b128(x, rs, cdw * 4, 0, STORE_AUX);
 }
 #endif
-
-}
+#ifdef TPS_EMU
+TPS_DEV void g32_store_clamped(uint64_t base, uint32_t n, uint32_t i, uint32_t v) {
+    if (i < n) ((uint32_t*)(uintptr_t)base)[i] = v;
+}
+#else
+TPS_DEV void g32_store_clamped(uint64_t base, uint32_t n, uint32_t i, uint32_t v) {
+    const __amdgpu_buffer_rsrc_t rs = __builtin_amdgcn_make_buffer_rsrc((void*)(uintptr_t)base, 0, (int)(n * 4u), 0x00020000);
+    __builtin_amdgcn_raw_buffer_store_b32(v, rs, (int)(i * 4u), 0, 0);
+}
+#endif
+
+}
```
